# codelion/adaptive-classifier

Hardware: AMD Instinct MI355X
Metric: predict() queries/sec + kNN GB/s vs HBM roofline, 768-d (higher is better)
Workload: dtype f32

## Files before the change

### adaptive-classifier_amd/csrc/bert.hip

```cpp
#include "common.h"
#include "attention_core.h"

#include <math.h>
#include <atomic>
#include <chrono>
#include <string.h>

namespace {

typedef float f32x4 __attribute__((ext_vector_type(4)));
constexpr int kMaxVec = 8;

__device__ __forceinline__ float wave_sum(float v) {
#pragma unroll
    for (int o = 1; o < 64; o <<= 1) v += __shfl_xor(v, o);
    return v;
}

template <bool F16 = false>
__device__ __forceinline__ void layernorm_store(f32x4 (&x)[kMaxVec], int H, int lane, const float* g,
                                                const float* b, float eps, float* dst, uint16_t* planes = nullptr,
                                                int64_t rows = 0, int64_t row = 0) {
    const int nv = H >> 2;
    float s = 0.f;
#pragma unroll
    for (int e = 0; e < kMaxVec; ++e)
        if (lane + 64 * e < nv) s += (x[e].x + x[e].y) + (x[e].z + x[e].w);
    const float mean = wave_sum(s) / (float)H;
    float q = 0.f;
#pragma unroll
    for (int e = 0; e < kMaxVec; ++e)
        if (lane + 64 * e < nv) {
            const float d0 = x[e].x - mean, d1 = x[e].y - mean, d2 = x[e].z - mean, d3 = x[e].w - mean;
            q += (d0 * d0 + d1 * d1) + (d2 * d2 + d3 * d3);
        }
    const float var = wave_sum(q) / (float)H;
    const float rstd = 1.0f / sqrtf(var + eps);
#pragma unroll
    for (int e = 0; e < kMaxVec; ++e) {
        const int c4 = lane + 64 * e;
        if (c4 < nv) {
            const f32x4 gg = *reinterpret_cast<const f32x4*>(g + 4 * c4);
            const f32x4 bb = *reinterpret_cast<const f32x4*>(b + 4 * c4);
            f32x4 y;
            y.x = (x[e].x - mean) * rstd * gg.x + bb.x;
            y.y = (x[e].y - mean) * rstd * gg.y + bb.y;
            y.z = (x[e].z - mean) * rstd * gg.z + bb.z;
            y.w = (x[e].w - mean) * rstd * gg.w + bb.w;
            *reinterpret_cast<f32x4*>(dst + 4 * c4) = y;
            if (planes)
                ac::emit_planes4(planes + ac::plane_off(rows, row, 4 * c4), rows * (int64_t)H, y, F16);
        }
    }
}

template <bool F16>
__global__ __launch_bounds__(256) void embed_ln_kernel(const int64_t* ids, const int64_t* type_ids, int T, int S,
                                                       int H, const float* word, const float* pos,
                                                       const float* type, const float* g, const float* b,
                                                       float eps, float* out, uint16_t* planes,
                                                       const int32_t* __restrict__ tok_src = nullptr,
                                                       const int32_t* __restrict__ t_dev = nullptr) {
    if (t_dev) T = t_dev[0];
    const int lane = threadIdx.x & 63;
    const int t = blockIdx.x * 4 + (threadIdx.x >> 6);
    if (t >= T) return;
    const int src = tok_src ? tok_src[t] : t;
    const int64_t id = ids[src];
    const int64_t tt = type_ids ? type_ids[src] : 0;
    const int p = src % S;
    const int nv = H >> 2;
    f32x4 x[kMaxVec];
#pragma unroll
    for (int e = 0; e < kMaxVec; ++e) {
        const int c4 = lane + 64 * e;
        if (c4 < nv) {
            const f32x4 w = *reinterpret_cast<const f32x4*>(word + id * H + 4 * c4);
            if (type) {
                const f32x4 ty = *reinterpret_cast<const f32x4*>(type + tt * H + 4 * c4);
                const f32x4 po = *reinterpret_cast<const f32x4*>(pos + (int64_t)p * H + 4 * c4);
                x[e] = (w + ty) + po;
            } else {
                x[e] = w;
            }
        }
    }
    layernorm_store<F16>(x, H, lane, g, b, eps, out + (int64_t)t * H, planes, T, t);
}

template <bool F16>
__global__ __launch_bounds__(256) void ln_kernel_t(const float* in, int T, int H, const float* g, const float* b,
                                                   float eps, float* out, uint16_t* planes, int64_t in_stride) {
    const int lane = threadIdx.x & 63;
    const int t = blockIdx.x * 4 + (threadIdx.x >> 6);
    if (t >= T) return;
    const int nv = H >> 2;
    f32x4 x[kMaxVec];
#pragma unroll
    for (int e = 0; e < kMaxVec; ++e) {
        const int c4 = lane + 64 * e;
        if (c4 < nv) x[e] = *reinterpret_cast<const f32x4*>(in + (int64_t)t * in_stride + 4 * c4);
    }
    layernorm_store<F16>(x, H, lane, g, b, eps, out + (int64_t)t * H, planes, T, t);
}

inline void launch_ln(bool f16, int blocks, hipStream_t stream, const float* in, int T, int H, const float* g, const float* b,
                      float eps, float* out, uint16_t* planes, int64_t in_stride) {
    if (f16) hipLaunchKernelGGL(ln_kernel_t<true>, dim3(blocks), dim3(256), 0, stream, in, T, H, g, b, eps, out, planes, in_stride);
    else hipLaunchKernelGGL(ln_kernel_t<false>, dim3(blocks), dim3(256), 0, stream, in, T, H, g, b, eps, out, planes, in_stride);
}

__global__ __launch_bounds__(256) void splitk_ln_normalize_kernel(const float* __restrict__ part, int ksplit, int M, int H,
                                                                  const float* __restrict__ bias, const float* __restrict__ residual,
                                                                  int64_t ldr, const float* __restrict__ g, const float* __restrict__ be,
                                                                  float eps, float* __restrict__ out, int64_t ldo) {
    const int lane = threadIdx.x & 63;
    const int i = blockIdx.x * (blockDim.x >> 6) + (threadIdx.x >> 6);
    if (i >= M) return;
    const int nv = H >> 2;
    const size_t slice = (size_t)M * H;
    f32x4 x[kMaxVec];
    const f32x4 zero4 = {0.f, 0.f, 0.f, 0.f};
#pragma unroll
    for (int e = 0; e < kMaxVec; ++e) x[e] = zero4;
    for (int z0 = 0; z0 < ksplit; z0 += 4) {
        f32x4 t[4][kMaxVec];
#pragma unroll
        for (int u = 0; u < 4; ++u)
#pragma unroll
            for (int e = 0; e < kMaxVec; ++e) {
                const int c4 = lane + 64 * e;
                t[u][e] = (z0 + u < ksplit && c4 < nv) ? *reinterpret_cast<const f32x4*>(part + (size_t)(z0 + u) * slice + (size_t)i * H + 4 * c4) : zero4;
            }
#pragma unroll
        for (int u = 0; u < 4; ++u)
            if (z0 + u < ksplit) {
#pragma unroll
                for (int e = 0; e < kMaxVec; ++e)
                    if (z0 + u == 0) x[e] = t[u][e];
                    else { x[e].x += t[u][e].x; x[e].y += t[u][e].y; x[e].z += t[u][e].z; x[e].w += t[u][e].w; }
            }
    }
#pragma unroll
    for (int e = 0; e < kMaxVec; ++e) {
        const int c4 = lane + 64 * e;
        if (c4 < nv) {
            const f32x4 s = x[e];
            const f32x4 bb = *reinterpret_cast<const f32x4*>(bias + 4 * c4);
            const f32x4 rr = *reinterpret_cast<const f32x4*>(residual + (int64_t)i * ldr + 4 * c4);
            x[e].x = (s.x + bb.x) + rr.x; x[e].y = (s.y + bb.y) + rr.y; x[e].z = (s.z + bb.z) + rr.z; x[e].w = (s.w + bb.w) + rr.w;
        }
    }
    float s = 0.f;
#pragma unroll
    for (int e = 0; e < kMaxVec; ++e)
        if (lane + 64 * e < nv) s += (x[e].x + x[e].y) + (x[e].z + x[e].w);
    const float mean = wave_sum(s) / (float)H;
    float q = 0.f;
#pragma unroll
    for (int e = 0; e < kMaxVec; ++e)
        if (lane + 64 * e < nv) {
            const float d0 = x[e].x - mean, d1 = x[e].y - mean, d2 = x[e].z - mean, d3 = x[e].w - mean;
            q += (d0 * d0 + d1 * d1) + (d2 * d2 + d3 * d3);
        }
    const float var = wave_sum(q) / (float)H;
    const float rstd = 1.0f / sqrtf(var + eps);
    float ss = 0.f;
#pragma unroll
    for (int e = 0; e < kMaxVec; ++e) {
        const int c4 = lane + 64 * e;
        if (c4 < nv) {
            const f32x4 gg = *reinterpret_cast<const f32x4*>(g + 4 * c4);
            const f32x4 bb = *reinterpret_cast<const f32x4*>(be + 4 * c4);
            f32x4 y;
            y.x = (x[e].x - mean) * rstd * gg.x + bb.x;
            y.y = (x[e].y - mean) * rstd * gg.y + bb.y;
            y.z = (x[e].z - mean) * rstd * gg.z + bb.z;
            y.w = (x[e].w - mean) * rstd * gg.w + bb.w;
            x[e] = y;
            ss = fmaf(y.x, y.x, ss); ss = fmaf(y.y, y.y, ss); ss = fmaf(y.z, y.z, ss); ss = fmaf(y.w, y.w, ss);
        }
    }
    const float nrm = fmaxf(sqrtf(wave_sum(ss)), 1e-12f);
#pragma unroll
    for (int e = 0; e < kMaxVec; ++e) {
        const int c4 = lane + 64 * e;
        if (c4 < nv) {
            f32x4 y = x[e];
            y.x = y.x / nrm; y.y = y.y / nrm; y.z = y.z / nrm; y.w = y.w / nrm;
            float* dst = out + (int64_t)i * ldo + 4 * c4;
            dst[0] = y.x; dst[1] = y.y; dst[2] = y.z; dst[3] = y.w;
        }
    }
    for (int c = H + lane; c < ldo; c += 64) out[(int64_t)i * ldo + c] = 0.f;
}

__global__ __launch_bounds__(256) void cls_normalize_kernel(const float* x, int b, int S, int H, float* out,
                                                            int64_t ldo) {
    const int lane = threadIdx.x & 63;
    const int i = blockIdx.x * 4 + (threadIdx.x >> 6);
    if (i >= b) return;
    const float* src = x + (int64_t)i * S * H;
    float s = 0.f;
    for (int c = lane; c < H; c += 64) s = fmaf(src[c], src[c], s);
    const float nrm = fmaxf(sqrtf(wave_sum(s)), 1e-12f);
    for (int c = lane; c < H; c += 64) out[(int64_t)i * ldo + c] = src[c] / nrm;
    for (int c = H + lane; c < ldo; c += 64) out[(int64_t)i * ldo + c] = 0.f;
}

template <bool NORM>
__global__ __launch_bounds__(256) void pool_mean_normalize_kernel(const float* __restrict__ x, const int64_t* __restrict__ mask,
                                                                  const int32_t* __restrict__ cu, int S, int H,
                                                                  const float* __restrict__ g, const float* __restrict__ be, float eps,
                                                                  float* __restrict__ out, int64_t ldo) {
    extern __shared__ __attribute__((aligned(16))) float pool_part[];
    __shared__ int pool_count[4];
    const int lane = threadIdx.x & 63, wv = threadIdx.x >> 6, i = blockIdx.x;
    const int nv = H >> 2;
    const int64_t row0 = cu ? (int64_t)cu[i] : (int64_t)i * S;
    const int n = cu ? cu[i + 1] - cu[i] : S;
    const int64_t* mk = (!cu && mask) ? mask + (int64_t)i * S : nullptr;
    const f32x4 zero4 = {0.f, 0.f, 0.f, 0.f};
    f32x4 acc[kMaxVec];
#pragma unroll
    for (int e = 0; e < kMaxVec; ++e) acc[e] = zero4;
    int count = 0;
    for (int t = wv; t < n; t += 4) {
        if (mk && mk[t] == 0) continue;
        const float* src = x + (row0 + t) * (int64_t)H;
        f32x4 r[kMaxVec];
#pragma unroll
        for (int e = 0; e < kMaxVec; ++e) {
            const int c4 = lane + 64 * e;
            r[e] = c4 < nv ? *reinterpret_cast<const f32x4*>(src + 4 * c4) : zero4;
        }
        if constexpr (NORM) {
            float s = 0.f;
#pragma unroll
            for (int e = 0; e < kMaxVec; ++e)
                if (lane + 64 * e < nv) s += (r[e].x + r[e].y) + (r[e].z + r[e].w);
            const float mean = wave_sum(s) / (float)H;
            float q = 0.f;
#pragma unroll
            for (int e = 0; e < kMaxVec; ++e)
                if (lane + 64 * e < nv) {
                    const float d0 = r[e].x - mean, d1 = r[e].y - mean, d2 = r[e].z - mean, d3 = r[e].w - mean;
                    q += (d0 * d0 + d1 * d1) + (d2 * d2 + d3 * d3);
                }
            const float var = wave_sum(q) / (float)H;
            const float rstd = 1.0f / sqrtf(var + eps);
#pragma unroll
            for (int e = 0; e < kMaxVec; ++e) {
                const int c4 = lane + 64 * e;
                if (c4 < nv) {
                    const f32x4 gg = *reinterpret_cast<const f32x4*>(g + 4 * c4);
                    const f32x4 bb = *reinterpret_cast<const f32x4*>(be + 4 * c4);
                    f32x4 y;
                    y.x = (r[e].x - mean) * rstd * gg.x + bb.x;
                    y.y = (r[e].y - mean) * rstd * gg.y + bb.y;
                    y.z = (r[e].z - mean) * rstd * gg.z + bb.z;
                    y.w = (r[e].w - mean) * rstd * gg.w + bb.w;
                    r[e] = y;
                }
            }
        }
#pragma unroll
        for (int e = 0; e < kMaxVec; ++e) { acc[e].x += r[e].x; acc[e].y += r[e].y; acc[e].z += r[e].z; acc[e].w += r[e].w; }
        ++count;
    }
    if (wv > 0) {
#pragma unroll
        for (int e = 0; e < kMaxVec; ++e) {
            const int c4 = lane + 64 * e;
            if (c4 < nv) *reinterpret_cast<f32x4*>(pool_part + (size_t)(wv - 1) * H + 4 * c4) = acc[e];
        }
        if (lane == 0) pool_count[wv] = count;
    }
    __syncthreads();
    if (wv > 0) return;
    for (int w = 1; w < 4; ++w) {
#pragma unroll
        for (int e = 0; e < kMaxVec; ++e) {
            const int c4 = lane + 64 * e;
            if (c4 < nv) {
                const f32x4 p = *reinterpret_cast<const f32x4*>(pool_part + (size_t)(w - 1) * H + 4 * c4);
                acc[e].x += p.x; acc[e].y += p.y; acc[e].z += p.z; acc[e].w += p.w;
            }
        }
        count += pool_count[w];
    }
    const float den = (float)(count > 1 ? count : 1);
    float ss = 0.f;
#pragma unroll
    for (int e = 0; e < kMaxVec; ++e)
        if (lane + 64 * e < nv) {
            f32x4 y = acc[e];
            y.x = y.x / den; y.y = y.y / den; y.z = y.z / den; y.w = y.w / den;
            acc[e] = y;
            ss = fmaf(y.x, y.x, ss); ss = fmaf(y.y, y.y, ss); ss = fmaf(y.z, y.z, ss); ss = fmaf(y.w, y.w, ss);
        }
    const float nrm = fmaxf(sqrtf(wave_sum(ss)), 1e-12f);
#pragma unroll
    for (int e = 0; e < kMaxVec; ++e) {
        const int c4 = lane + 64 * e;
        if (c4 < nv) {
            float* dst = out + (int64_t)i * ldo + 4 * c4;
            dst[0] = acc[e].x / nrm; dst[1] = acc[e].y / nrm; dst[2] = acc[e].z / nrm; dst[3] = acc[e].w / nrm;
        }
    }
    for (int c = H + lane; c < ldo; c += 64) out[(int64_t)i * ldo + c] = 0.f;
}

constexpr int DH = 64;
constexpr int KT = 64;

using acattn::f32x16;
using acattn::rope_rotate;

__device__ __forceinline__ const float* rel_bias_row(int head, const float* table, int span) {
    return table + (int64_t)head * (2 * span - 1) + (span - 1);
}
template <bool ROPE, int DHT = 64, bool BIAS = false, typename... REL>
__global__ __launch_bounds__(64) void attention_mfma_kernel(const float* qkv, const int64_t* mask, int S_, int H,
                                                            float scale, float* ctx, uint16_t* ctx_planes,
                                                            const float* rope_cos, const float* rope_sin,
                                                            int window, const int32_t* __restrict__ cu = nullptr,
                                                            int64_t total_rows = 0, int f16 = 0, int boundary_stride = 0,
                                                            int nseq = 0, REL... rel) {
    static_assert(sizeof...(REL) == (BIAS ? 2 : 0), "the bias table and its span come with BIAS, and only then");
    const int lane = threadIdx.x;
    const int qt = blockIdx.x, head = blockIdx.y;
    int bi = blockIdx.z;
    if (boundary_stride > 0) {
        const int brow = boundary_stride * ((int)blockIdx.z + 1);
        int lo = 0, hi = nseq;
        while (hi - lo > 1) { const int mid = (lo + hi) >> 1; if (cu[mid] <= brow) lo = mid; else hi = mid; }
        if (cu[lo] == brow || brow >= cu[nseq]) return;
        bi = lo;
    }
    const int64_t ld = 3 * (int64_t)H;
    const int64_t row0 = cu ? (int64_t)cu[bi] : (int64_t)bi * S_;
    const int S = cu ? cu[bi + 1] - cu[bi] : S_;
    if (qt * 32 >= S) return;
    const float* base = qkv + row0 * ld + head * DHT;
    const int64_t rows = cu ? total_rows : (int64_t)gridDim.z * S_;
    if constexpr (BIAS)
        acattn::attention_tile<ROPE, DHT, true, true, true>(base, base + H, base + 2 * H, ld, S, qt, lane, scale,
                                                            mask ? mask + (int64_t)bi * S_ : nullptr, rope_cos, rope_sin, window,
                                                            ctx ? ctx + row0 * H + head * DHT : nullptr, H, ctx_planes, rows, row0,
                                                            head * DHT, f16, rel_bias_row(head, rel...));
    else
        acattn::attention_tile<ROPE, DHT>(base, base + H, base + 2 * H, ld, S, qt, lane, scale, mask ? mask + (int64_t)bi * S_ : nullptr,
                                          rope_cos, rope_sin, window, ctx ? ctx + row0 * H + head * DHT : nullptr, H, ctx_planes, rows,
                                          row0, head * DHT, f16);
}

template <bool ROPE, int DHT = 64, int KTT = KT, bool BIAS = false, typename... REL>
__global__ __launch_bounds__(64) void attention_cls_kernel(const float* qkv, const int64_t* mask, int S_, int H,
                                                           float scale, float* ctx_cls, const float* rope_cos,
                                                           const float* rope_sin, int window,
                                                           const int32_t* __restrict__ cu = nullptr,
                                                           const float* __restrict__ q_cls = nullptr, REL... rel) {
    static_assert(sizeof...(REL) == (BIAS ? 2 : 0), "the bias table and its span come with BIAS, and only then");
    static_assert(DHT == 64 || (DHT == 32 && !ROPE), "head dim 64, or 32 without RoPE");
    __shared__ float Ks[KTT][DHT + 1];
    __shared__ __attribute__((aligned(16))) float Vs[KTT][DHT];
    __shared__ float qs[DHT];
    __shared__ float ps[KTT];
    const int lane = threadIdx.x;
    const int head = blockIdx.x, bi = blockIdx.y;
    const int64_t ld = 3 * (int64_t)H;
    const int64_t row0 = cu ? (int64_t)cu[bi] : (int64_t)bi * S_;
    const int S = cu ? cu[bi + 1] - cu[bi] : S_;
    const float* base = qkv + row0 * ld + head * DHT;
    if (lane < DHT) qs[lane] = (q_cls ? q_cls[(int64_t)bi * H + head * DHT + lane] : base[lane]) * scale;
    float m = -INFINITY, l = 0.f, o = 0.f;
    const int Svis = (window >= 0 && window + 1 < S) ? window + 1 : S;
    for (int k0 = 0; k0 < Svis; k0 += KTT) {
        const int nk = (Svis - k0) < KTT ? (Svis - k0) : KTT;
        const int kl = lane < KTT ? lane : 0;
        __syncthreads();
        constexpr int LPR = DHT / 4;
        for (int r = lane / LPR; r < KTT; r += 64 / LPR) {
            const int c = (lane % LPR) * 4;
            f32x4 kv = {0.f, 0.f, 0.f, 0.f}, vv = {0.f, 0.f, 0.f, 0.f};
            if (r < nk) {
                const float* kp = base + (int64_t)(k0 + r) * ld + H;
                kv = *reinterpret_cast<const f32x4*>(kp + c);
                vv = *reinterpret_cast<const f32x4*>(kp + H + c);
            }
            Ks[r][c] = kv.x; Ks[r][c + 1] = kv.y; Ks[r][c + 2] = kv.z; Ks[r][c + 3] = kv.w;
            *reinterpret_cast<f32x4*>(&Vs[r][c]) = vv;
        }
        __syncthreads();
        const bool valid = lane < nk && (!mask || mask[(int64_t)bi * S_ + k0 + lane] != 0);
        float sc = 0.f;
        if constexpr (ROPE) {
            const int pos = (k0 + lane < S) ? k0 + lane : S - 1;
            const float* cs = rope_cos + (int64_t)pos * 32;
            const float* sn = rope_sin + (int64_t)pos * 32;
#pragma unroll 8
            for (int d = 0; d < 32; ++d) {
                const float lo = Ks[kl][d], hi = Ks[kl][d + 32], c = cs[d], sv = sn[d];
                sc = fmaf(qs[d], lo * c + (-hi) * sv, sc);
                sc = fmaf(qs[d + 32], hi * c + lo * sv, sc);
            }
        } else {
#pragma unroll 16
            for (int d = 0; d < DHT; ++d) sc = fmaf(qs[d], Ks[kl][d], sc);
        }
        if constexpr (BIAS) sc = sc + rel_bias_row(head, rel...)[(k0 + lane < S) ? k0 + lane : S - 1];
        sc = valid ? sc : -INFINITY;
        float cmax = sc;
#pragma unroll
        for (int off = 1; off < 64; off <<= 1) cmax = fmaxf(cmax, __shfl_xor(cmax, off));
        const float m_new = fmaxf(m, cmax);
        if (m_new == -INFINITY) continue;
        const float corr = expf(m - m_new);
        const float p = expf(sc - m_new);
        if (lane < KTT) ps[lane] = p;
        float psum = p;
#pragma unroll
        for (int off = 1; off < 64; off <<= 1) psum += __shfl_xor(psum, off);
        l = l * corr + psum;
        o *= corr;
        __syncthreads();
        if (lane < DHT)
            for (int j = 0; j < nk; ++j) o = fmaf(ps[j], Vs[j][lane], o);
        m = m_new;
    }
    if (lane < DHT) ctx_cls[(int64_t)bi * H + head * DHT + lane] = l > 0.f ? o / l : 0.f;
}

__global__ __launch_bounds__(256) void geglu_kernel(const float* __restrict__ u, int64_t T, int I, float* __restrict__ g,
                                                    uint16_t* __restrict__ planes, int interleaved32) {
    const int nq = I >> 3;
    const int64_t idx = (int64_t)blockIdx.x * 256 + threadIdx.x;
    if (idx >= T * nq) return;
    const int64_t row = idx / nq;
    const int q = (int)(idx - row * nq);
    const int c = 8 * q;
    const float* a = u + row * 2 * (int64_t)I + (interleaved32 ? (c >> 5) * 64 + (c & 31) : c);
    const int goff = interleaved32 ? 32 : I;
    f32x4 o[2];
#pragma unroll
    for (int e = 0; e < 2; ++e) {
        const f32x4 x = *reinterpret_cast<const f32x4*>(a + 4 * e);
        const f32x4 gate = *reinterpret_cast<const f32x4*>(a + goff + 4 * e);
#pragma unroll
        for (int c = 0; c < 4; ++c) o[e][c] = ac::gelu_erf(x[c]) * gate[c];
        *reinterpret_cast<f32x4*>(g + row * I + 8 * q + 4 * e) = o[e];
    }
    if (planes) {
        uint4 Hh, Mm, Ll;
        ac::split8(o[0], o[1], Hh, Mm, Ll);
        uint16_t* p = planes + ac::plane_off(T, row, 8 * q);
        const int64_t plane = T * (int64_t)I;
        *reinterpret_cast<uint4*>(p) = Hh;
        *reinterpret_cast<uint4*>(p + plane) = Mm;
        *reinterpret_cast<uint4*>(p + 2 * plane) = Ll;
    }
}

__global__ __launch_bounds__(256) void pack_lens_kernel(const int64_t* __restrict__ mask, int b, int S, int32_t* __restrict__ lens,
                                                        int32_t* __restrict__ info) {
    const int lane = threadIdx.x & 63;
    const int s = blockIdx.x * 4 + (threadIdx.x >> 6);
    if (s >= b) return;
    int n = 0, bad = 0;
    for (int p0 = 0; p0 < S; p0 += 64) {
        const int p = p0 + lane;
        const bool on = p < S && mask[(int64_t)s * S + p] != 0;
        const uint64_t m = __ballot(on);
        const int ones = __popcll(m);
        const uint64_t want = ones == 64 ? ~0ull : ((1ull << ones) - 1);
        if (m != want || (ones > 0 && n != p0)) bad = 1;
        n += ones;
    }
    if (lane == 0) { lens[s] = n; if (bad || n == 0) atomicOr(&info[1], 1); }
}
__global__ __launch_bounds__(1024) void pack_scan_kernel(const int32_t* __restrict__ lens, int b, int32_t* __restrict__ cu,
                                                         int32_t* __restrict__ info) {
    __shared__ int part[1024];
    const int tid = threadIdx.x;
    const int per = (b + 1023) / 1024;
    int sum = 0, mx = 0;
    for (int i = tid * per; i < (tid + 1) * per && i < b; ++i) { sum += lens[i]; mx = lens[i] > mx ? lens[i] : mx; }
    part[tid] = sum;
    __syncthreads();
    for (int o = 1; o < 1024; o <<= 1) {
        const int v = tid >= o ? part[tid - o] : 0;
        __syncthreads();
        part[tid] += v;
        __syncthreads();
    }
    int run = tid ? part[tid - 1] : 0;
    for (int i = tid * per; i < (tid + 1) * per && i < b; ++i) { cu[i] = run; run += lens[i]; }
    if (tid == 1023) { cu[b] = part[1023]; info[0] = part[1023]; }
    atomicMax(&info[2], mx);
}
__global__ __launch_bounds__(256) void pack_fill_kernel(const int32_t* __restrict__ cu, int b, int S, int32_t* __restrict__ tok_src) {
    const int lane = threadIdx.x & 63;
    const int s = blockIdx.x * 4 + (threadIdx.x >> 6);
    if (s >= b) return;
    const int r0 = cu[s], n = cu[s + 1] - r0;
    for (int p = lane; p < n; p += 64) tok_src[r0 + p] = s * S + p;
}
__global__ __launch_bounds__(256) void gather_rows_kernel(const float* __restrict__ in, const int32_t* __restrict__ rows, int n, int H,
                                                          float* __restrict__ out) {
    const int lane = threadIdx.x & 63;
    const int i = blockIdx.x * 4 + (threadIdx.x >> 6);
    if (i >= n) return;
    const f32x4* src = reinterpret_cast<const f32x4*>(in + (int64_t)rows[i] * H);
    f32x4* dst = reinterpret_cast<f32x4*>(out + (int64_t)i * H);
    for (int c = lane; c < (H >> 2); c += 64) dst[c] = src[c];
}

struct BertWs {
    size_t x, qkv, ctx, y, ffn, xp, ctxp, ffnp, small, lnctl, lnpart, cu, tile_seq, attn_xchg, pack_src, pack_info, total;
    size_t lnctl_bytes, attn_xchg_bytes;
};
__global__ __launch_bounds__(256) void iota_cu_kernel(int32_t* cu, int b, int S) {
    const int i = blockIdx.x * 256 + threadIdx.x;
    if (i <= b) cu[i] = i * S;
}
__global__ __launch_bounds__(1024) void pack_prologue_kernel(const int64_t* __restrict__ mask, int b, int S, int32_t* __restrict__ cu,
                                                             int32_t* __restrict__ tok_src, int32_t* __restrict__ info,
                                                             int32_t* __restrict__ tile_seq, unsigned* __restrict__ zero_a, int zero_a_words,
                                                             unsigned* __restrict__ zero_b, int zero_b_words, unsigned* __restrict__ verdict,
                                                             int clear_verdict, int32_t* host_slot, int epoch) {
    extern __shared__ int32_t pk_lds[];
#ifdef AC_PROLOGUE_STAMPS
#define PK_STAMP(i) do { if (threadIdx.x == 0) reinterpret_cast<unsigned long long*>(info + 16)[i] = __builtin_amdgcn_s_memrealtime(); } while (0)
#else
#define PK_STAMP(i) do {} while (0)
#endif
    PK_STAMP(0);
    __shared__ int part[16];
    __shared__ int s_bad, s_longest;
    int32_t* lens = pk_lds;
    int32_t* cus = pk_lds + b;
    const int tid = threadIdx.x, n = b * S;
    for (int i = tid; i < b; i += 1024) lens[i] = 0;
    if (tid == 0) { s_bad = 0; s_longest = 0; }
    __syncthreads();
    for (int i = tid; i < zero_a_words; i += 1024) zero_a[i] = 0u;
    for (int i = tid; i < zero_b_words; i += 1024) zero_b[i] = 0u;
    if (tid == 0) {
        if (clear_verdict) { verdict[0] = 0u; verdict[1] = 0u; }
        else { verdict[1] |= verdict[0]; verdict[0] = 0u; }
    }
    PK_STAMP(1);
    int bad = 0;
    for (int i0 = 8 * tid; i0 < n; i0 += 8 * 1024) {
        int64_t m[9];
        m[0] = i0 > 0 ? mask[i0 - 1] : 1;
#pragma unroll
        for (int u = 0; u < 8; ++u) m[u + 1] = i0 + u < n ? mask[i0 + u] : 0;
        int row = i0 / S, p = i0 - row * S, ones = 0;
#pragma unroll
        for (int u = 0; u < 8; ++u) {
            if (i0 + u < n && m[u + 1] != 0) {
                ++ones;
                if (p > 0 && m[u] == 0) bad = 1;
            }
            if (++p == S) {
                if (ones) atomicAdd(&lens[row], ones);
                p = 0; ++row; ones = 0;
            }
        }
        if (ones) atomicAdd(&lens[row], ones);
    }
    if (bad) s_bad = 1;
    __syncthreads();
    PK_STAMP(2);
    const int per = (b + 1023) / 1024;
    int sum = 0, mx = 0;
    for (int i = tid * per; i < (tid + 1) * per && i < b; ++i) {
        const int l = lens[i];
        sum += l; mx = l > mx ? l : mx;
        if (l == 0) bad = 1;
    }
    if (bad) s_bad = 1;
#pragma unroll
    for (int o = 1; o < 64; o <<= 1) { const int v = __shfl_xor(mx, o); mx = v > mx ? v : mx; }
    if ((tid & 63) == 0 && mx) atomicMax(&s_longest, mx);
    int incl = sum;
#pragma unroll
    for (int o = 1; o < 64; o <<= 1) {
        const int v = __shfl_up(incl, o);
        if ((tid & 63) >= o) incl += v;
    }
    if ((tid & 63) == 63) part[tid >> 6] = incl;
    __syncthreads();
    int wave_base = 0, grand = 0;
#pragma unroll
    for (int wv = 0; wv < 16; ++wv) {
        const int t = part[wv];
        if (wv < (tid >> 6)) wave_base += t;
        grand += t;
    }
    incl += wave_base;
    int run = incl - sum;
    for (int i = tid * per; i < (tid + 1) * per && i < b; ++i) { cus[i] = run; cu[i] = run; run += lens[i]; }
    const int total = grand;
    PK_STAMP(3);
    if (tid == 0) {
        cus[b] = total; cu[b] = total; info[0] = total; info[1] = s_bad; info[2] = s_longest; info[3] = 0;
        if (host_slot) {
            host_slot[0] = total; host_slot[1] = s_bad; host_slot[2] = s_longest;
            __threadfence_system();
            __hip_atomic_store(&host_slot[3], epoch, __ATOMIC_RELEASE, __HIP_MEMORY_SCOPE_SYSTEM);
        }
    }
    __syncthreads();
    PK_STAMP(4);
    for (int i = tid; i < n; i += 1024) {
        const int q = i / S, p = i - q * S;
        if (p < lens[q]) tok_src[cus[q] + p] = i;
    }
    PK_STAMP(5);
    const int ntiles = (total + ac::kQkvAttnRows - 1) / ac::kQkvAttnRows, lane = tid & 63;
    for (int t = tid >> 6; t < ntiles; t += 16) {
        auto first_at_or_after = [&](int row) { int lo = 0, hi = b; while (lo < hi) { const int mid = (lo + hi) >> 1; if (cus[mid] < row) lo = mid + 1; else hi = mid; } return lo; };
        const int sb = first_at_or_after(t * ac::kQkvAttnRows), se = first_at_or_after((t + 1) * ac::kQkvAttnRows), ns = se - sb;
        for (int i = lane; i < ac::kQkvAttnCu; i += 64) {
            int v = 0;
            if (i == 0) v = ns;
            else if (i - 1 <= ns) v = cus[sb + i - 1];
            tile_seq[(size_t)t * ac::kQkvAttnCu + i] = v;
        }
    }
    PK_STAMP(6);
}
constexpr size_t kLnAbortHead = 256;
__global__ void ln_verdict_roll_kernel(unsigned* w) {
    w[1] |= w[0];
    w[0] = 0u;
}
BertWs bert_ws(const ac_bert_config& c, int b, int S) {
    BertWs w;
    const size_t T = (size_t)b * S;
    size_t off = kLnAbortHead;
    auto take = [&](size_t n) { size_t o = off; off += ac::align_up(n * sizeof(float), 256); return o; };
    w.x = take(T * c.hidden);
    w.qkv = take(T * 3 * c.hidden);
    w.ctx = take(T * c.hidden);
    w.y = take(T * c.hidden);
    w.ffn = take(T * c.intermediate);
    auto take16 = [&](size_t n) { size_t o = off; off += ac::align_up(n * sizeof(uint16_t), 256); return o; };
    w.xp = take16(3 * T * c.hidden);
    w.ctxp = take16(3 * T * c.hidden);
    w.ffnp = take16(3 * T * c.intermediate);
    w.small = off;
    if (T <= 32) off += ac::bert_small_ws_bytes(c.hidden, c.intermediate);
    w.lnctl = off;
    w.lnctl_bytes = ac::align_up((size_t)c.layers * 2 * ac::pipe_ln_panels((int)T) * sizeof(unsigned), 256);
    off += w.lnctl_bytes;
    w.lnpart = off;
    off += ac::align_up(ac::pipe_ln_part_bytes((int)T, c.hidden), 256);
    w.cu = off;
    off += ac::align_up((size_t)(b + 1) * sizeof(int32_t), 256);
    w.tile_seq = off;
    off += ac::align_up(ac::qkv_attn_tile_seq_bytes((int)T), 256);
    w.attn_xchg = off;
    w.attn_xchg_bytes = ac::align_up(((T + ac::kQkvAttnRows - 1) / ac::kQkvAttnRows) * (size_t)c.heads * sizeof(unsigned), 256);
    off += w.attn_xchg_bytes;
    w.pack_src = off;
    off += ac::align_up(T * sizeof(int32_t), 256);
    w.pack_info = off;
    off += 256;
    w.total = off;
    return w;
}

int check_cfg(const ac_bert_config* c) {
    AC_REQUIRE(c != nullptr, AC_EINVAL, "bert: config is NULL");
    AC_REQUIRE(c->hidden >= 64 && c->layers >= 1 && c->heads >= 1 && c->intermediate >= 4, AC_EINVAL,
               "bert: bad config");
    AC_REQUIRE(c->hidden % 4 == 0 && c->hidden <= 64 * 4 * kMaxVec, AC_EUNSUPPORTED,
               "bert: hidden=%d unsupported (must be a multiple of 4 and <= %d)", c->hidden, 64 * 4 * kMaxVec);
    AC_REQUIRE(c->hidden == c->heads * 64 || c->hidden == c->heads * 32, AC_EUNSUPPORTED,
               "bert: head dim %d unsupported (64 or 32)", c->hidden / c->heads);
    AC_REQUIRE(c->gemm_arith_opt >= 0 && c->gemm_arith_opt <= 3 && c->ln_fusion_opt >= 0 && c->ln_fusion_opt <= 3 &&
                   c->one_launch_opt >= 0 && c->one_launch_opt <= 2, AC_EINVAL,
               "bert: per-call options out of range (gemm_arith_opt %d, ln_fusion_opt %d, one_launch_opt %d)", c->gemm_arith_opt,
               c->ln_fusion_opt, c->one_launch_opt);
    AC_REQUIRE(c->pool_opt >= AC_POOL_DEFAULT && c->pool_opt <= AC_POOL_MEAN, AC_EINVAL,
               "bert: pool_opt %d out of range (0 = default = AC_POOL_CLS, AC_POOL_CLS, AC_POOL_MEAN)", c->pool_opt);
    return AC_OK;
}

int check_rel_bias(const ac_bert_weights* w, int S, const char* who) {
    AC_REQUIRE(!w->attn_rel_bias || (w->rel_span >= 1 && S <= w->rel_span), AC_EINVAL,
               "%s: S=%d exceeds rel_span=%d of the relative position bias table (attn_rel_bias needs 1 <= S <= rel_span)", who, S,
               w->rel_span);
    return AC_OK;
}

}

extern "C" int ac_bert_workspace(const ac_bert_config* cfg, int b, int S, size_t* bytes) {
    int rc = check_cfg(cfg);
    if (rc) return rc;
    AC_REQUIRE(bytes && b >= 0 && S >= 1, AC_EINVAL, "bert workspace: bad arguments");
    *bytes = bert_ws(*cfg, b > 0 ? b : 1, S).total;
    return AC_OK;
}

namespace {

static bool tail_fused() {
    const char* e = getenv("AC_BERT_TAIL_FUSED");
    return !(e && atoi(e) == 0);
}
inline bool pools_mean(int pool_opt) { return pool_opt == AC_POOL_MEAN; }
inline int token_layers(const ac_bert_config& c) { return pools_mean(c.pool_opt) ? c.layers : c.layers - 1; }
struct EncodePlan { bool wplanes, pl, f16; };
EncodePlan encode_plan(const ac_bert_config& c, const ac_bert_weights* w, int T) {
    const int H = c.hidden, I = c.intermediate;
    EncodePlan p;
    p.wplanes = w->qkv_w3 && w->ao_w3 && w->ff1_w3 && w->ff2_w3;
    p.pl = p.wplanes && ac::linear_takes_planes(T, H, H) && ac::linear_takes_planes(T, H, I) && (H % 8) == 0;
    p.f16 = p.pl && ac::gemm_arith() == AC_GEMM_F16X2 && w->qkv_wh && w->ao_wh && w->ff1_wh && w->ff2_wh && token_layers(c) > 0 &&
            ac::linear_f16x2_takes(T, 3 * H, H) && ac::linear_f16x2_takes(T, H, H) && ac::linear_f16x2_takes(T, I, H) &&
            ac::linear_f16x2_takes(T, H, I);
    return p;
}
void launch_embed(const ac_bert_config& c, const ac_bert_weights* w, const EncodePlan& pn, const int64_t* d_ids, const int64_t* d_type_ids,
                  int rows, int S, float* x, uint16_t* xp, const int32_t* tok_src, const int32_t* t_dev, hipStream_t stream) {
    const int H = c.hidden, tok_blocks = (rows + 3) / 4;
    if (pn.f16)
        hipLaunchKernelGGL(embed_ln_kernel<true>, dim3(tok_blocks), dim3(256), 0, stream, d_ids, d_type_ids, rows, S, H,
                           w->word_emb, w->pos_emb, w->type_emb, w->emb_ln_g, w->emb_ln_b, c.ln_eps, x, xp, tok_src, t_dev);
    else
        hipLaunchKernelGGL(embed_ln_kernel<false>, dim3(tok_blocks), dim3(256), 0, stream, d_ids, d_type_ids, rows, S, H,
                           w->word_emb, w->pos_emb, w->type_emb, w->emb_ln_g, w->emb_ln_b, c.ln_eps, x,
                           pn.pl ? xp : nullptr, tok_src, t_dev);
}
constexpr int kPreCtl = 1, kPreEmbed = 2;
int bert_encode_impl(const ac_bert_config* cfg, const ac_bert_weights* w, const int64_t* d_ids, const int64_t* d_type_ids,
                     const int64_t* d_mask, int b, int S, const int32_t* cu, const int32_t* tok_src, int T, int Smax,
                     float* d_out, int64_t ldo, void* d_ws, size_t ws_bytes, hipStream_t stream, int pre = 0) {
    int rc;
    const ac_bert_config& c = *cfg;
    const BertWs ws = bert_ws(c, b, S);
    AC_REQUIRE(d_ws && ws_bytes >= ws.total, AC_EWORKSPACE, "bert_encode_cls: workspace %zu < %zu", ws_bytes, ws.total);
    char* base = (char*)d_ws;
    float* x = (float*)(base + ws.x);
    float* qkv = (float*)(base + ws.qkv);
    float* ctx = (float*)(base + ws.ctx);
    float* y = (float*)(base + ws.y);
    float* ffn = (float*)(base + ws.ffn);
    const int H = c.hidden, I = c.intermediate;

    uint16_t* xp = (uint16_t*)(base + ws.xp);
    uint16_t* ctxp = (uint16_t*)(base + ws.ctxp);
    uint16_t* ffnp = (uint16_t*)(base + ws.ffnp);
    const EncodePlan pn = encode_plan(c, w, T);
    const bool wplanes = pn.wplanes, pl = pn.pl;
    const bool f16 = pn.f16;
    const bool pool = pools_mean(c.pool_opt);
    const bool fuse_ln = pl && token_layers(c) > 0 && ac::pipe_ln_applies(T, H, H) && ac::pipe_ln_applies(T, H, I);
    unsigned* ln_abort = (unsigned*)base;
    if (!(pre & kPreCtl)) {
        hipLaunchKernelGGL(ln_verdict_roll_kernel, dim3(1), dim3(1), 0, stream, ln_abort);
        AC_LAUNCH_CHECK();
    }
    unsigned* ln_count = (unsigned*)(base + ws.lnctl);
    const int ln_panels = ac::pipe_ln_panels(T);
    if (fuse_ln && !(pre & kPreCtl)) AC_HIP_CHECK(hipMemsetAsync(base + ws.lnctl, 0, ws.lnctl_bytes, stream));

    if (!(pre & kPreEmbed)) {
        launch_embed(c, w, pn, d_ids, d_type_ids, T, S, x, xp, tok_src, nullptr, stream);
        AC_LAUNCH_CHECK();
    }
    const int dh = c.hidden / c.heads;
    const float scale = 1.0f / sqrtf((float)dh);
    const int32_t* cu_at = cu;
    const float* rel = w->attn_rel_bias;
    const int rel_span = w->rel_span;
    const bool fuse_attn = !rel && pl && token_layers(c) > 0 && dh == 64 && (cu || !d_mask) && ac::qkv_attn_applies(T, H, c.heads, Smax);
    if (fuse_attn && !cu) {
        int32_t* cuw = (int32_t*)(base + ws.cu);
        hipLaunchKernelGGL(iota_cu_kernel, dim3((b + 256) / 256), dim3(256), 0, stream, cuw, b, S);
        AC_LAUNCH_CHECK();
        cu_at = cuw;
    }
    int32_t* tile_seq = (int32_t*)(base + ws.tile_seq);
    unsigned* attn_xchg = nullptr;
    if (fuse_attn) {
        if (!(pre & kPreCtl) || !cu) {
            rc = ac::qkv_attn_tile_seq(cu_at, b, T, tile_seq, stream);
            if (rc) return rc;
        }
        if (ac::qkv_attn_exchange_applies(T, c.heads, (int)f16)) {
            attn_xchg = (unsigned*)(base + ws.attn_xchg);
            if (!(pre & kPreCtl)) AC_HIP_CHECK(hipMemsetAsync(attn_xchg, 0, ws.attn_xchg_bytes, stream));
        }
    }
    for (int l = 0; l < c.layers; ++l) {
        const uint16_t* qkv_w3 = wplanes ? w->qkv_w3[l] : nullptr;
        const uint16_t* ao_w3 = wplanes ? w->ao_w3[l] : nullptr;
        const uint16_t* ff1_w3 = wplanes ? w->ff1_w3[l] : nullptr;
        const uint16_t* ff2_w3 = wplanes ? w->ff2_w3[l] : nullptr;
        const bool last = (l == c.layers - 1) && !pool;
        const int Ml = last ? b : T;
        const bool lp = pl && !last;
        const float* resid = x;
        int64_t ldres = last ? (int64_t)S * H : H;
        const bool q_cls_only = last && T >= 4 * b;
        if (last && cu) {
            hipLaunchKernelGGL(gather_rows_kernel, dim3((b + 3) / 4), dim3(256), 0, stream, x, cu, b, H, ffn);
            AC_LAUNCH_CHECK();
            resid = ffn;
            ldres = H;
        }
        if (fuse_attn && !last) {
            rc = ac::launch_gemm_pipe_qkv_attn(xp, T, f16 ? w->qkv_wh[l] : qkv_w3, 3 * H, w->qkv_b[l], T, H, c.heads, cu_at, tile_seq, b, Smax,
                                               scale, ctxp, qkv, stream, (int)f16, attn_xchg, (unsigned)(l + 1), ln_abort);
            if (rc) return rc;
            const int nbound = (T - 1) / ac::kQkvAttnRows;
            if (nbound > 0 && !attn_xchg) {
                hipLaunchKernelGGL((attention_mfma_kernel<false, 64>), dim3((Smax + 31) / 32, c.heads, nbound), dim3(64), 0, stream, qkv,
                                   nullptr, S, H, scale, ctx, ctxp, nullptr, nullptr, -1, cu_at, (int64_t)T, (int)f16, ac::kQkvAttnRows, b);
                AC_LAUNCH_CHECK();
            }
        } else if (q_cls_only) {
            const int64_t HH = (int64_t)H * H;
            rc = f16 ? ac::linear_f16x2(xp, w->qkv_wh[l] + (int64_t)H * 8, w->qkv_b[l] + H, nullptr, 0, qkv + H, 3 * H, nullptr, T, 2 * H, H, 0,
                                        stream, 3 * H)
                     : ac::linear_f32(x, H, w->qkv_w[l] + HH, H, w->qkv_b[l] + H, nullptr, 0, qkv + H, 3 * H, T, 2 * H, H, 0, nullptr, 1.f,
                                      stream, 0.f, 0, qkv_w3 ? qkv_w3 + (int64_t)H * 8 : nullptr, pl ? xp : nullptr, nullptr, 3 * H);
            if (rc) return rc;
            rc = ac::linear_f32_splitk(resid, ldres, w->qkv_w[l], H, w->qkv_b[l], nullptr, 0, y, H, b, H, H, 0, qkv_w3, ctx,
                                       (size_t)T * H * sizeof(float), stream, 3 * H);
        } else {
            rc = f16 ? ac::linear_f16x2(xp, w->qkv_wh[l], w->qkv_b[l], nullptr, 0, qkv, 3 * H, nullptr, T, 3 * H, H, 0, stream)
                     : ac::linear_f32(x, H, w->qkv_w[l], H, w->qkv_b[l], nullptr, 0, qkv, 3 * H, T, 3 * H, H, 0, nullptr, 1.f,
                                      stream, 0.f, 0, qkv_w3, pl ? xp : nullptr);
        }
        if (rc) return rc;
        if (fuse_attn && !last) {
        } else if (last) {
            const float* qc = q_cls_only ? y : nullptr;
            if (rel && dh == 64 && Smax <= 32)
                hipLaunchKernelGGL((attention_cls_kernel<false, 64, 32, true>), dim3(c.heads, b), dim3(64), 0, stream, qkv, d_mask, S, H, scale,
                                   ctx, nullptr, nullptr, -1, cu, qc, rel, rel_span);
            else if (rel && dh == 64)
                hipLaunchKernelGGL((attention_cls_kernel<false, 64, KT, true>), dim3(c.heads, b), dim3(64), 0, stream, qkv, d_mask, S, H, scale,
                                   ctx, nullptr, nullptr, -1, cu, qc, rel, rel_span);
            else if (rel)
                hipLaunchKernelGGL((attention_cls_kernel<false, 32, KT, true>), dim3(c.heads, b), dim3(64), 0, stream, qkv, d_mask, S, H, scale,
                                   ctx, nullptr, nullptr, -1, cu, qc, rel, rel_span);
            else if (dh == 64 && Smax <= 32)
                hipLaunchKernelGGL((attention_cls_kernel<false, 64, 32>), dim3(c.heads, b), dim3(64), 0, stream, qkv, d_mask, S, H, scale,
                                   ctx, nullptr, nullptr, -1, cu, qc);
            else if (dh == 64)
                hipLaunchKernelGGL((attention_cls_kernel<false, 64>), dim3(c.heads, b), dim3(64), 0, stream, qkv, d_mask, S, H, scale,
                                   ctx, nullptr, nullptr, -1, cu, qc);
            else
                hipLaunchKernelGGL((attention_cls_kernel<false, 32>), dim3(c.heads, b), dim3(64), 0, stream, qkv, d_mask, S, H, scale,
                                   ctx, nullptr, nullptr, -1, cu, qc);
        } else {
            if (rel && dh == 64)
                hipLaunchKernelGGL((attention_mfma_kernel<false, 64, true>), dim3((Smax + 31) / 32, c.heads, b), dim3(64), 0, stream, qkv,
                                   d_mask, S, H, scale, ctx, lp ? ctxp : nullptr, nullptr, nullptr, -1, cu, (int64_t)T, (int)f16, 0, 0,
                                   rel, rel_span);
            else if (rel)
                hipLaunchKernelGGL((attention_mfma_kernel<false, 32, true>), dim3((Smax + 31) / 32, c.heads, b), dim3(64), 0, stream, qkv,
                                   d_mask, S, H, scale, ctx, lp ? ctxp : nullptr, nullptr, nullptr, -1, cu, (int64_t)T, (int)f16, 0, 0,
                                   rel, rel_span);
            else if (dh == 64)
                hipLaunchKernelGGL((attention_mfma_kernel<false, 64>), dim3((Smax + 31) / 32, c.heads, b), dim3(64), 0, stream, qkv,
                                   d_mask, S, H, scale, ctx, lp ? ctxp : nullptr, nullptr, nullptr, -1, cu, (int64_t)T, (int)f16);
            else
                hipLaunchKernelGGL((attention_mfma_kernel<false, 32>), dim3((Smax + 31) / 32, c.heads, b), dim3(64), 0, stream, qkv,
                                   d_mask, S, H, scale, ctx, lp ? ctxp : nullptr, nullptr, nullptr, -1, cu, (int64_t)T, (int)f16);
        }
        AC_LAUNCH_CHECK();
        const int lblocks = (Ml + 3) / 4;
        const bool fl = fuse_ln && lp;
        if (fl) {
            rc = ac::launch_gemm_pipe_ln(ctxp, Ml, f16 ? w->ao_wh[l] : ao_w3, H, w->ao_b[l], x, H, x, H, Ml, H, H, w->ln1_g[l], w->ln1_b[l], c.ln_eps,
                                         base + ws.lnpart, ln_count + (size_t)(2 * l) * ln_panels, ln_abort, xp, stream, (int)f16);
            if (rc) return rc;
        } else {
            rc = last ? ac::linear_f32_splitk(ctx, H, w->ao_w[l], H, w->ao_b[l], resid, ldres, y, H, Ml, H, H, 0, ao_w3, qkv,
                                              (size_t)T * 3 * H * sizeof(float), stream)
                      : (f16 ? ac::linear_f16x2(ctxp, w->ao_wh[l], w->ao_b[l], resid, ldres, y, H, nullptr, Ml, H, H, 0, stream)
                             : ac::linear_f32(ctx, H, w->ao_w[l], H, w->ao_b[l], resid, ldres, y, H, Ml, H, H, 0, nullptr, 1.f, stream,
                                              0.f, 0, ao_w3, lp ? ctxp : nullptr));
            if (rc) return rc;
            launch_ln(f16, lblocks, stream, y, Ml, H, w->ln1_g[l], w->ln1_b[l], c.ln_eps, last ? ctx : x, lp ? xp : nullptr, (int64_t)H);
            AC_LAUNCH_CHECK();
        }
        float* x1 = last ? ctx : x;
        rc = last ? ac::linear_f32_splitk(x1, H, w->ff1_w[l], H, w->ff1_b[l], nullptr, 0, ffn, I, Ml, I, H, 2, ff1_w3, qkv,
                                          (size_t)T * 3 * H * sizeof(float), stream)
                  : (f16 ? ac::linear_f16x2(xp, w->ff1_wh[l], w->ff1_b[l], nullptr, 0, nullptr, I, ffnp, Ml, I, H, 2, stream)
                         : ac::linear_f32(x1, H, w->ff1_w[l], H, w->ff1_b[l], nullptr, 0, ffn, I, Ml, I, H, 2, nullptr, 1.f, stream,
                                          0.f, 0, ff1_w3, lp ? xp : nullptr, lp ? ffnp : nullptr));
        if (rc) return rc;
        if (fl) {
            rc = ac::launch_gemm_pipe_ln(ffnp, Ml, f16 ? w->ff2_wh[l] : ff2_w3, H, w->ff2_b[l], x, H, x, H, Ml, H, I, w->ln2_g[l], w->ln2_b[l], c.ln_eps,
                                         base + ws.lnpart, ln_count + (size_t)(2 * l + 1) * ln_panels, ln_abort, xp, stream, (int)f16);
            if (rc) return rc;
            continue;
        }
        if (last && tail_fused()) {
            int ks = 0;
            rc = ac::linear_f32_splitk(ffn, I, w->ff2_w[l], I, w->ff2_b[l], x1, H, y, H, Ml, H, I, 0, ff2_w3, qkv,
                                       (size_t)T * 3 * H * sizeof(float), stream, 0, &ks);
            if (rc) return rc;
            if (ks > 0) {
                hipLaunchKernelGGL(splitk_ln_normalize_kernel, dim3(b), dim3(64), 0, stream, qkv, ks, b, H, w->ff2_b[l], x1, (int64_t)H,
                                   w->ln2_g[l], w->ln2_b[l], c.ln_eps, d_out, ldo);
                AC_LAUNCH_CHECK();
                return AC_OK;
            }
            launch_ln(f16, lblocks, stream, y, Ml, H, w->ln2_g[l], w->ln2_b[l], c.ln_eps, x, nullptr, (int64_t)H);
            AC_LAUNCH_CHECK();
            break;
        }
        rc = last ? ac::linear_f32_splitk(ffn, I, w->ff2_w[l], I, w->ff2_b[l], x1, H, y, H, Ml, H, I, 0, ff2_w3, qkv,
                                          (size_t)T * 3 * H * sizeof(float), stream)
                  : (f16 ? ac::linear_f16x2(ffnp, w->ff2_wh[l], w->ff2_b[l], x1, H, y, H, nullptr, Ml, H, I, 0, stream)
                         : ac::linear_f32(ffn, I, w->ff2_w[l], I, w->ff2_b[l], x1, H, y, H, Ml, H, I, 0, nullptr, 1.f, stream, 0.f, 0,
                                          ff2_w3, lp ? ffnp : nullptr));
        if (rc) return rc;
        launch_ln(f16, lblocks, stream, y, Ml, H, w->ln2_g[l], w->ln2_b[l], c.ln_eps, x, lp ? xp : nullptr, (int64_t)H);
        AC_LAUNCH_CHECK();
    }
    if (pool) {
        hipLaunchKernelGGL(pool_mean_normalize_kernel<false>, dim3(b), dim3(256), 3 * (size_t)H * sizeof(float), stream, x, d_mask, cu, S, H,
                           (const float*)nullptr, (const float*)nullptr, 0.f, d_out, ldo);
        AC_LAUNCH_CHECK();
        return AC_OK;
    }
    hipLaunchKernelGGL(cls_normalize_kernel, dim3((b + 3) / 4), dim3(256), 0, stream, x, b, 1, H, d_out, ldo);
    AC_LAUNCH_CHECK();
    return AC_OK;
}

}

extern "C" int ac_bert_encode_cls_opts(const ac_bert_config* cfg, const ac_bert_weights* w, const int64_t* d_ids,
                                       const int64_t* d_type_ids, const int64_t* d_mask, int b, int S,
                                       float* d_out, int64_t ldo, void* d_ws, size_t ws_bytes, int opts, int* used_one_launch,
                                       ac_stream_t stream_) {
    if (used_one_launch) *used_one_launch = 0;
    int rc = check_cfg(cfg);
    if (rc) return rc;
    if (b == 0) return AC_OK;
    const ac::CallScope scope(cfg->gemm_arith_opt, cfg->ln_fusion_opt, cfg->one_launch_opt);
    AC_REQUIRE(w && d_ids && d_out && b > 0 && S >= 1 && S <= cfg->max_pos && ldo >= cfg->hidden, AC_EINVAL,
               "bert_encode_cls: bad arguments (b=%d S=%d max_pos=%d)", b, S, cfg->max_pos);
    if ((rc = check_rel_bias(w, S, "bert_encode_cls"))) return rc;
    if (b * S <= 32 && !(opts & AC_BERT_LAYERED) && !pools_mean(cfg->pool_opt) && !w->attn_rel_bias) {
        const BertWs ws = bert_ws(*cfg, b, S);
        AC_REQUIRE(d_ws && ws_bytes >= ws.total, AC_EWORKSPACE, "bert_encode_cls: workspace %zu < %zu", ws_bytes, ws.total);
        rc = ac::bert_small_encode(*cfg, *w, d_ids, d_type_ids, d_mask, b, S, d_out, ldo, (char*)d_ws + ws.small, (hipStream_t)stream_);
        if (rc == AC_OK && used_one_launch) *used_one_launch = 1;
        if (rc != 1) return rc;
    }
    return bert_encode_impl(cfg, w, d_ids, d_type_ids, d_mask, b, S, nullptr, nullptr, b * S, S, d_out, ldo, d_ws, ws_bytes,
                            (hipStream_t)stream_);
}

extern "C" int ac_bert_encode_cls(const ac_bert_config* cfg, const ac_bert_weights* w, const int64_t* d_ids,
                                  const int64_t* d_type_ids, const int64_t* d_mask, int b, int S,
                                  float* d_out, int64_t ldo, void* d_ws, size_t ws_bytes, ac_stream_t stream_) {
    return ac_bert_encode_cls_opts(cfg, w, d_ids, d_type_ids, d_mask, b, S, d_out, ldo, d_ws, ws_bytes, 0, nullptr, stream_);
}

extern "C" int ac_bert_one_launch_status(const ac_bert_config* cfg, int b, int S, const void* d_ws, size_t ws_bytes,
                                         int* aborted, ac_stream_t stream_) {
    int rc = check_cfg(cfg);
    if (rc) return rc;
    AC_REQUIRE(aborted && d_ws && b > 0 && S >= 1 && b * S <= 32, AC_EINVAL, "bert_one_launch_status: bad arguments");
    const BertWs ws = bert_ws(*cfg, b, S);
    AC_REQUIRE(ws_bytes >= ws.total, AC_EWORKSPACE, "bert_one_launch_status: workspace %zu < %zu", ws_bytes, ws.total);
    return ac::bert_small_aborted(cfg->hidden, cfg->intermediate, (const char*)d_ws + ws.small, (hipStream_t)stream_, aborted);
}

extern "C" int ac_bert_ln_fusion_status(const ac_bert_config* cfg, int b, int S, const void* d_ws, size_t ws_bytes,
                                       int* aborted, ac_stream_t stream_) {
    int rc = check_cfg(cfg);
    if (rc) return rc;
    (void)b; (void)S;
    AC_REQUIRE(aborted && d_ws && ws_bytes >= kLnAbortHead, AC_EINVAL, "bert_ln_fusion_status: bad arguments");
    unsigned flag[2] = {0, 0};
    AC_HIP_CHECK(hipMemcpyAsync(flag, (const char*)d_ws, sizeof(flag), hipMemcpyDeviceToHost, (hipStream_t)stream_));
    AC_HIP_CHECK(hipStreamSynchronize((hipStream_t)stream_));
    *aborted = (flag[0] | flag[1]) != 0;
    return AC_OK;
}

extern "C" int ac_bert_ln_fusion_clear(void* d_ws, size_t ws_bytes, ac_stream_t stream_) {
    AC_REQUIRE(d_ws && ws_bytes >= kLnAbortHead, AC_EINVAL, "bert_ln_fusion_clear: bad arguments");
    AC_HIP_CHECK(hipMemsetAsync(d_ws, 0, 2 * sizeof(unsigned), (hipStream_t)stream_));
    return AC_OK;
}

extern "C" int ac_bert_pack(const int64_t* d_mask, int b, int S, int32_t* d_cu, int32_t* d_tok_src, int32_t* d_info,
                            ac_stream_t stream_) {
    hipStream_t stream = (hipStream_t)stream_;
    AC_REQUIRE(d_mask && d_cu && d_tok_src && d_info && b >= 1 && S >= 1, AC_EINVAL, "bert_pack: bad arguments");
    AC_HIP_CHECK(hipMemsetAsync(d_info, 0, 4 * sizeof(int32_t), stream));
    int32_t* lens = d_tok_src;
    hipLaunchKernelGGL(pack_lens_kernel, dim3((b + 3) / 4), dim3(256), 0, stream, d_mask, b, S, lens, d_info);
    AC_LAUNCH_CHECK();
    hipLaunchKernelGGL(pack_scan_kernel, dim3(1), dim3(1024), 0, stream, lens, b, d_cu, d_info);
    AC_LAUNCH_CHECK();
    hipLaunchKernelGGL(pack_fill_kernel, dim3((b + 3) / 4), dim3(256), 0, stream, d_cu, b, S, d_tok_src);
    AC_LAUNCH_CHECK();
    return AC_OK;
}

namespace {
int32_t* info_slot(int* epoch_out) {
    static int32_t* base = [] {
        void* p = nullptr;
        if (hipHostMalloc(&p, 64 * 64, hipHostMallocCoherent | hipHostMallocMapped | hipHostMallocPortable) != hipSuccess) { (void)hipGetLastError(); return (int32_t*)nullptr; }
        memset(p, 0, 64 * 64);
        return (int32_t*)p;
    }();
    static std::atomic<unsigned> next{0};
    const unsigned n = next.fetch_add(1, std::memory_order_relaxed) + 1;
    *epoch_out = (int)(n & 0x3fffffff) + 1;
    return base ? base + 16 * (n & 63) : nullptr;
}
}

static std::atomic<long long> g_unpad_wait_ns{0};
extern "C" long long ac_bert_unpad_last_wait_ns(void) { return g_unpad_wait_ns.load(std::memory_order_relaxed); }

extern "C" int ac_bert_encode_cls_unpad(const ac_bert_config* cfg, const ac_bert_weights* w, const int64_t* d_ids,
                                        const int64_t* d_type_ids, const int64_t* d_mask, int b, int S, float* d_out, int64_t ldo,
                                        void* d_ws, size_t ws_bytes, int clear_verdict, int* total_tokens, int* path, ac_stream_t stream_) {
    if (total_tokens) *total_tokens = 0;
    if (path) *path = AC_BERT_PATH_PACKED;
    int rc = check_cfg(cfg);
    if (rc) return rc;
    if (b == 0) return AC_OK;
    hipStream_t stream = (hipStream_t)stream_;
    const ac::CallScope scope(cfg->gemm_arith_opt, cfg->ln_fusion_opt, cfg->one_launch_opt);
    AC_REQUIRE(w && d_ids && d_mask && d_out && b > 0 && S >= 2 && S <= cfg->max_pos && ldo >= cfg->hidden && (int64_t)b * S > 32 &&
                   (int64_t)b * S < ((int64_t)1 << 30),
               AC_EINVAL, "bert_encode_cls_unpad: bad arguments (b=%d S=%d max_pos=%d; more than 32 token rows)", b, S, cfg->max_pos);
    if ((rc = check_rel_bias(w, S, "bert_encode_cls_unpad"))) return rc;
    const ac_bert_config& c = *cfg;
    const BertWs ws = bert_ws(c, b, S);
    AC_REQUIRE(d_ws && ws_bytes >= ws.total, AC_EWORKSPACE, "bert_encode_cls_unpad: workspace %zu < %zu", ws_bytes, ws.total);
    char* base = (char*)d_ws;
    int32_t* cu = (int32_t*)(base + ws.cu);
    int32_t* src = (int32_t*)(base + ws.pack_src);
    int32_t* info = (int32_t*)(base + ws.pack_info);
    int epoch = 0;
    int32_t* slot = info_slot(&epoch);
    const size_t lds = (size_t)(2 * b + 1) * sizeof(int32_t);
    AC_REQUIRE(slot && lds <= 96 * 1024, AC_EUNSUPPORTED, "bert_encode_cls_unpad: %d sequences in one call (or no pinned host memory): "
               "use ac_bert_pack + ac_bert_encode_cls_packed", b);
    if (lds > 48 * 1024) (void)hipFuncSetAttribute((const void*)pack_prologue_kernel, hipFuncAttributeMaxDynamicSharedMemorySize, (int)lds);
    hipLaunchKernelGGL(pack_prologue_kernel, dim3(1), dim3(1024), lds, stream, d_mask, b, S, cu, src, info, (int32_t*)(base + ws.tile_seq),
                       (unsigned*)(base + ws.lnctl), (int)(ws.lnctl_bytes / 4), (unsigned*)(base + ws.attn_xchg), (int)(ws.attn_xchg_bytes / 4),
                       (unsigned*)base, clear_verdict, slot, epoch);
    AC_LAUNCH_CHECK();
    const EncodePlan lo = encode_plan(c, w, b), hi = encode_plan(c, w, b * S);
    const bool early = lo.pl == hi.pl && lo.f16 == hi.f16;
    if (early) {
        launch_embed(c, w, hi, d_ids, d_type_ids, b * S, S, (float*)(base + ws.x), (uint16_t*)(base + ws.xp), src, info, stream);
        AC_LAUNCH_CHECK();
    }
    volatile int32_t* vs = slot;
    bool seen = false;
    const auto wait_t0 = std::chrono::steady_clock::now();
    for (int spin = 0; spin < 200000 && !seen; ++spin) {
        seen = __atomic_load_n(&vs[3], __ATOMIC_ACQUIRE) == epoch;
        if (!seen) __builtin_ia32_pause();
    }
    if (!seen) {
        AC_HIP_CHECK(hipStreamSynchronize(stream));
        seen = __atomic_load_n(&vs[3], __ATOMIC_ACQUIRE) == epoch;
        AC_REQUIRE(seen, AC_EHIP, "bert_encode_cls_unpad: the packing kernel's report never arrived");
    }
    g_unpad_wait_ns.store(std::chrono::duration_cast<std::chrono::nanoseconds>(std::chrono::steady_clock::now() - wait_t0).count(),
                          std::memory_order_relaxed);
    const int total = vs[0], not_prefix = vs[1], longest = vs[2];
    if (total_tokens) *total_tokens = total;
    if (!not_prefix && total < b * S) {
        AC_REQUIRE(total >= b && longest >= 1 && longest <= S, AC_EHIP, "bert_encode_cls_unpad: bad report (%d rows, longest %d)", total, longest);
        return bert_encode_impl(cfg, w, d_ids, d_type_ids, nullptr, b, S, cu, src, total, longest, d_out, ldo, d_ws, ws_bytes, stream,
                                kPreCtl | (early ? kPreEmbed : 0));
    }
    if (path) *path = not_prefix ? AC_BERT_PATH_PADDED_MASK : AC_BERT_PATH_PADDED;
    if (total_tokens) *total_tokens = b * S;
    return bert_encode_impl(cfg, w, d_ids, d_type_ids, not_prefix ? d_mask : nullptr, b, S, nullptr, nullptr, b * S, S, d_out, ldo, d_ws,
                            ws_bytes, stream);
}

extern "C" int ac_bert_encode_cls_packed(const ac_bert_config* cfg, const ac_bert_weights* w, const int64_t* d_ids,
                                         const int64_t* d_type_ids, int b, int S, const int32_t* d_cu,
                                         const int32_t* d_tok_src, int total_tokens, int longest, float* d_out, int64_t ldo,
                                         void* d_ws, size_t ws_bytes, ac_stream_t stream_) {
    int rc = check_cfg(cfg);
    if (rc) return rc;
    if (b == 0) return AC_OK;
    const ac::CallScope scope(cfg->gemm_arith_opt, cfg->ln_fusion_opt, cfg->one_launch_opt);
    AC_REQUIRE(w && d_ids && d_out && d_cu && d_tok_src && b > 0 && S >= 1 && S <= cfg->max_pos && ldo >= cfg->hidden &&
                   total_tokens >= b && total_tokens <= b * S && longest >= 1 && longest <= S,
               AC_EINVAL, "bert_encode_cls_packed: bad arguments (b=%d S=%d tokens=%d longest=%d)", b, S, total_tokens, longest);
    if ((rc = check_rel_bias(w, S, "bert_encode_cls_packed"))) return rc;
    return bert_encode_impl(cfg, w, d_ids, d_type_ids, nullptr, b, S, d_cu, d_tok_src, total_tokens, longest, d_out, ldo, d_ws,
                            ws_bytes, (hipStream_t)stream_);
}

namespace {

struct MbWs {
    size_t x, y, xn, qkv, ctx, u, g, xnp, ctxp, gp, total;
};
MbWs mb_ws(const ac_modernbert_config& c, int b, int S) {
    MbWs w;
    const size_t T = (size_t)b * S, H = c.hidden, I = c.intermediate;
    size_t off = 0;
    auto take = [&](size_t n) { size_t o = off; off += ac::align_up(n * sizeof(float), 256); return o; };
    auto take16 = [&](size_t n) { size_t o = off; off += ac::align_up(n * sizeof(uint16_t), 256); return o; };
    w.x = take(T * H); w.y = take(T * H); w.xn = take(T * H);
    w.qkv = take(T * 3 * H); w.ctx = take(T * H);
    w.u = take(T * 2 * I); w.g = take(T * I);
    w.xnp = take16(3 * T * H); w.ctxp = take16(3 * T * H); w.gp = take16(3 * T * I);
    w.total = off;
    return w;
}

int check_mb(const ac_modernbert_config* c) {
    AC_REQUIRE(c != nullptr, AC_EINVAL, "modernbert: config is NULL");
    AC_REQUIRE(c->hidden >= 64 && c->layers >= 1 && c->heads >= 1 && c->intermediate >= 8 && c->global_every >= 1 &&
                   c->local_window >= 0 && c->max_pos >= 1,
               AC_EINVAL, "modernbert: bad config");
    AC_REQUIRE(c->hidden % 4 == 0 && c->hidden <= 64 * 4 * kMaxVec && c->intermediate % 8 == 0, AC_EUNSUPPORTED,
               "modernbert: hidden=%d / intermediate=%d unsupported", c->hidden, c->intermediate);
    AC_REQUIRE(c->hidden == c->heads * DH, AC_EUNSUPPORTED, "modernbert: head dim %d unsupported (only %d)",
               c->hidden / c->heads, DH);
    AC_REQUIRE(c->gemm_arith_opt >= 0 && c->gemm_arith_opt <= 3, AC_EINVAL, "modernbert: gemm_arith_opt %d out of range", c->gemm_arith_opt);
    AC_REQUIRE(c->pool_opt >= AC_POOL_DEFAULT && c->pool_opt <= AC_POOL_MEAN, AC_EINVAL,
               "modernbert: pool_opt %d out of range (0 = default = AC_POOL_CLS, AC_POOL_CLS, AC_POOL_MEAN)", c->pool_opt);
    return AC_OK;
}

}

extern "C" int ac_modernbert_workspace(const ac_modernbert_config* cfg, int b, int S, size_t* bytes) {
    int rc = check_mb(cfg);
    if (rc) return rc;
    AC_REQUIRE(bytes && b >= 0 && S >= 1, AC_EINVAL, "modernbert workspace: bad arguments");
    *bytes = mb_ws(*cfg, b > 0 ? b : 1, S).total;
    return AC_OK;
}

namespace {

int modernbert_encode_impl(const ac_modernbert_config* cfg, const ac_modernbert_weights* w, const int64_t* d_ids,
                           const int64_t* d_mask, int b, int S, const int32_t* cu, const int32_t* tok_src, int T, int Smax,
                           float* d_out, int64_t ldo, void* d_ws, size_t ws_bytes, hipStream_t stream) {
    int rc;
    AC_REQUIRE(w->tok_emb && w->emb_norm_g && w->final_norm_g && w->zero_bias && w->rope_cos_global &&
                   w->rope_sin_global && w->rope_cos_local && w->rope_sin_local && w->attn_norm_g && w->wqkv && w->wo &&
                   w->mlp_norm_g && w->wi && w->wo2,
               AC_EINVAL, "modernbert_encode_cls: missing weights");
    const ac_modernbert_config& c = *cfg;
    const MbWs ws = mb_ws(c, b, S);
    AC_REQUIRE(d_ws && ws_bytes >= ws.total, AC_EWORKSPACE, "modernbert_encode_cls: workspace %zu < %zu", ws_bytes, ws.total);
    char* base = (char*)d_ws;
    float* x = (float*)(base + ws.x);
    float* y = (float*)(base + ws.y);
    float* xn = (float*)(base + ws.xn);
    float* qkv = (float*)(base + ws.qkv);
    float* ctx = (float*)(base + ws.ctx);
    float* u = (float*)(base + ws.u);
    float* g = (float*)(base + ws.g);
    uint16_t* xnp = (uint16_t*)(base + ws.xnp);
    uint16_t* ctxp = (uint16_t*)(base + ws.ctxp);
    uint16_t* gp = (uint16_t*)(base + ws.gp);
    const int H = c.hidden, I = c.intermediate;
    const int tok_blocks = (T + 3) / 4;
    const float* zb = w->zero_bias;
    auto opt = [&](const float* const* arr, int l) -> const float* { return (arr && arr[l]) ? arr[l] : zb; };
    const bool wplanes = w->wqkv3 && w->wo3 && w->wi3 && w->wo23;
    const bool pl = wplanes && ac::linear_takes_planes(T, H, H) && ac::linear_takes_planes(T, H, I) && (H % 8) == 0;

    hipLaunchKernelGGL(embed_ln_kernel<false>, dim3(tok_blocks), dim3(256), 0, stream, d_ids, (const int64_t*)nullptr, T, S, H,
                       w->tok_emb, (const float*)nullptr, (const float*)nullptr, w->emb_norm_g,
                       w->emb_norm_b ? w->emb_norm_b : zb, c.norm_eps, x, pl ? xnp : nullptr, tok_src);
    AC_LAUNCH_CHECK();
    const float scale = 1.0f / sqrtf((float)DH);
    const bool pool = pools_mean(c.pool_opt);
    for (int l = 0; l < c.layers; ++l) {
        const float* a_in = x;
        if (l > 0) {
            AC_REQUIRE(w->attn_norm_g[l] != nullptr, AC_EINVAL, "modernbert: attn_norm weight of layer %d is NULL", l);
            hipLaunchKernelGGL(ln_kernel_t<false>, dim3(tok_blocks), dim3(256), 0, stream, x, T, H, w->attn_norm_g[l],
                               opt(w->attn_norm_b, l), c.norm_eps, xn, pl ? xnp : nullptr, (int64_t)H);
            AC_LAUNCH_CHECK();
            a_in = xn;
        }
        rc = ac::linear_f32(a_in, H, w->wqkv[l], H, opt(w->wqkv_b, l), nullptr, 0, qkv, 3 * H, T, 3 * H, H, 0, nullptr,
                            1.f, stream, 0.f, 0, wplanes ? w->wqkv3[l] : nullptr, pl ? xnp : nullptr);
        if (rc) return rc;
        const bool global = (l % c.global_every) == 0;
        const float* rc_ = global ? w->rope_cos_global : w->rope_cos_local;
        const float* rs_ = global ? w->rope_sin_global : w->rope_sin_local;
        const int win = global ? -1 : c.local_window;
        const bool last = (l == c.layers - 1) && !pool;
        const int Ml = last ? b : T;
        const bool lp = last ? (wplanes && ac::linear_takes_planes(b, H, H) && ac::linear_takes_planes(b, H, I) && (H % 8) == 0) : pl;
        const float* resid = x;
        int64_t ldres = last ? (int64_t)S * H : H;
        if (last) {
            hipLaunchKernelGGL((attention_cls_kernel<true, 64>), dim3(c.heads, b), dim3(64), 0, stream, qkv, d_mask, S, H, scale, ctx,
                               rc_, rs_, win, cu);
            if (cu) {
                AC_LAUNCH_CHECK();
                hipLaunchKernelGGL(gather_rows_kernel, dim3((b + 3) / 4), dim3(256), 0, stream, x, cu, b, H, g);
                resid = g;
                ldres = H;
            }
        } else {
            hipLaunchKernelGGL((attention_mfma_kernel<true, 64>), dim3((Smax + 31) / 32, c.heads, b), dim3(64), 0, stream, qkv, d_mask,
                               S, H, scale, ctx, pl ? ctxp : nullptr, rc_, rs_, win, cu, (int64_t)T);
        }
        AC_LAUNCH_CHECK();
        rc = ac::linear_f32(ctx, H, w->wo[l], H, opt(w->wo_b, l), resid, ldres, y, H, Ml, H, H, 0, nullptr, 1.f,
                            stream, 0.f, 0, wplanes ? w->wo3[l] : nullptr, (pl && !last) ? ctxp : nullptr);
        if (rc) return rc;
        hipLaunchKernelGGL(ln_kernel_t<false>, dim3((Ml + 3) / 4), dim3(256), 0, stream, y, Ml, H, w->mlp_norm_g[l],
                           opt(w->mlp_norm_b, l), c.norm_eps, xn, lp ? xnp : nullptr, (int64_t)H);
        AC_LAUNCH_CHECK();
        if (lp && w->wi_interleaved32) {
            rc = ac::linear_f32(xn, H, w->wi[l], H, opt(w->wi_b, l), nullptr, 0, nullptr, I, Ml, 2 * I, H, 3, nullptr, 1.f,
                                stream, 0.f, 0, w->wi3[l], xnp, gp);
            if (rc) return rc;
        } else {
            rc = ac::linear_f32(xn, H, w->wi[l], H, opt(w->wi_b, l), nullptr, 0, u, 2 * I, Ml, 2 * I, H, 0, nullptr, 1.f,
                                stream, 0.f, 0, wplanes ? w->wi3[l] : nullptr, lp ? xnp : nullptr);
            if (rc) return rc;
            const int64_t units = (int64_t)Ml * (I / 8);
            hipLaunchKernelGGL(geglu_kernel, dim3((unsigned)((units + 255) / 256)), dim3(256), 0, stream, u, (int64_t)Ml, I, g,
                               lp ? gp : nullptr, w->wi_interleaved32);
            AC_LAUNCH_CHECK();
        }
        rc = ac::linear_f32(g, I, w->wo2[l], I, opt(w->wo2_b, l), y, H, x, H, Ml, H, I, 0, nullptr, 1.f, stream, 0.f, 0,
                            wplanes ? w->wo23[l] : nullptr, lp ? gp : nullptr);
        if (rc) return rc;
    }
    if (pool) {
        hipLaunchKernelGGL(pool_mean_normalize_kernel<true>, dim3(b), dim3(256), 3 * (size_t)H * sizeof(float), stream, x, d_mask, cu, S, H,
                           w->final_norm_g, w->final_norm_b ? w->final_norm_b : zb, c.norm_eps, d_out, ldo);
        AC_LAUNCH_CHECK();
        return AC_OK;
    }
    hipLaunchKernelGGL(ln_kernel_t<false>, dim3((b + 3) / 4), dim3(256), 0, stream, x, b, H, w->final_norm_g,
                       w->final_norm_b ? w->final_norm_b : zb, c.norm_eps, xn, (uint16_t*)nullptr, (int64_t)H);
    AC_LAUNCH_CHECK();
    hipLaunchKernelGGL(cls_normalize_kernel, dim3((b + 3) / 4), dim3(256), 0, stream, xn, b, 1, H, d_out, ldo);
    AC_LAUNCH_CHECK();
    return AC_OK;
}

}

extern "C" int ac_modernbert_encode_cls(const ac_modernbert_config* cfg, const ac_modernbert_weights* w,
                                        const int64_t* d_ids, const int64_t* d_mask, int b, int S, float* d_out,
                                        int64_t ldo, void* d_ws, size_t ws_bytes, ac_stream_t stream_) {
    int rc = check_mb(cfg);
    if (rc) return rc;
    if (b == 0) return AC_OK;
    const ac::CallScope scope(cfg->gemm_arith_opt, 0, 0);
    AC_REQUIRE(w && d_ids && d_out && b > 0 && S >= 1 && S <= cfg->max_pos && ldo >= cfg->hidden, AC_EINVAL,
               "modernbert_encode_cls: bad arguments (b=%d S=%d max_pos=%d)", b, S, cfg->max_pos);
    return modernbert_encode_impl(cfg, w, d_ids, d_mask, b, S, nullptr, nullptr, b * S, S, d_out, ldo, d_ws, ws_bytes,
                                  (hipStream_t)stream_);
}

extern "C" int ac_modernbert_encode_cls_packed(const ac_modernbert_config* cfg, const ac_modernbert_weights* w,
                                               const int64_t* d_ids, int b, int S, const int32_t* d_cu,
                                               const int32_t* d_tok_src, int total_tokens, int longest, float* d_out,
                                               int64_t ldo, void* d_ws, size_t ws_bytes, ac_stream_t stream_) {
    int rc = check_mb(cfg);
    if (rc) return rc;
    if (b == 0) return AC_OK;
    const ac::CallScope scope(cfg->gemm_arith_opt, 0, 0);
    AC_REQUIRE(w && d_ids && d_out && d_cu && d_tok_src && b > 0 && S >= 1 && S <= cfg->max_pos && ldo >= cfg->hidden &&
                   total_tokens >= b && total_tokens <= b * S && longest >= 1 && longest <= S,
               AC_EINVAL, "modernbert_encode_cls_packed: bad arguments (b=%d S=%d tokens=%d longest=%d)", b, S, total_tokens, longest);
    return modernbert_encode_impl(cfg, w, d_ids, nullptr, b, S, d_cu, d_tok_src, total_tokens, longest, d_out, ldo, d_ws, ws_bytes,
                                  (hipStream_t)stream_);
}
```

### adaptive-classifier_amd/csrc/common.h

```cpp
#pragma once
#include <atomic>
#include <hip/hip_runtime.h>
#include <stdarg.h>
#include <stdint.h>
#include <stdio.h>

#include "../../include/acamd.h"

namespace ac {

void set_error(const char* fmt, ...);

struct DevInfo {
    int cus;
    int lds_per_block;
    size_t hbm_bytes;
    int hw_cus;
};
const DevInfo& dev_info();

bool test_hooks_enabled();
#define AC_TEST_HOOK_ONLY(name)                                                                                                   \
    do {                                                                                                                          \
        if (!ac::test_hooks_enabled()) {                                                                                          \
            ac::set_error(name ": process-wide switches are test hooks; this process did not enable them (AC_TEST_HOOKS=1)");    \
            return AC_EUNSUPPORTED;                                                                                               \
        }                                                                                                                         \
    } while (0)

bool first_call_on_device(std::atomic<unsigned long long>& done);

#define AC_HIP_CHECK(expr)                                                              \
    do {                                                                                \
        hipError_t _e = (expr);                                                         \
        if (_e != hipSuccess) {                                                         \
            ac::set_error("%s failed: %s (%s:%d)", #expr, hipGetErrorString(_e),        \
                          __FILE__, __LINE__);                                          \
            return AC_EHIP;                                                             \
        }                                                                               \
    } while (0)

#define AC_REQUIRE(cond, code, ...)                                                     \
    do {                                                                                \
        if (!(cond)) {                                                                  \
            ac::set_error(__VA_ARGS__);                                                 \
            return (code);                                                              \
        }                                                                               \
    } while (0)

#define AC_LAUNCH_CHECK()                                                               \
    do {                                                                                \
        hipError_t _e = hipGetLastError();                                              \
        if (_e != hipSuccess) {                                                         \
            ac::set_error("kernel launch failed: %s (%s:%d)", hipGetErrorString(_e),    \
                          __FILE__, __LINE__);                                          \
            return AC_EHIP;                                                             \
        }                                                                               \
    } while (0)

__host__ __device__ static inline size_t align_up(size_t x, size_t a) { return (x + a - 1) / a * a; }
static inline int next_pow2(int x) { int p = 1; while (p < x) p <<= 1; return p; }

int linear_f32(const float* A, int64_t lda, const float* W, int64_t ldw, const float* bias,
               const float* residual, int64_t ldr, float* C, int64_t ldc, int M, int N, int K, int act,
               const uint8_t* mask, float mask_scale, hipStream_t stream, float drop_p = 0.f,
               uint64_t drop_seed = 0, const uint16_t* W_planes = nullptr, const uint16_t* A_planes = nullptr,
               uint16_t* C_planes = nullptr, int64_t w_plane_rows = 0);
int linear_f32_splitk(const float* A, int64_t lda, const float* W, int64_t ldw, const float* bias, const float* residual,
                      int64_t ldr, float* C, int64_t ldc, int M, int N, int K, int act, const uint16_t* W_planes, float* scratch,
                      size_t scratch_bytes, hipStream_t stream, int64_t w_plane_rows = 0, int* partials_only = nullptr);
bool pipe_ln_applies(int M, int N, int K);
size_t pipe_ln_part_bytes(int M, int N);
int pipe_ln_panels(int M);
int launch_gemm_pipe_ln(const uint16_t* Ap, int64_t a_rows, const uint16_t* Wp, int64_t w_rows, const float* bias,
                        const float* residual, int64_t ldr, float* C, int64_t ldc, int M, int N, int K, const float* gamma,
                        const float* beta, float eps, void* part, unsigned* count, unsigned* abort_flag, uint16_t* planes,
                        hipStream_t stream, int f16 = 0);
constexpr int kQkvAttnRows = 256;
constexpr int kQkvAttnCu = 264;
bool qkv_attn_applies(int M, int H, int heads, int smax);
size_t qkv_attn_tile_seq_bytes(int M);
int qkv_attn_tile_seq(const int32_t* cu, int b, int M, int32_t* tile_seq, hipStream_t stream);
bool qkv_attn_exchange_applies(int M, int heads, int f16);
int launch_gemm_pipe_qkv_attn(const uint16_t* Ap, int64_t a_rows, const uint16_t* Wp, int64_t w_rows, const float* bias, int M, int H,
                              int heads, const int32_t* cu, const int32_t* tile_seq, int b, int smax, float scale, uint16_t* ctx_planes,
                              float* qkv, hipStream_t stream, int f16 = 0, unsigned* exchange = nullptr, unsigned epoch = 0,
                              unsigned* abort_flag = nullptr);
bool linear_takes_planes(int M, int N, int K);

__host__ __device__ static inline bool dropout_keep(uint64_t seed, uint64_t idx, float p) {
    uint64_t z = seed + idx * 0x9E3779B97F4A7C15ull;
    z = (z ^ (z >> 30)) * 0xBF58476D1CE4E5B9ull;
    z = (z ^ (z >> 27)) * 0x94D049BB133111EBull;
    z ^= z >> 31;
    return (float)(z >> 40) * (1.0f / 16777216.0f) >= p;
}
#ifdef __HIPCC__
typedef __bf16 bf16x2_t __attribute__((ext_vector_type(2)));
typedef float f32x2_t __attribute__((ext_vector_type(2)));
typedef float f32x4_t __attribute__((ext_vector_type(4)));

__device__ __forceinline__ uint32_t pack_bf16(float a, float b) {
    const f32x2_t f = {a, b};
    return __builtin_bit_cast(uint32_t, __builtin_convertvector(f, bf16x2_t));
}
__device__ __forceinline__ void split2(float a, float b, uint32_t& h, uint32_t& m, uint32_t& l) {
    h = pack_bf16(a, b);
    const float ra = a - __uint_as_float(h << 16), rb = b - __uint_as_float(h & 0xffff0000u);
    m = pack_bf16(ra, rb);
    const float sa = ra - __uint_as_float(m << 16), sb = rb - __uint_as_float(m & 0xffff0000u);
    l = pack_bf16(sa, sb);
}
__device__ __forceinline__ void split4(const f32x4_t& x, uint2& H, uint2& M, uint2& L) {
    split2(x[0], x[1], H.x, M.x, L.x);
    split2(x[2], x[3], H.y, M.y, L.y);
}
__device__ __forceinline__ void split8(const f32x4_t& x0, const f32x4_t& x1, uint4& H, uint4& M, uint4& L) {
    split2(x0[0], x0[1], H.x, M.x, L.x);
    split2(x0[2], x0[3], H.y, M.y, L.y);
    split2(x1[0], x1[1], H.z, M.z, L.z);
    split2(x1[2], x1[3], H.w, M.w, L.w);
}
constexpr int kF16ActLog2 = 6, kF16WLog2 = 10;
constexpr float kF16ActScale = (float)(1 << kF16ActLog2), kF16OutScale = 1.0f / (float)(1 << (kF16ActLog2 + kF16WLog2));
typedef _Float16 f16x2_t __attribute__((ext_vector_type(2)));
__device__ __forceinline__ void split2h(float a, float b, float s, uint32_t& h, uint32_t& l) {
    a *= s; b *= s;
    const f16x2_t hv = {(_Float16)a, (_Float16)b};
    const f16x2_t lv = {(_Float16)(a - (float)hv[0]), (_Float16)(b - (float)hv[1])};
    h = __builtin_bit_cast(uint32_t, hv);
    l = __builtin_bit_cast(uint32_t, lv);
}
__device__ __forceinline__ void split4h(const f32x4_t& x, float s, uint2& H, uint2& L) {
    split2h(x[0], x[1], s, H.x, L.x);
    split2h(x[2], x[3], s, H.y, L.y);
}
__device__ __forceinline__ void split8h(const f32x4_t& x0, const f32x4_t& x1, float s, uint4& H, uint4& L) {
    split2h(x0[0], x0[1], s, H.x, L.x);
    split2h(x0[2], x0[3], s, H.y, L.y);
    split2h(x1[0], x1[1], s, H.z, L.z);
    split2h(x1[2], x1[3], s, H.w, L.w);
}
__device__ __forceinline__ void emit_planes4(uint16_t* p, int64_t plane, const f32x4_t& v, int f16) {
    if (f16) {
        uint2 H, L;
        split4h(v, kF16ActScale, H, L);
        *reinterpret_cast<uint2*>(p) = H;
        *reinterpret_cast<uint2*>(p + plane) = L;
    } else {
        uint2 H, M, L;
        split4(v, H, M, L);
        *reinterpret_cast<uint2*>(p) = H;
        *reinterpret_cast<uint2*>(p + plane) = M;
        *reinterpret_cast<uint2*>(p + 2 * plane) = L;
    }
}
__device__ __forceinline__ void emit_planes8(uint16_t* p, int64_t plane, const f32x4_t& v0, const f32x4_t& v1, int f16) {
    if (f16) {
        uint4 H, L;
        split8h(v0, v1, kF16ActScale, H, L);
        *reinterpret_cast<uint4*>(p) = H;
        *reinterpret_cast<uint4*>(p + plane) = L;
    } else {
        uint4 H, M, L;
        split8(v0, v1, H, M, L);
        *reinterpret_cast<uint4*>(p) = H;
        *reinterpret_cast<uint4*>(p + plane) = M;
        *reinterpret_cast<uint4*>(p + 2 * plane) = L;
    }
}
__device__ __forceinline__ float gelu_erf(float x) {
    const float t = x * 0.70710678118654752440f;
    const float a = fminf(__builtin_fabsf(t), 4.0f);
    float p = -1.160484225692926e-05f;
    p = __builtin_fmaf(p, a, 0.00015296465426217765f);
    p = __builtin_fmaf(p, a, -0.0008482354460284114f);
    p = __builtin_fmaf(p, a, 0.002274787751957774f);
    p = __builtin_fmaf(p, a, -8.480761607643217e-05f);
    p = __builtin_fmaf(p, a, -0.027724474668502808f);
    p = __builtin_fmaf(p, a, 0.1483079046010971f);
    p = __builtin_fmaf(p, a, 0.9184429049491882f);
    p = __builtin_fmaf(p, a, 1.6279072761535645f);
    const float e = __builtin_amdgcn_exp2f(-(p * a));
    const float r = __builtin_copysignf(1.0f - e, t);
    return 0.5f * x * (1.0f + r);
}

typedef float gelu_f32x2 __attribute__((ext_vector_type(2)));
__device__ __forceinline__ gelu_f32x2 gelu_erf2(gelu_f32x2 x) {
    const gelu_f32x2 t = x * 0.70710678118654752440f;
    const gelu_f32x2 a = __builtin_elementwise_min(__builtin_elementwise_abs(t), (gelu_f32x2){4.0f, 4.0f});
    gelu_f32x2 p = {-1.160484225692926e-05f, -1.160484225692926e-05f};
    p = __builtin_elementwise_fma(p, a, (gelu_f32x2){0.00015296465426217765f, 0.00015296465426217765f});
    p = __builtin_elementwise_fma(p, a, (gelu_f32x2){-0.0008482354460284114f, -0.0008482354460284114f});
    p = __builtin_elementwise_fma(p, a, (gelu_f32x2){0.002274787751957774f, 0.002274787751957774f});
    p = __builtin_elementwise_fma(p, a, (gelu_f32x2){-8.480761607643217e-05f, -8.480761607643217e-05f});
    p = __builtin_elementwise_fma(p, a, (gelu_f32x2){-0.027724474668502808f, -0.027724474668502808f});
    p = __builtin_elementwise_fma(p, a, (gelu_f32x2){0.1483079046010971f, 0.1483079046010971f});
    p = __builtin_elementwise_fma(p, a, (gelu_f32x2){0.9184429049491882f, 0.9184429049491882f});
    p = __builtin_elementwise_fma(p, a, (gelu_f32x2){1.6279072761535645f, 1.6279072761535645f});
    const gelu_f32x2 pa = p * a;
    const gelu_f32x2 e = {__builtin_amdgcn_exp2f(-pa[0]), __builtin_amdgcn_exp2f(-pa[1])};
    const gelu_f32x2 om = (gelu_f32x2){1.0f, 1.0f} - e;
    const gelu_f32x2 r = {__builtin_copysignf(om[0], t[0]), __builtin_copysignf(om[1], t[1])};
    return (x * 0.5f) * ((gelu_f32x2){1.0f, 1.0f} + r);
}

__device__ __forceinline__ int64_t plane_off(int64_t rows, int64_t row, int k) {
    return ((int64_t)(k >> 3) * rows + row) * 8 + (k & 7);
}
__device__ __forceinline__ uint32_t fkey(float f) {
    uint32_t b = __float_as_uint(f);
    return (b & 0x80000000u) ? ~b : (b | 0x80000000u);
}
__device__ __forceinline__ float fkey_inv(uint32_t k) {
    uint32_t b = (k & 0x80000000u) ? (k & 0x7fffffffu) : ~k;
    return __uint_as_float(b);
}
#endif

size_t knn_planes_bytes(int64_t rows, int D);
double knn_batch_gamma(int D);
int knn_prepare_store(const float* X, int64_t ldx, int64_t rows, int D, uint16_t* plane, float* norms, uint32_t* maxnorm_bits,
                      hipStream_t stream);
int knn_update_store(const float* X, int64_t ldx, int64_t n_old, int64_t n_new, int D, uint16_t* plane, float* norms, int64_t row0,
                     int64_t nrows, int32_t* exponent_changed, hipStream_t stream);
int knn_prepare_queries(const double* sampleD, int kp, const float* Q, int64_t ldQ, int D, int nq, const uint32_t* maxnorm_bits,
                        double gamma, uint16_t* qplane, float* thr, float* qfac, hipStream_t stream, int32_t* zero_ints = nullptr,
                        int64_t zero_count = 0);
int64_t knn_sample_rows(int64_t N, int64_t stride);
struct SelArgs;
int knn_batch_launch(bool ip, const uint16_t* Pp, const float* pnorm, int64_t N, int D, const uint16_t* Qp, int nq, const float* thr,
                     const float* qfac, float* cand_d, int32_t* cand_i, int32_t* cand_cnt, int cap, int segs, int64_t row_stride,
                     int best_only, hipStream_t stream, int32_t* clear_ctr = nullptr, int32_t* clear_stats = nullptr,
                     int two_phase_kp = 0, unsigned* wgmin = nullptr, void* ctl = nullptr,
                     const SelArgs* sel = nullptr);
bool ln_fusion_enabled();
bool knn_batch_two_phase_applies(int64_t N, int nq, int kp, int segs);
size_t knn_batch_two_phase_bytes();

struct MergeParams {
    const float* P = nullptr;
    int64_t N = 0;
    int64_t ldP = 0;
    const float* Q = nullptr;
    int64_t ldQ = 0;
    int D = 0;
    int Dp = 0;
    int k = 0;
    int kp = 0;
    int G = 0;
    int nblk = 0;
    double gamma = 0;
    const int32_t* cand_cnt = nullptr;
    int cand_cap = 0, cand_segs = 1;
    int32_t* cand_cnt_clear = nullptr;
    float* thr_out = nullptr;
    int64_t run_stride = 0;
    int64_t row_offset = 0;
    const float* part_d = nullptr;
    const int32_t* part_i = nullptr;
    const float* part_maxnorm = nullptr;
    float* outD = nullptr;
    double* outD64 = nullptr;
    int64_t* outI = nullptr;
    int32_t* flags = nullptr;
    int32_t* stats = nullptr;
    int fb_S = 0, fb_F = 0;
    double* fb_d = nullptr;
    int32_t* fb_i = nullptr;
    int32_t* fb_slotctr = nullptr;
    int thr_only = 0;
};
struct SelArgs {
    const uint64_t* sel = nullptr;
    int64_t sel_bit0 = 0;
    const int64_t* ids = nullptr;
    int64_t n_ids = 0;
    int by_ids = 0;
};
constexpr int kKnnSmallN = 8192;
struct WsTake {
    size_t off = 0;
    size_t operator()(size_t n) { const size_t o = off; off += align_up(n, 256); return o; }
};
struct ExactPlan {
    int fb_S = 1, fb_F = 1;
    size_t off_flags = 0, off_fb_d = 0, off_fb_i = 0, off_fb_ctr = 0, merge_lds = 0, fb_lds = 0;
};
void knn_exact_plan(ExactPlan* ep, WsTake& take, int k, int kp, int Dp, size_t list_bytes, int fb_F);
MergeParams knn_merge_params(const float* P, int64_t N, int64_t ldP, const float* Q, int64_t ldQ, int D, int Dp, int k, int kp,
                             int64_t row_offset, float* outD, double* outD64, int64_t* outI, int32_t* stats, char* ws,
                             const ExactPlan& ep);
int knn_merge_launch(bool ip, const MergeParams& mp, int nq, size_t attr_lds, size_t lds, hipStream_t stream, const SelArgs* sel = nullptr,
                     const float* sel_thr = nullptr);
int knn_exact_tail(bool ip, const MergeParams& mp, const ExactPlan& ep, int nq, size_t merge_lds, hipStream_t stream, const SelArgs* sel = nullptr,
                   const float* sel_thr = nullptr);
int knn_small_exact_launch(bool ip, const MergeParams& mp, int nq, int npow2, hipStream_t stream, const SelArgs* sel = nullptr);

struct KnnSweepShape {
    int Dp = 0;
    int ng = 0;
    int kp = 0, cap = 0;
    bool small = false;
};
int knn_sweep_shape(int64_t N, int D, int nq, int k, KnnSweepShape* s);
size_t knn_query_tile_bytes(int TQ, int ng);
double knn_sweep_gamma0(int ng);
int64_t knn_residency_groups(const void* kernel, size_t lds, int nqt, int64_t ntiles);
const float* knn_zeros_device();
int knn_check_store(const char* who, const float* d_P, int64_t ldP, int Dp);

struct CallOpts { int arith = -1, ln_fusion = -1, one_launch = -1; };
CallOpts& call_opts();
struct CallScope {
    CallOpts saved;
    CallScope(int arith_opt, int ln_fusion_opt, int one_launch_opt);
    ~CallScope();
    CallScope(const CallScope&) = delete;
    CallScope& operator=(const CallScope&) = delete;
};

int gemm_arith();
void set_gemm_arith(int mode);
inline bool arith_split() { return gemm_arith() != AC_GEMM_F32; }
bool linear_f16x2_takes(int M, int N, int K);
int linear_f16x2(const uint16_t* Ap, const uint16_t* Wp, const float* bias, const float* residual, int64_t ldr, float* C,
                 int64_t ldc, uint16_t* Cp, int M, int N, int K, int act, hipStream_t stream, int64_t w_plane_rows = 0);
int gemm_f32(int transA, int transB, int M, int N, int K, float alpha, const float* A, int64_t lda,
             const float* B, int64_t ldb, float beta, float* C, int64_t ldc, const float* gate,
             int64_t ldg, float gate_scale, hipStream_t stream);

int head_backward_pair(const float* dY, int64_t ldy, const float* Aact, int64_t lda_act, const float* W, int64_t ldw, int B,
                       int Hout, int Hin, float gate_scale, float* gW, float* dA, float* gb_in, hipStream_t stream);

int persistent_mask();
int set_persistent_mask(int m);

size_t head_epoch_ws_bytes(int H1, int H2);
int head_epoch_persistent(const ac_head_dims& d, float* P, float* M, float* V, float* Gout, const float* X, int64_t ldx,
                          const int64_t* y, const float* T, int64_t ldt, int loss_kind, const int64_t* order, int64_t n_total,
                          int batch, float dropout_p, uint64_t seed0, const float* F, const float* Old, float lambda_B,
                          float lam_direct, float max_norm, float lr, float beta1, float beta2, float eps, float wd, int step0,
                          float* out, float* loss_accum, void* ws, hipStream_t stream);

long long head_epoch_launches();
long long bert_small_launches();
size_t bert_small_ws_bytes(int H, int I);
int bert_small_encode(const ac_bert_config& c, const ac_bert_weights& w, const int64_t* ids, const int64_t* type_ids,
                      const int64_t* mask, int b, int S, float* out, int64_t ldo, void* ws, hipStream_t stream);
int bert_small_aborted(int H, int I, const void* ws, hipStream_t stream, int* aborted);

}
```

### adaptive-classifier_amd/csrc/gemm.hip

```cpp
#include "common.h"
#include "gemm_common.h"
#ifndef AC_XCD_REMAP
#define AC_XCD_REMAP 1
#endif

#include <math.h>
#include <stdlib.h>
#include <string.h>

#include <atomic>
#include <type_traits>

namespace {

using namespace acg;

constexpr int BN = kTileN, BK = kStageK;
constexpr int kTileThreads = kBlock4;

__device__ __forceinline__ int tile_slot(int row, int c4) {
    const int rg = row >> 5, i = row & 31, kb = c4 >> 1, h = c4 & 1;
    return ((rg * 4 + kb) << 6) + (((h << 5) + i) ^ c4);
}

template <int EPI, int TM>
__global__ __launch_bounds__(kTileThreads, TM == 2 ? 2 : 3) void gemm_tile_nt(
    const float* __restrict__ A, int64_t lda, const float* __restrict__ W, int64_t ldw,
    float* __restrict__ C, int64_t ldc, int M, int N, int K, Epilogue epi) {
    constexpr int BM = 64 * TM;
    constexpr int A_SLOTS = (BM / 32) * 4 * 64, W_SLOTS = (BN / 32) * 4 * 64;
    constexpr int PA = BM / 32, PW = BN / 32;
    __shared__ __attribute__((aligned(16))) f32x4 lds[2][A_SLOTS + W_SLOTS];

    const int tid = threadIdx.x, lane = tid & 63, wave = tid >> 6;
    const int wm = wave >> 1, wn = wave & 1;
    const int ntn = (N + BN - 1) / BN;
    const int bn = blockIdx.x % ntn, bm = blockIdx.x / ntn;
    const int m0 = bm * BM, n0 = bn * BN;

    const int srow = tid >> 3, sc4 = tid & 7;
    const float* aptr[PA];
    const float* wptr[PW];
    int aslot[PA], wslot[PW];
#pragma unroll
    for (int p = 0; p < PA; ++p) {
        int ra = m0 + srow + 32 * p; if (ra > M - 1) ra = M - 1;
        aptr[p] = A + (int64_t)ra * lda + 4 * sc4;
        aslot[p] = tile_slot(srow + 32 * p, sc4);
    }
#pragma unroll
    for (int p = 0; p < PW; ++p) {
        int rw = n0 + srow + 32 * p; if (rw > N - 1) rw = N - 1;
        wptr[p] = W + (int64_t)rw * ldw + 4 * sc4;
        wslot[p] = A_SLOTS + tile_slot(srow + 32 * p, sc4);
    }

    f32x16 acc[TM][2];
#pragma unroll
    for (int a = 0; a < TM; ++a)
#pragma unroll
        for (int b = 0; b < 2; ++b)
#pragma unroll
            for (int r = 0; r < 16; ++r) acc[a][b][r] = 0.f;

    const int nk = K / BK;
    f32x4 ra[PA], rw[PW];
#pragma unroll
    for (int p = 0; p < PA; ++p) ra[p] = *reinterpret_cast<const f32x4*>(aptr[p]);
#pragma unroll
    for (int p = 0; p < PW; ++p) rw[p] = *reinterpret_cast<const f32x4*>(wptr[p]);
#pragma unroll
    for (int p = 0; p < PA; ++p) lds[0][aslot[p]] = ra[p];
#pragma unroll
    for (int p = 0; p < PW; ++p) lds[0][wslot[p]] = rw[p];
    __syncthreads();

    const int h = lane >> 5;
    for (int kt = 0; kt < nk; ++kt) {
        const int cur = kt & 1;
        const int knext = (kt + 1 < nk) ? (kt + 1) * BK : kt * BK;
#pragma unroll
        for (int p = 0; p < PA; ++p) ra[p] = *reinterpret_cast<const f32x4*>(aptr[p] + knext);
#pragma unroll
        for (int p = 0; p < PW; ++p) rw[p] = *reinterpret_cast<const f32x4*>(wptr[p] + knext);
        __builtin_amdgcn_sched_barrier(0);
        const f32x4* As = lds[cur];
        const f32x4* Ws = lds[cur] + A_SLOTS;
#pragma unroll
        for (int kb = 0; kb < 4; ++kb) {
            const int sl = lane ^ ((kb * 2 + h) & 7);
            f32x4 af[TM], bf[2];
#pragma unroll
            for (int a = 0; a < TM; ++a) af[a] = As[(((TM * wm + a) * 4 + kb) << 6) + sl];
#pragma unroll
            for (int b = 0; b < 2; ++b) bf[b] = Ws[(((2 * wn + b) * 4 + kb) << 6) + sl];
#pragma unroll
            for (int s = 0; s < 4; ++s)
#pragma unroll
                for (int a = 0; a < TM; ++a)
#pragma unroll
                    for (int b = 0; b < 2; ++b)
                        acc[a][b] = __builtin_amdgcn_mfma_f32_32x32x2f32(af[a][s], bf[b][s], acc[a][b], 0, 0, 0);
        }
        __builtin_amdgcn_sched_barrier(0);
#pragma unroll
        for (int p = 0; p < PA; ++p) lds[cur ^ 1][aslot[p]] = ra[p];
#pragma unroll
        for (int p = 0; p < PW; ++p) lds[cur ^ 1][wslot[p]] = rw[p];
        __syncthreads();
    }

    store_tile<EPI, TM>(acc, C, ldc, M, N, m0, n0, wm, wn, lane, epi);
}

using ac::split8;

__device__ __forceinline__ int split_slot(int row, int q) {
    const int rg = row >> 5, i = row & 31, c = q >> 1, kg = q & 1;
    return ((rg * 2 + c) << 6) + (((kg << 5) + i) ^ (q << 2));
}

template <int EPI, int TM>
__global__ __launch_bounds__(kTileThreads, TM == 2 ? 3 : 4) void gemm_split_nt(
    const float* __restrict__ A, int64_t lda, const float* __restrict__ W, int64_t ldw,
    float* __restrict__ C, int64_t ldc, int M, int N, int K, Epilogue epi) {
    constexpr int BM = 64 * TM;
    constexpr int A_SLOTS = (BM / 32) * 2 * 64, W_SLOTS = (BN / 32) * 2 * 64;
    constexpr int PA = BM / 64, PW = BN / 64;
    __shared__ uint4 lds[3][A_SLOTS + W_SLOTS];

    const int tid = threadIdx.x, lane = tid & 63, wave = tid >> 6;
    const int wm = wave >> 1, wn = wave & 1;
    const int ntn = (N + BN - 1) / BN;
    const int bn = blockIdx.x % ntn, bm = blockIdx.x / ntn;
    const int m0 = bm * BM, n0 = bn * BN;

    const int srow = tid >> 2, sq = tid & 3;
    const float* aptr[PA];
    const float* wptr[PW];
    int aslot[PA], wslot[PW];
#pragma unroll
    for (int p = 0; p < PA; ++p) {
        int ra = m0 + srow + 64 * p; if (ra > M - 1) ra = M - 1;
        aptr[p] = A + (int64_t)ra * lda + 8 * sq;
        aslot[p] = split_slot(srow + 64 * p, sq);
    }
#pragma unroll
    for (int p = 0; p < PW; ++p) {
        int rw = n0 + srow + 64 * p; if (rw > N - 1) rw = N - 1;
        wptr[p] = W + (int64_t)rw * ldw + 8 * sq;
        wslot[p] = A_SLOTS + split_slot(srow + 64 * p, sq);
    }

    f32x16 acc[TM][2];
#pragma unroll
    for (int a = 0; a < TM; ++a)
#pragma unroll
        for (int b = 0; b < 2; ++b)
#pragma unroll
            for (int r = 0; r < 16; ++r) acc[a][b][r] = 0.f;

    f32x4 ra[PA][2], rw[PW][2];
    auto load_tile = [&](int k0) {
#pragma unroll
        for (int p = 0; p < PA; ++p) {
            ra[p][0] = *reinterpret_cast<const f32x4*>(aptr[p] + k0);
            ra[p][1] = *reinterpret_cast<const f32x4*>(aptr[p] + k0 + 4);
        }
#pragma unroll
        for (int p = 0; p < PW; ++p) {
            rw[p][0] = *reinterpret_cast<const f32x4*>(wptr[p] + k0);
            rw[p][1] = *reinterpret_cast<const f32x4*>(wptr[p] + k0 + 4);
        }
    };
    auto store_tile_lds = [&]() {
#pragma unroll
        for (int p = 0; p < PA; ++p) {
            uint4 H, Mi, L;
            split8(ra[p][0], ra[p][1], H, Mi, L);
            lds[0][aslot[p]] = H; lds[1][aslot[p]] = Mi; lds[2][aslot[p]] = L;
        }
#pragma unroll
        for (int p = 0; p < PW; ++p) {
            uint4 H, Mi, L;
            split8(rw[p][0], rw[p][1], H, Mi, L);
            lds[0][wslot[p]] = H; lds[1][wslot[p]] = Mi; lds[2][wslot[p]] = L;
        }
    };

    const int nk = K / BK;
    load_tile(0);
    store_tile_lds();
    __syncthreads();

    const int kg = lane >> 5;
    for (int kt = 0; kt < nk; ++kt) {
        load_tile((kt + 1 < nk) ? (kt + 1) * BK : kt * BK);
        __builtin_amdgcn_sched_barrier(0);
#pragma unroll
        for (int c = 0; c < 2; ++c) {
            const int sl = lane ^ ((2 * c + kg) << 2);
            bf16x8_t af[TM][3], bf[2][3];
#pragma unroll
            for (int pl = 0; pl < 3; ++pl) {
#pragma unroll
                for (int a = 0; a < TM; ++a)
                    af[a][pl] = __builtin_bit_cast(bf16x8_t, lds[pl][(((TM * wm + a) * 2 + c) << 6) + sl]);
#pragma unroll
                for (int b = 0; b < 2; ++b)
                    bf[b][pl] = __builtin_bit_cast(bf16x8_t, lds[pl][A_SLOTS + (((2 * wn + b) * 2 + c) << 6) + sl]);
            }
            constexpr int PAIRS[6][2] = {{2, 0}, {0, 2}, {1, 1}, {1, 0}, {0, 1}, {0, 0}};
#pragma unroll
            for (int pr = 0; pr < 6; ++pr)
#pragma unroll
                for (int a = 0; a < TM; ++a)
#pragma unroll
                    for (int b = 0; b < 2; ++b)
                        acc[a][b] = __builtin_amdgcn_mfma_f32_32x32x16_bf16(af[a][PAIRS[pr][0]], bf[b][PAIRS[pr][1]],
                                                                            acc[a][b], 0, 0, 0);
        }
        __builtin_amdgcn_sched_barrier(0);
        __syncthreads();
        store_tile_lds();
        __syncthreads();
    }
    store_tile<EPI, TM>(acc, C, ldc, M, N, m0, n0, wm, wn, lane, epi);
}

__global__ __launch_bounds__(256) void split_planes_kernel(const float* __restrict__ X, int64_t ldx, int64_t rows,
                                                           int K, uint16_t* __restrict__ P) {
    const int nq = K >> 3;
    const int64_t u = (int64_t)blockIdx.x * 256 + threadIdx.x;
    if (u >= rows * nq) return;
    const int64_t row = u / nq;
    const int q = (int)(u - row * nq);
    const float* src = X + row * ldx + 8 * q;
    uint4 H, Mi, L;
    split8(*reinterpret_cast<const f32x4*>(src), *reinterpret_cast<const f32x4*>(src + 4), H, Mi, L);
    const int64_t plane = rows * (int64_t)K;
    uint16_t* dst = P + ((int64_t)q * rows + row) * 8;
    *reinterpret_cast<uint4*>(dst) = H;
    *reinterpret_cast<uint4*>(dst + plane) = Mi;
    *reinterpret_cast<uint4*>(dst + 2 * plane) = L;
}

__global__ __launch_bounds__(256) void split_planes_f16_kernel(const float* __restrict__ X, int64_t ldx, int64_t rows,
                                                               int K, float scale, uint16_t* __restrict__ P) {
    const int nq = K >> 3;
    const int64_t u = (int64_t)blockIdx.x * 256 + threadIdx.x;
    if (u >= rows * nq) return;
    const int64_t row = u / nq;
    const int q = (int)(u - row * nq);
    const float* src = X + row * ldx + 8 * q;
    uint4 H, L;
    ac::split8h(*reinterpret_cast<const f32x4*>(src), *reinterpret_cast<const f32x4*>(src + 4), scale, H, L);
    uint16_t* dst = P + ((int64_t)q * rows + row) * 8;
    *reinterpret_cast<uint4*>(dst) = H;
    *reinterpret_cast<uint4*>(dst + rows * (int64_t)K) = L;
}

constexpr int SBK = 16;

template <int EPI, int TM, bool A_PLANES, bool C_PLANES, int WMW = 2>
__global__ __launch_bounds__(128 * WMW, (WMW == 2 ? 3 : 4)) void gemm_planes_nt(
    const float* __restrict__ A, int64_t lda, const uint16_t* __restrict__ Ap, int64_t a_rows,
    const uint16_t* __restrict__ Wp, int64_t w_rows, float* __restrict__ C, int64_t ldc, int M, int N, int K,
    Epilogue epi) {
    constexpr int BM = 32 * TM * WMW;
    constexpr int RA = BM / 32, RW = BN / 32;
    __shared__ uint4 lds[2][3][(RA + RW) * 64];

    const int tid = threadIdx.x, lane = tid & 63;
    const int wave = __builtin_amdgcn_readfirstlane(tid >> 6);
    const int wm = wave >> 1, wn = wave & 1;
    const int ntn = (N + BN - 1) / BN;
    const int tile = AC_XCD_REMAP ? xcd_tile_id(blockIdx.x, gridDim.x) : (int)blockIdx.x;
    const int bn = tile % ntn, bm = tile / ntn;
    const int m0 = bm * BM, n0 = bn * BN;
    const int i = lane & 31, kg = lane >> 5;

    int wrow = n0 + 32 * (wave & 3) + i; if (wrow > N - 1) wrow = N - 1;
    const uint16_t* wsrc = Wp + ((int64_t)kg * w_rows + wrow) * 8;
    const int64_t w_plane = w_rows * (int64_t)K, w_step = 2 * w_rows * 8;
    int arow = m0 + 32 * wave + i; if (arow > M - 1) arow = M - 1;
    const uint16_t* asrc = A_PLANES ? Ap + ((int64_t)kg * a_rows + arow) * 8 : nullptr;
    const int64_t a_plane = a_rows * (int64_t)K, a_step = 2 * a_rows * 8;
    static_assert(!(WMW == 4 && !A_PLANES), "the 8-wave tile is built for pre-split A only");
    const int frow = tid >> 1, fkg = tid & 1;
    int farow = m0 + frow; if (farow > M - 1) farow = M - 1;
    const float* fsrc = A_PLANES ? nullptr : A + (int64_t)farow * lda + 8 * fkg;
    const int fslot = (frow >> 5) * 64 + fkg * 32 + (frow & 31);
    const bool fact = frow < BM;

    auto stage_glds = [&](int kt, int buf) {
        if (WMW == 2 || wave < RW) {
#pragma unroll
            for (int p = 0; p < 3; ++p)
                __builtin_amdgcn_global_load_lds((glb_void_t*)(wsrc + p * w_plane + kt * w_step),
                                                 (lds_void_t*)&lds[buf][p][(RA + wave) * 64], 16, 0, 0);
        }
        if (A_PLANES && wave < RA) {
#pragma unroll
            for (int p = 0; p < 3; ++p)
                __builtin_amdgcn_global_load_lds((glb_void_t*)(asrc + p * a_plane + kt * a_step),
                                                 (lds_void_t*)&lds[buf][p][wave * 64], 16, 0, 0);
        }
    };
    f32x4 fa0, fa1;
    auto load_a = [&](int kt) {
        fa0 = *reinterpret_cast<const f32x4*>(fsrc + kt * SBK);
        fa1 = *reinterpret_cast<const f32x4*>(fsrc + kt * SBK + 4);
    };
    auto store_a = [&](int buf) {
        uint4 H, Mi, L;
        split8(fa0, fa1, H, Mi, L);
        if (fact) { lds[buf][0][fslot] = H; lds[buf][1][fslot] = Mi; lds[buf][2][fslot] = L; }
    };

    f32x16 acc[TM][2];
#pragma unroll
    for (int a = 0; a < TM; ++a)
#pragma unroll
        for (int b = 0; b < 2; ++b)
#pragma unroll
            for (int r = 0; r < 16; ++r) acc[a][b][r] = 0.f;

    const int nk = K / SBK;
    stage_glds(0, 0);
    if (!A_PLANES) { load_a(0); store_a(0); }
    __syncthreads();

    for (int kt = 0; kt < nk; ++kt) {
        const int cur = kt & 1;
        const int nxt = (kt + 1 < nk) ? kt + 1 : kt;
        stage_glds(nxt, cur ^ 1);
        if (!A_PLANES) load_a(nxt);
        bf16x8_t af[TM][3], bf[2][3];
#pragma unroll
        for (int pl = 0; pl < 3; ++pl) {
#pragma unroll
            for (int a = 0; a < TM; ++a) af[a][pl] = __builtin_bit_cast(bf16x8_t, lds[cur][pl][(TM * wm + a) * 64 + lane]);
#pragma unroll
            for (int b = 0; b < 2; ++b) bf[b][pl] = __builtin_bit_cast(bf16x8_t, lds[cur][pl][(RA + 2 * wn + b) * 64 + lane]);
        }
        constexpr int PAIRS[6][2] = {{2, 0}, {0, 2}, {1, 1}, {1, 0}, {0, 1}, {0, 0}};
#pragma unroll
        for (int pr = 0; pr < 6; ++pr)
#pragma unroll
            for (int a = 0; a < TM; ++a)
#pragma unroll
                for (int b = 0; b < 2; ++b)
                    acc[a][b] = __builtin_amdgcn_mfma_f32_32x32x16_bf16(af[a][PAIRS[pr][0]], bf[b][PAIRS[pr][1]],
                                                                        acc[a][b], 0, 0, 0);
        if (!A_PLANES) store_a(cur ^ 1);
        __syncthreads();
    }
    if (C_PLANES) {
        static_assert(sizeof(lds) >= 2 * WMW * kTrFloats * sizeof(float), "transpose scratch must fit the staging buffers");
        store_tile_planes<EPI, TM>(acc, reinterpret_cast<uint16_t*>(C), M, N, m0, n0, wm, wn, lane, epi,
                                   reinterpret_cast<float*>(&lds[0][0][0]) + wave * kTrFloats);
    } else store_tile<EPI, TM, BM>(acc, C, ldc, M, N, m0, n0, wm, wn, lane, epi);
}

__global__ __launch_bounds__(256, 3) void gemm_planes_splitk_nt(const float* __restrict__ A, int64_t lda,
                                                                const uint16_t* __restrict__ Wp, int64_t w_rows,
                                                                float* __restrict__ part, int M, int N, int K, int ksplit) {
    constexpr int BM = 64, RA = 2, RW = BN / 32;
    __shared__ uint4 lds[2][3][(RA + RW) * 64];
    const int tid = threadIdx.x, lane = tid & 63;
    const int wave = __builtin_amdgcn_readfirstlane(tid >> 6);
    const int wm = wave >> 1, wn = wave & 1;
    const int ntn = (N + BN - 1) / BN;
    const int ntiles = (int)gridDim.x / ksplit, z = (int)blockIdx.x / ntiles, tile = (int)blockIdx.x - z * ntiles;
    const int bn = tile % ntn, bm = tile / ntn;
    const int m0 = bm * BM, n0 = bn * BN;
    const int i = lane & 31, kg = lane >> 5;
    int wrow = n0 + 32 * (wave & 3) + i; if (wrow > N - 1) wrow = N - 1;
    const uint16_t* wsrc = Wp + ((int64_t)kg * w_rows + wrow) * 8;
    const int64_t w_plane = w_rows * (int64_t)K, w_step = 2 * w_rows * 8;
    const int frow = tid >> 1, fkg = tid & 1;
    int farow = m0 + frow; if (farow > M - 1) farow = M - 1;
    const float* fsrc = A + (int64_t)farow * lda + 8 * fkg;
    const int fslot = (frow >> 5) * 64 + fkg * 32 + (frow & 31);
    const bool fact = frow < BM;
    auto stage_glds = [&](int kt, int buf) {
#pragma unroll
        for (int p = 0; p < 3; ++p)
            __builtin_amdgcn_global_load_lds((glb_void_t*)(wsrc + p * w_plane + kt * w_step),
                                             (lds_void_t*)&lds[buf][p][(RA + wave) * 64], 16, 0, 0);
    };
    f32x4 fa0, fa1;
    auto load_a = [&](int kt) {
        fa0 = *reinterpret_cast<const f32x4*>(fsrc + kt * SBK);
        fa1 = *reinterpret_cast<const f32x4*>(fsrc + kt * SBK + 4);
    };
    auto store_a = [&](int buf) {
        uint4 H, Mi, L;
        split8(fa0, fa1, H, Mi, L);
        if (fact) { lds[buf][0][fslot] = H; lds[buf][1][fslot] = Mi; lds[buf][2][fslot] = L; }
    };
    f32x16 acc[1][2];
#pragma unroll
    for (int b = 0; b < 2; ++b)
#pragma unroll
        for (int r = 0; r < 16; ++r) acc[0][b][r] = 0.f;
    const int nks = K / SBK / ksplit, kt_lo = z * nks, kt_hi = kt_lo + nks;
    stage_glds(kt_lo, 0);
    load_a(kt_lo); store_a(0);
    __syncthreads();
    for (int kt = kt_lo; kt < kt_hi; ++kt) {
        const int cur = (kt - kt_lo) & 1;
        const int nxt = (kt + 1 < kt_hi) ? kt + 1 : kt;
        stage_glds(nxt, cur ^ 1);
        load_a(nxt);
        bf16x8_t af[3], bf[2][3];
#pragma unroll
        for (int pl = 0; pl < 3; ++pl) {
            af[pl] = __builtin_bit_cast(bf16x8_t, lds[cur][pl][wm * 64 + lane]);
#pragma unroll
            for (int b = 0; b < 2; ++b) bf[b][pl] = __builtin_bit_cast(bf16x8_t, lds[cur][pl][(RA + 2 * wn + b) * 64 + lane]);
        }
        constexpr int PAIRS[6][2] = {{2, 0}, {0, 2}, {1, 1}, {1, 0}, {0, 1}, {0, 0}};
#pragma unroll
        for (int pr = 0; pr < 6; ++pr)
#pragma unroll
            for (int b = 0; b < 2; ++b)
                acc[0][b] = __builtin_amdgcn_mfma_f32_32x32x16_bf16(af[PAIRS[pr][0]], bf[b][PAIRS[pr][1]], acc[0][b], 0, 0, 0);
        store_a(cur ^ 1);
        __syncthreads();
    }
    Epilogue none{};
    store_tile<EPI_IDENT, 1, BM>(acc, part + (size_t)z * M * N, N, M, N, m0, n0, wm, wn, lane, none);
}

__global__ __launch_bounds__(256) void gemm_splitk_reduce(const float* __restrict__ part, int ksplit, int M, int N, float* __restrict__ C,
                                                          int64_t ldc, Epilogue epi) {
    const int64_t e4 = (int64_t)blockIdx.x * 256 + threadIdx.x;
    const int n4 = N >> 2;
    if (e4 >= (int64_t)M * n4) return;
    const int row = (int)(e4 / n4), col = (int)(e4 % n4) * 4;
    const size_t slice = (size_t)M * N;
    f32x4 s = *reinterpret_cast<const f32x4*>(part + (size_t)row * N + col);
    for (int z = 1; z < ksplit; ++z) {
        const f32x4 t = *reinterpret_cast<const f32x4*>(part + z * slice + (size_t)row * N + col);
        s.x += t.x; s.y += t.y; s.z += t.z; s.w += t.w;
    }
    float* dst = C + (int64_t)row * ldc + col;
    dst[0] = apply_epilogue(epi, s.x, row, col, C, ldc, N);
    dst[1] = apply_epilogue(epi, s.y, row, col + 1, C, ldc, N);
    dst[2] = apply_epilogue(epi, s.z, row, col + 2, C, ldc, N);
    dst[3] = apply_epilogue(epi, s.w, row, col + 3, C, ldc, N);
}

template <bool KMAJ>
__device__ __forceinline__ f32x4 load_frag(const float* base, int64_t ld, int idx, int idx_max, int k0,
                                           int K, bool vec_ok) {
    f32x4 v = {0.f, 0.f, 0.f, 0.f};
    if (KMAJ) {
        const float* p = base + (int64_t)idx * ld + k0;
        if (vec_ok && k0 + 3 < K) {
            v = *reinterpret_cast<const f32x4*>(p);
        } else {
#pragma unroll
            for (int s = 0; s < 4; ++s) if (k0 + s < K) v[s] = p[s];
        }
    } else {
#pragma unroll
        for (int s = 0; s < 4; ++s) if (k0 + s < K) v[s] = base[(int64_t)(k0 + s) * ld + idx];
    }
    (void)idx_max;
    return v;
}

template <bool AK, bool BKM>
__device__ __forceinline__ void gemm_direct_tile(const float* __restrict__ A, int64_t lda, const float* __restrict__ B,
                                                 int64_t ldb, float* __restrict__ C, int64_t ldc, int M, int N, int K,
                                                 const Epilogue& epi, int m0, int n0, float (*red)[16][64],
                                                 float* __restrict__ colsum) {
    const int tid = threadIdx.x, lane = tid & 63, wave = tid >> 6;
    const int i = lane & 31, h = lane >> 5;
    int arow = m0 + i; if (arow > M - 1) arow = M - 1;
    int bcol = n0 + i; if (bcol > N - 1) bcol = N - 1;
    const bool avec = AK && ((lda & 3) == 0) && ((((uintptr_t)A) & 15) == 0);
    const bool bvec = BKM && ((ldb & 3) == 0) && ((((uintptr_t)B) & 15) == 0);

    const int nkb = (K + 7) / 8;
    const int kb_lo = (int)(((int64_t)wave * nkb) / 4), kb_hi = (int)(((int64_t)(wave + 1) * nkb) / 4);
    f32x16 acc;
#pragma unroll
    for (int r = 0; r < 16; ++r) acc[r] = 0.f;
    for (int kb = kb_lo; kb < kb_hi; ++kb) {
        const int k0 = kb * 8 + 4 * h;
        const f32x4 a = load_frag<AK>(A, lda, arow, M, k0, K, avec);
        const f32x4 b = load_frag<BKM>(B, ldb, bcol, N, k0, K, bvec);
#pragma unroll
        for (int s = 0; s < 4; ++s) acc = __builtin_amdgcn_mfma_f32_32x32x2f32(a[s], b[s], acc, 0, 0, 0);
    }
#pragma unroll
    for (int r = 0; r < 16; ++r) red[wave][r][lane] = acc[r];
    __syncthreads();
    float outv[4];
#pragma unroll
    for (int e = 0; e < 4; ++e) {
        const int o = tid + 256 * e;
        const int r = o >> 6, l = o & 63;
        const float v = ((red[0][r][l] + red[1][r][l]) + red[2][r][l]) + red[3][r][l];
        const int64_t row = m0 + acc_row32(r, l);
        const int col = n0 + (l & 31);
        outv[e] = 0.f;
        if (row < M && col < N) { outv[e] = apply_epilogue(epi, v, row, col, C, ldc, N); C[row * ldc + col] = outv[e]; }
    }
    if (colsum) {
        __syncthreads();
#pragma unroll
        for (int e = 0; e < 4; ++e) { const int o = tid + 256 * e; red[0][o >> 6][o & 63] = outv[e]; }
        __syncthreads();
        if (tid < 32 && n0 + tid < N) {
            float sacc = 0.f;
            for (int row = 0; row < 32; ++row) {
                const int hh = (row >> 2) & 1, r = (row & 3) + 4 * (row >> 3);
                sacc += red[0][r][tid + 32 * hh];
            }
            colsum[n0 + tid] = sacc;
        }
    }
}

template <bool AK, bool BKM>
__global__ __launch_bounds__(256) void gemm_direct(const float* __restrict__ A, int64_t lda,
                                                   const float* __restrict__ B, int64_t ldb,
                                                   float* __restrict__ C, int64_t ldc, int M, int N, int K,
                                                   Epilogue epi) {
    __shared__ float red[4][16][64];
    gemm_direct_tile<AK, BKM>(A, lda, B, ldb, C, ldc, M, N, K, epi, blockIdx.y * 32, blockIdx.x * 32, red, nullptr);
}

struct DirectProblem {
    const float* A; int64_t lda; const float* B; int64_t ldb; float* C; int64_t ldc; int M, N, K; Epilogue epi; float* colsum;
};
__global__ __launch_bounds__(256) void gemm_direct_pair(DirectProblem p1, DirectProblem p2, int nblk1) {
    __shared__ float red[4][16][64];
    const int b = blockIdx.x;
    if (b < nblk1) {
        const int tn = (p1.N + 31) / 32;
        gemm_direct_tile<false, false>(p1.A, p1.lda, p1.B, p1.ldb, p1.C, p1.ldc, p1.M, p1.N, p1.K, p1.epi, (b / tn) * 32, (b % tn) * 32,
                                       red, nullptr);
    } else {
        const int t = b - nblk1, tn = (p2.N + 31) / 32;
        gemm_direct_tile<true, false>(p2.A, p2.lda, p2.B, p2.ldb, p2.C, p2.ldc, p2.M, p2.N, p2.K, p2.epi, (t / tn) * 32, (t % tn) * 32,
                                      red, p2.colsum);
    }
}

constexpr int kFtWaves = kBlock8 / 64;
__global__ __launch_bounds__(kFtWaves * 64) void gemm_fewtiles_nt(const float* __restrict__ A, int64_t lda,
                                                                  const float* __restrict__ W, int64_t ldw,
                                                                  float* __restrict__ C, int64_t ldc, int M, int N, int K,
                                                                  Epilogue epi, int tiles_n) {
    __shared__ float red[kFtWaves][16][64];
    const int tid = threadIdx.x, lane = tid & 63, wave = tid >> 6;
    const int m0 = (blockIdx.x / tiles_n) * 32, n0 = (blockIdx.x % tiles_n) * 32;
    const int i = lane & 31, h = lane >> 5;
    int arow = m0 + i; if (arow > M - 1) arow = M - 1;
    int wrow = n0 + i; if (wrow > N - 1) wrow = N - 1;
    const float* ap = A + (int64_t)arow * lda + 8 * h;
    const float* wp = W + (int64_t)wrow * ldw + 8 * h;
    f32x16 acc;
#pragma unroll
    for (int r = 0; r < 16; ++r) acc[r] = 0.f;
    const f32x4 zero = {0.f, 0.f, 0.f, 0.f};
    auto load = [&](int s, f32x4 (&a)[2], f32x4 (&b)[2]) {
        const int k = 16 * (kFtWaves * s + wave);
        if (k + 8 * h < K) {
            a[0] = *reinterpret_cast<const f32x4*>(ap + k); a[1] = *reinterpret_cast<const f32x4*>(ap + k + 4);
            b[0] = *reinterpret_cast<const f32x4*>(wp + k); b[1] = *reinterpret_cast<const f32x4*>(wp + k + 4);
        } else {
            a[0] = a[1] = b[0] = b[1] = zero;
        }
    };
    const int nslots = (K + 16 * kFtWaves - 1) / (16 * kFtWaves);
    f32x4 a0[2], b0[2], a1[2], b1[2];
    load(0, a0, b0);
    for (int s = 0; s < nslots; s += 2) {
        load(s + 1, a1, b1);
#pragma unroll
        for (int e = 0; e < 2; ++e)
#pragma unroll
            for (int c = 0; c < 4; ++c) acc = __builtin_amdgcn_mfma_f32_32x32x2f32(a0[e][c], b0[e][c], acc, 0, 0, 0);
        load(s + 2, a0, b0);
#pragma unroll
        for (int e = 0; e < 2; ++e)
#pragma unroll
            for (int c = 0; c < 4; ++c) acc = __builtin_amdgcn_mfma_f32_32x32x2f32(a1[e][c], b1[e][c], acc, 0, 0, 0);
    }
#pragma unroll
    for (int r = 0; r < 16; ++r) red[wave][r][lane] = acc[r];
    __syncthreads();
#pragma unroll
    for (int e = 0; e < 2; ++e) {
        const int o = tid + 512 * e;
        const int r = o >> 6, l = o & 63;
        const float v = (((red[0][r][l] + red[1][r][l]) + (red[2][r][l] + red[3][r][l])) +
                         ((red[4][r][l] + red[5][r][l]) + (red[6][r][l] + red[7][r][l])));
        const int64_t row = m0 + acc_row32(r, l);
        const int col = n0 + (l & 31);
        if (row < M && col < N) C[row * ldc + col] = apply_epilogue(epi, v, row, col, C, ldc, N);
    }
}

constexpr int kSmWaves = kBlock8 / 64;
template <int J> struct SmGroup { static constexpr int value = (J >= 4) ? 3 : 6; };

template <int J>
__global__ __launch_bounds__(kSmWaves * 64) void gemm_smallm_nt(const float* __restrict__ X, int64_t ldx,
                                                                 const float* __restrict__ W, int64_t ldw,
                                                                 float* __restrict__ C, int64_t ldc, int M, int N, int K,
                                                                 Epilogue epi) {
    __shared__ float red[kSmWaves][J][4][64];
    constexpr int kSmGroup = SmGroup<J>::value;
    const int tid = threadIdx.x, lane = tid & 63, wave = tid >> 6;
    const int n0 = blockIdx.x * 16;
    const int i = lane & 15, h = lane >> 4;
    int wrow = n0 + i; if (wrow > N - 1) wrow = N - 1;
    const float* wp = W + (int64_t)wrow * ldw + 4 * h;
    const float* xp[J];
#pragma unroll
    for (int jj = 0; jj < J; ++jj) {
        int m = 16 * jj + i; if (m > M - 1) m = M - 1;
        xp[jj] = X + (int64_t)m * ldx + 4 * h;
    }
    const int nkb = (K + 15) / 16;
    const int kb_lo = (int)(((int64_t)wave * nkb) / kSmWaves), kb_hi = (int)(((int64_t)(wave + 1) * nkb) / kSmWaves);
    f32x4 acc[J];
#pragma unroll
    for (int jj = 0; jj < J; ++jj) acc[jj] = f32x4{0.f, 0.f, 0.f, 0.f};

    f32x4 wa[2][kSmGroup], xb[2][kSmGroup][J];
#define AC_SM_LOAD(Bf, kb0)                                                              \
    _Pragma("unroll") for (int u = 0; u < kSmGroup; ++u) {                               \
        int col = ((kb0) + u) * 16;                                                      \
        if (col + 4 * h > K - 4) col = K - 4 - 4 * h;                                    \
        wa[Bf][u] = *reinterpret_cast<const f32x4*>(wp + col);                           \
        _Pragma("unroll") for (int jj = 0; jj < J; ++jj)                                 \
            xb[Bf][u][jj] = *reinterpret_cast<const f32x4*>(xp[jj] + col);               \
    }
#define AC_SM_COMPUTE(Bf, kb0)                                                           \
    _Pragma("unroll") for (int u = 0; u < kSmGroup; ++u) {                               \
        const bool ok = ((kb0) + u) < kb_hi && (((kb0) + u) * 16 + 4 * h) < K;           \
        const f32x4 zero = {0.f, 0.f, 0.f, 0.f};                                         \
        const f32x4 a = ok ? wa[Bf][u] : zero;                                           \
        _Pragma("unroll") for (int s = 0; s < 4; ++s)                                    \
            _Pragma("unroll") for (int jj = 0; jj < J; ++jj)                             \
                acc[jj] = __builtin_amdgcn_mfma_f32_16x16x4f32(a[s], xb[Bf][u][jj][s], acc[jj], 0, 0, 0); \
    }
    if (kb_lo < kb_hi) {
        AC_SM_LOAD(0, kb_lo);
        for (int kb = kb_lo; kb < kb_hi; kb += 2 * kSmGroup) {
            AC_SM_LOAD(1, kb + kSmGroup);
            __builtin_amdgcn_sched_barrier(0);
            AC_SM_COMPUTE(0, kb);
            __builtin_amdgcn_sched_barrier(0);
            AC_SM_LOAD(0, kb + 2 * kSmGroup);
            __builtin_amdgcn_sched_barrier(0);
            AC_SM_COMPUTE(1, kb + kSmGroup);
            __builtin_amdgcn_sched_barrier(0);
        }
    }
#undef AC_SM_LOAD
#undef AC_SM_COMPUTE
#pragma unroll
    for (int jj = 0; jj < J; ++jj)
#pragma unroll
        for (int r = 0; r < 4; ++r) red[wave][jj][r][lane] = acc[jj][r];
    __syncthreads();
    for (int o = tid; o < J * 256; o += kSmWaves * 64) {
        const int jj = o >> 8, r = (o >> 6) & 3, l = o & 63;
        float v = 0.f;
#pragma unroll
        for (int w = 0; w < kSmWaves; ++w) v += red[w][jj][r][l];
        const int m = 16 * jj + (l & 15), n = n0 + 4 * (l >> 4) + r;
        if (m < M && n < N) C[(int64_t)m * ldc + n] = apply_epilogue(epi, v, m, n, C, ldc, N);
    }
}

template <int... Vs, class F> static bool pick(int v, F&& f) { return ((v == Vs && (f(std::integral_constant<int, Vs>{}), true)) || ...); }
template <class L> static bool launch_smallm(const GemmPlan& p, L&& go) { return pick<1, 2, 4>(p.J, [&](auto J) { go(gemm_smallm_nt<decltype(J)::value>); }); }
template <bool SPLIT, class L> static bool launch_tiled(const GemmPlan& p, L&& go) {
    return pick<EPI_GENERIC, EPI_BIAS, EPI_BIAS_GELU, EPI_BIAS_RES, EPI_BIAS_RELU>(p.cls, [&](auto E) { pick<1, 2>(p.tm, [&](auto TM) {
        if constexpr (SPLIT) go(gemm_split_nt<decltype(E)::value, decltype(TM)::value>); else go(gemm_tile_nt<decltype(E)::value, decltype(TM)::value>);
    }); });
}
template <bool CP, int WMW, class L> static bool launch_planes(const GemmPlan& p, L&& go) {
    auto one = [&](auto E) {
        if constexpr (WMW == 4) go(gemm_planes_nt<decltype(E)::value, 2, true, CP, 4>);
        else pick<1, 2>(p.tm, [&](auto TM) {
            if (CP || p.a_planes) go(gemm_planes_nt<decltype(E)::value, decltype(TM)::value, true, CP, 2>);
            else if constexpr (!CP) go(gemm_planes_nt<decltype(E)::value, decltype(TM)::value, false, false, 2>);
        });
    };
    if constexpr (CP) return pick<EPI_BIAS, EPI_BIAS_GELU, EPI_GEGLU32>(p.cls, one);
    else if constexpr (WMW == 4) return pick<EPI_BIAS, EPI_BIAS_GELU, EPI_BIAS_RES>(p.cls, one);
    else return pick<EPI_GENERIC, EPI_BIAS, EPI_BIAS_GELU, EPI_BIAS_RES, EPI_BIAS_RELU>(p.cls, one);
}
template <class L> static void launch_direct(bool ak, bool bk, L&& go) { pick<0, 1>(ak, [&](auto AK) { pick<0, 1>(bk, [&](auto BKM) { go(gemm_direct<decltype(AK)::value != 0, decltype(BKM)::value != 0>); }); }); }

static int launch_gemm(bool a_kmaj, bool b_kmaj, const float* A, int64_t lda, const float* B, int64_t ldb, float* C, int64_t ldc, int M, int N, int K,
                       const Epilogue& epi, hipStream_t stream, const uint16_t* Bp = nullptr, int64_t b_rows = 0, const uint16_t* Ap = nullptr,
                       int64_t a_rows = 0, uint16_t* Cp = nullptr) {
    if (M <= 0 || N <= 0) return AC_OK;
    GemmQuery q;
    q.M = M; q.N = N; q.K = K; q.a_kmaj = a_kmaj; q.b_kmaj = b_kmaj;
    q.aligned = ((lda & 3) == 0) && ((ldb & 3) == 0) && ((((uintptr_t)A) & 15) == 0) && ((((uintptr_t)B) & 15) == 0);
    q.a_planes = Ap != nullptr; q.w_planes = Bp != nullptr; q.c_planes = Cp != nullptr;
    q.act = epi.act; q.alpha = epi.alpha; q.beta = epi.beta; q.drop_p = epi.drop_p;
    q.bias = epi.bias != nullptr; q.residual = epi.residual != nullptr; q.mask = epi.mask != nullptr; q.gate = epi.gate != nullptr;
    const GemmPlan p = gemm_plan(q, ac::gemm_env());
    const dim3 grid(p.grid_x, p.grid_y), block(p.block);
    auto nt = [&](auto* kern) { hipLaunchKernelGGL(kern, grid, block, 0, stream, A, lda, B, ldb, C, ldc, M, N, K, epi); };
    auto pl = [&](auto* kern) { hipLaunchKernelGGL(kern, grid, block, 0, stream, A, lda, Ap, a_rows, Bp, b_rows, Cp ? reinterpret_cast<float*>(Cp) : C, ldc, M, N, K, epi); };
    bool built = true;
    switch (p.family) {
        case GEMM_REFUSE: ac::set_error(p.refusal, M, N, K); return AC_EUNSUPPORTED;
        case GEMM_RING: return ac::launch_gemm_pipe(p.cfg, Ap, a_rows, Bp, b_rows, C, ldc, Cp, M, N, K, p.cls, epi, stream);
        case GEMM_SMALLM: built = launch_smallm(p, nt); break;
        case GEMM_FEWTILES: hipLaunchKernelGGL(gemm_fewtiles_nt, grid, block, 0, stream, A, lda, B, ldb, C, ldc, M, N, K, epi, (N + 31) / 32); break;
        case GEMM_PLANES8: built = Cp ? launch_planes<true, 4>(p, pl) : launch_planes<false, 4>(p, pl); break;
        case GEMM_PLANES: built = Cp ? launch_planes<true, 2>(p, pl) : launch_planes<false, 2>(p, pl); break;
        case GEMM_SPLIT: built = launch_tiled<true>(p, nt); break;
        case GEMM_TILE: built = launch_tiled<false>(p, nt); break;
        default: launch_direct(a_kmaj, b_kmaj, nt); break;
    }
    AC_REQUIRE(built, AC_EUNSUPPORTED, "gemm: the plan names a kernel that is not built (family %d, class %d)", p.family, p.cls);
    AC_LAUNCH_CHECK();
    return AC_OK;
}

}

namespace ac {
static std::atomic<int> g_gemm_arith{-1};
int gemm_arith() {
    if (const int o = call_opts().arith; o >= 0) return o;
    int v = g_gemm_arith.load(std::memory_order_relaxed);
    if (v < 0) {
        v = AC_GEMM_BF16X3;
        if (const char* e = getenv("AC_GEMM_ARITH"))
            v = (strcmp(e, "f32") == 0) ? AC_GEMM_F32 : (strcmp(e, "f16x2") == 0) ? AC_GEMM_F16X2 : AC_GEMM_BF16X3;
        g_gemm_arith.store(v, std::memory_order_relaxed);
    }
    return v;
}
void set_gemm_arith(int v) { g_gemm_arith.store(v, std::memory_order_relaxed); }
static std::atomic<int> g_gemm_variant{-1};
int gemm_variant() {
    int v = g_gemm_variant.load(std::memory_order_relaxed);
    if (v < 0) {
        v = 0;
        if (const char* e = getenv("AC_GEMM_VARIANT")) v = atoi(e);
        g_gemm_variant.store(v, std::memory_order_relaxed);
    }
    return v;
}
acg::PipeTable g_pipe_table, g_pipe_table_f16;
acg::GemmEnv gemm_env() {
    acg::GemmEnv e;
    e.cus = dev_info().cus; e.arith = gemm_arith(); e.variant = gemm_variant();
    if (const char* s = getenv("AC_GEMM_TM")) e.force_tm = atoi(s);
    if (const char* s = getenv("AC_GEMM_FEWTILES")) e.fewtiles = atoi(s) != 0;
    static const int tile256_env = getenv("AC_GEMM_TILE256") ? atoi(getenv("AC_GEMM_TILE256")) : -1;
    e.force_tile256 = tile256_env;
    e.table = g_pipe_table; e.table_f16 = g_pipe_table_f16;
    return e;
}
bool linear_takes_planes(int M, int N, int K) { return acg::linear_takes_planes(M, N, K, gemm_env()); }
int linear_f32(const float* A, int64_t lda, const float* W, int64_t ldw, const float* bias,
               const float* residual, int64_t ldr, float* C, int64_t ldc, int M, int N, int K, int act,
               const uint8_t* mask, float mask_scale, hipStream_t stream, float drop_p, uint64_t drop_seed,
               const uint16_t* Wp, const uint16_t* Ap, uint16_t* Cp, int64_t w_plane_rows) {
    Epilogue e;
    e.bias = bias; e.residual = residual; e.ldr = ldr; e.act = act; e.mask = mask; e.mask_scale = mask_scale;
    e.drop_p = mask ? 0.f : drop_p; e.drop_seed = drop_seed;
    return launch_gemm(true, true, A, lda, W, ldw, C, ldc, M, N, K, e, stream, Wp, w_plane_rows > 0 ? w_plane_rows : N, Ap, M, Cp);
}
bool linear_f16x2_takes(int M, int N, int K) { return acg::linear_f16x2_takes(M, N, K, gemm_env()); }
int linear_f16x2(const uint16_t* Ap, const uint16_t* Wp, const float* bias, const float* residual, int64_t ldr, float* C,
                 int64_t ldc, uint16_t* Cp, int M, int N, int K, int act, hipStream_t stream, int64_t w_plane_rows) {
    AC_REQUIRE(Ap && Wp && bias && (C || Cp), AC_EINVAL, "linear_f16x2: null pointer");
    GemmQuery q;
    q.M = M; q.N = N; q.K = K; q.f16 = q.a_planes = q.w_planes = q.bias = true; q.c_planes = Cp != nullptr; q.act = act; q.residual = residual != nullptr;
    const GemmPlan p = gemm_plan(q, gemm_env());
    AC_REQUIRE(p.family == GEMM_RING, AC_EUNSUPPORTED, p.refusal, M, N, K);
    AC_REQUIRE((act == ACT_NONE || (act == ACT_GELU && Cp)) && !(Cp && residual), AC_EUNSUPPORTED,
               "linear_f16x2: act %d / residual / planes-out combination not built", act);
    Epilogue e;
    e.bias = bias; e.residual = residual; e.ldr = ldr; e.act = act;
    return launch_gemm_pipe(p.cfg, Ap, M, Wp, w_plane_rows > 0 ? w_plane_rows : N, C, ldc, Cp, M, N, K, p.cls, e, stream, 1);
}
int linear_f32_splitk(const float* A, int64_t lda, const float* W, int64_t ldw, const float* bias, const float* residual,
                      int64_t ldr, float* C, int64_t ldc, int M, int N, int K, int act, const uint16_t* Wp, float* scratch,
                      size_t scratch_bytes, hipStream_t stream, int64_t w_plane_rows, int* partials_only) {
    if (partials_only) *partials_only = 0;
    const acg::GemmEnv env = gemm_env();
    const int64_t tiles = tiles_of(M, N, 64, BN);
    const bool a_aligned = (lda % 4) == 0 && ((((uintptr_t)A) & 15) == 0);
    const bool direct = W && (int64_t)M * N * K <= kSplitKFewMaxMac &&
                        fewtiles_takes(M, N, K, a_aligned && (ldw % 4) == 0 && ((((uintptr_t)W) & 15) == 0), env);
    const int ksplit = direct ? 1 : splitk_slices(M, N, K, a_aligned, Wp && scratch ? scratch_bytes : 0, env);
    if (ksplit == 1)
        return linear_f32(A, lda, W, ldw, bias, residual, ldr, C, ldc, M, N, K, act, nullptr, 1.f, stream, 0.f, 0, Wp, nullptr, nullptr, w_plane_rows);
    hipLaunchKernelGGL(gemm_planes_splitk_nt, dim3((unsigned)(tiles * ksplit)), dim3(256), 0, stream, A, lda, Wp,
                       w_plane_rows > 0 ? w_plane_rows : (int64_t)N, scratch, M, N, K, ksplit);
    AC_LAUNCH_CHECK();
    if (partials_only) { *partials_only = ksplit; return AC_OK; }
    Epilogue e;
    e.bias = bias; e.residual = residual; e.ldr = ldr; e.act = act;
    const int64_t n4 = (int64_t)M * (N / 4);
    hipLaunchKernelGGL(gemm_splitk_reduce, dim3((unsigned)((n4 + 255) / 256)), dim3(256), 0, stream, scratch, ksplit, M, N, C, ldc, e);
    AC_LAUNCH_CHECK();
    return AC_OK;
}
int head_backward_pair(const float* dY, int64_t ldy, const float* Aact, int64_t lda_act, const float* W, int64_t ldw, int B,
                       int Hout, int Hin, float gate_scale, float* gW, float* dA, float* gb_in, hipStream_t stream) {
    AC_REQUIRE(B >= 1 && B <= 32, AC_EUNSUPPORTED, "head_backward_pair: B=%d (<= 32)", B);
    Epilogue g;
    g.gate = Aact; g.ldg = lda_act; g.gate_scale = gate_scale;
    const DirectProblem p1{dY, ldy, Aact, lda_act, gW, Hin, Hout, Hin, B, Epilogue{}, nullptr};
    const DirectProblem p2{dY, ldy, W, ldw, dA, Hin, B, Hin, Hout, g, gb_in};
    const int nblk1 = ((Hout + 31) / 32) * ((Hin + 31) / 32), nblk2 = (Hin + 31) / 32;
    hipLaunchKernelGGL(gemm_direct_pair, dim3(nblk1 + nblk2), dim3(256), 0, stream, p1, p2, nblk1);
    AC_LAUNCH_CHECK();
    return AC_OK;
}
int gemm_f32(int transA, int transB, int M, int N, int K, float alpha, const float* A, int64_t lda,
             const float* B, int64_t ldb, float beta, float* C, int64_t ldc, const float* gate, int64_t ldg,
             float gate_scale, hipStream_t stream) {
    Epilogue e;
    e.alpha = alpha; e.beta = beta; e.gate = gate; e.ldg = ldg; e.gate_scale = gate_scale;
    return launch_gemm(transA == 0, transB != 0, A, lda, B, ldb, C, ldc, M, N, K, e, stream);
}
}

extern "C" int ac_linear_f32(const float* d_A, int64_t lda, const float* d_W, int64_t ldw,
                             const float* d_bias, const float* d_residual, int64_t ldr, float* d_C,
                             int64_t ldc, int M, int N, int K, int act, ac_stream_t stream) {
    AC_REQUIRE(d_A && d_W && d_C, AC_EINVAL, "linear: null pointer");
    AC_REQUIRE(M >= 0 && N >= 0 && K >= 1 && lda >= K && ldw >= K && ldc >= N, AC_EINVAL,
               "linear: bad shape M=%d N=%d K=%d", M, N, K);
    AC_REQUIRE(act >= 0 && act <= 2, AC_EINVAL, "linear: bad activation %d", act);
    return ac::linear_f32(d_A, lda, d_W, ldw, d_bias, d_residual, ldr, d_C, ldc, M, N, K, act, nullptr, 1.f,
                          (hipStream_t)stream);
}

extern "C" int ac_gemm_f32(int transA, int transB, int M, int N, int K, float alpha, const float* d_A,
                           int64_t lda, const float* d_B, int64_t ldb, float beta, float* d_C,
                           int64_t ldc, ac_stream_t stream) {
    AC_REQUIRE(d_A && d_B && d_C, AC_EINVAL, "gemm: null pointer");
    AC_REQUIRE(M >= 0 && N >= 0 && K >= 1, AC_EINVAL, "gemm: bad shape");
    return ac::gemm_f32(transA, transB, M, N, K, alpha, d_A, lda, d_B, ldb, beta, d_C, ldc, nullptr, 0, 1.f,
                        (hipStream_t)stream);
}

extern "C" int ac_gemm_set_arith(int mode) {
    AC_TEST_HOOK_ONLY("ac_gemm_set_arith");
    AC_REQUIRE(mode == AC_GEMM_F32 || mode == AC_GEMM_BF16X3 || mode == AC_GEMM_F16X2, AC_EINVAL, "gemm arith: unknown mode %d", mode);
    ac::set_gemm_arith(mode);
    return AC_OK;
}
extern "C" int ac_gemm_get_arith(void) { return ac::gemm_arith(); }
extern "C" int ac_gemm_set_variant(int v) {
    AC_TEST_HOOK_ONLY("ac_gemm_set_variant");
    AC_REQUIRE(v == 0 || v == 1 || v >= 1000, AC_EINVAL, "gemm variant: unknown value %d", v);
    ac::g_gemm_variant.store(v, std::memory_order_relaxed);
    return AC_OK;
}

extern "C" int ac_split_bf16x3(const float* d_X, int64_t ldx, int64_t rows, int K, uint16_t* d_planes,
                               ac_stream_t stream) {
    AC_REQUIRE(d_X && d_planes, AC_EINVAL, "split: null pointer");
    AC_REQUIRE(rows >= 0 && K >= 8 && (K % 8) == 0 && ldx >= K && (ldx % 4) == 0 && (((uintptr_t)d_X) & 15) == 0 &&
                   (((uintptr_t)d_planes) & 15) == 0,
               AC_EINVAL, "split: K=%d must be a multiple of 8, rows 16-byte aligned", K);
    if (rows == 0) return AC_OK;
    const int64_t units = rows * (K / 8);
    hipLaunchKernelGGL(split_planes_kernel, dim3((unsigned)((units + 255) / 256)), dim3(256), 0, (hipStream_t)stream,
                       d_X, ldx, rows, K, d_planes);
    AC_LAUNCH_CHECK();
    return AC_OK;
}

extern "C" int ac_split_f16x2(const float* d_X, int64_t ldx, int64_t rows, int K, int scale_log2, uint16_t* d_planes,
                              ac_stream_t stream) {
    AC_REQUIRE(d_X && d_planes, AC_EINVAL, "split: null pointer");
    AC_REQUIRE(rows >= 0 && K >= 8 && (K % 8) == 0 && ldx >= K && (ldx % 4) == 0 && (((uintptr_t)d_X) & 15) == 0 &&
                   (((uintptr_t)d_planes) & 15) == 0 && scale_log2 >= -14 && scale_log2 <= 15,
               AC_EINVAL, "split: K=%d must be a multiple of 8, rows 16-byte aligned, scale 2^%d", K, scale_log2);
    if (rows == 0) return AC_OK;
    const int64_t units = rows * (K / 8);
    hipLaunchKernelGGL(split_planes_f16_kernel, dim3((unsigned)((units + 255) / 256)), dim3(256), 0, (hipStream_t)stream,
                       d_X, ldx, rows, K, ldexpf(1.0f, scale_log2), d_planes);
    AC_LAUNCH_CHECK();
    return AC_OK;
}

extern "C" int ac_linear_f16x2(const uint16_t* d_A_planes, const uint16_t* d_W_planes, const float* d_bias,
                               const float* d_residual, int64_t ldr, float* d_C, int64_t ldc, uint16_t* d_C_planes, int M,
                               int N, int K, int act, ac_stream_t stream) {
    AC_REQUIRE(M >= 1 && N >= 1 && K >= 1 && (d_C_planes || ldc >= N) && (!d_residual || ldr >= N), AC_EINVAL,
               "linear_f16x2: bad shape M=%d N=%d K=%d", M, N, K);
    return ac::linear_f16x2(d_A_planes, d_W_planes, d_bias, d_residual, ldr, d_C, ldc, d_C_planes, M, N, K, act,
                            (hipStream_t)stream);
}

extern "C" int ac_linear_bf16x3(const float* d_A, int64_t lda, const uint16_t* d_A_planes, const float* d_W,
                                int64_t ldw, const uint16_t* d_W_planes, const float* d_bias,
                                const float* d_residual, int64_t ldr, float* d_C, int64_t ldc,
                                uint16_t* d_C_planes, int M, int N, int K, int act, ac_stream_t stream) {
    AC_REQUIRE(d_A && d_W && (d_C || d_C_planes), AC_EINVAL, "linear: null pointer");
    AC_REQUIRE(M >= 0 && N >= 0 && K >= 1 && lda >= K && ldw >= K && (d_C_planes || ldc >= N), AC_EINVAL,
               "linear: bad shape M=%d N=%d K=%d", M, N, K);
    AC_REQUIRE(act >= 0 && act <= 3 && (act != 3 || d_C_planes), AC_EINVAL, "linear: bad activation %d", act);
    AC_REQUIRE(!d_A_planes || d_W_planes, AC_EINVAL, "linear: A planes need W planes");
    return ac::linear_f32(d_A, lda, d_W, ldw, d_bias, d_residual, ldr, d_C, ldc, M, N, K, act, nullptr, 1.f,
                          (hipStream_t)stream, 0.f, 0, d_W_planes,
                          (d_A_planes && ac::linear_takes_planes(M, N, K)) ? d_A_planes : nullptr, d_C_planes);
}

extern "C" int ac_gemm_occupancy(int kernel, int tm, int* blocks_per_cu) {
    AC_REQUIRE(blocks_per_cu && (tm == 1 || tm == 2) && kernel >= 0 && kernel <= 2, AC_EINVAL, "occupancy: bad arguments");
    const void* f = nullptr;
    if (kernel == 0) f = tm == 2 ? (const void*)gemm_tile_nt<EPI_BIAS, 2> : (const void*)gemm_tile_nt<EPI_BIAS, 1>;
    else if (kernel == 1) f = tm == 2 ? (const void*)gemm_split_nt<EPI_BIAS, 2> : (const void*)gemm_split_nt<EPI_BIAS, 1>;
    else f = tm == 2 ? (const void*)gemm_planes_nt<EPI_BIAS, 2, true, false> : (const void*)gemm_planes_nt<EPI_BIAS, 1, true, false>;
    AC_HIP_CHECK(hipOccupancyMaxActiveBlocksPerMultiprocessor(blocks_per_cu, f, kTileThreads, 0));
    return AC_OK;
}
```

### adaptive-classifier_amd/csrc/knn_exact.hip

```cpp
#include "common.h"
#include "knn_stream.h"

#include <float.h>
#include <math.h>

namespace {

using ac::MergeParams;
using ac::SelArgs;
using ac::fkey;
using ac::fkey_inv;
using acknn::f32x4;
using acknn::exact_term;
using acknn::exact_wave;
using acknn::exact_wave_sum;
using acknn::exact_lane;

template <bool IP>
__device__ __forceinline__ void emit_hit(const MergeParams& prm, size_t at, bool real, double key, int64_t id) {
    const double v = IP ? -key : key;
    prm.outD[at] = real ? (float)v : (IP ? -FLT_MAX : FLT_MAX);
    if (prm.outD64) prm.outD64[at] = real ? v : (IP ? -(double)INFINITY : (double)INFINITY);
    prm.outI[at] = real ? id + prm.row_offset : -1;
}

__device__ __forceinline__ bool row_selected(const SelArgs& sa, int64_t row) {
    const int64_t b = sa.sel_bit0 + row;
    return (sa.sel[b >> 6] >> (b & 63)) & 1ull;
}

constexpr int kMergeThreads = 256;

template <typename KeyFn, typename ActiveFn>
__device__ __forceinline__ uint32_t block_radix_select(int n, int want, KeyFn key_of, ActiveFn active,
                                                       int* hist, int* bcast, int* rank_in_ties, int* n_ties) {
    const int tid = threadIdx.x;
    __shared__ int wave_tot[kMergeThreads / 64];
    uint32_t prefix = 0;
    for (int shift = 24; shift >= 0; shift -= 8) {
        hist[tid] = 0;
        __syncthreads();
        const uint32_t himask = shift == 24 ? 0u : (0xffffffffu << (shift + 8));
        int run_bin = -1, run_cnt = 0;
        for (int t = tid; t < n; t += kMergeThreads) {
            if (!active(t)) continue;
            const uint32_t key = key_of(t);
            if ((key & himask) != (prefix & himask)) continue;
            const int bin = (int)((key >> shift) & 255u);
            if (bin == run_bin) { ++run_cnt; continue; }
            if (run_cnt) atomicAdd(&hist[run_bin], run_cnt);
            run_bin = bin; run_cnt = 1;
        }
        if (run_cnt) atomicAdd(&hist[run_bin], run_cnt);
        __syncthreads();
        const int mine_cnt = hist[tid];
        int c = mine_cnt;
#pragma unroll
        for (int o = 1; o < 64; o <<= 1) { const int v = __shfl_up(c, o); if ((tid & 63) >= o) c += v; }
        if ((tid & 63) == 63) wave_tot[tid >> 6] = c;
        __syncthreads();
        for (int w = 0; w < (tid >> 6); ++w) c += wave_tot[w];
        c -= mine_cnt;
        const int mine = hist[tid];
        if (c < want && want <= c + mine) { bcast[0] = tid; bcast[1] = want - c; bcast[2] = mine; }
        __syncthreads();
        prefix |= (uint32_t)bcast[0] << shift;
        want = bcast[1];
        *n_ties = bcast[2];
        __syncthreads();
    }
    *rank_in_ties = want;
    return prefix;
}

template <bool IP, bool SEL = false>
__device__ __forceinline__ void knn_merge_rerank_body(const MergeParams& prm, char* smem, const float* sel_thr = nullptr) {
    const int q = blockIdx.x;
    const int tid = threadIdx.x;
    const int lane = tid & 63;
    const int wave = tid >> 6;
    const int n = prm.cand_cnt ? prm.cand_cap : prm.G * prm.kp;
    const int kp = prm.kp;
    const int segs = prm.cand_cnt ? prm.cand_segs : 1, segcap = n / segs;
    const bool cand = segs > 1;

    uint32_t* keys = reinterpret_cast<uint32_t*>(smem);
    size_t off = ac::align_up((size_t)n * 4, 16);
    int32_t* cid = reinterpret_cast<int32_t*>(smem + off);
    if (cand) off += ac::align_up((size_t)n * 4, 16);
    float* qrow = reinterpret_cast<float*>(smem + off);
    off += ac::align_up((size_t)prm.Dp * 4, 16);
    unsigned long long* sel = reinterpret_cast<unsigned long long*>(smem + off);
    off += (size_t)kp * 8;
    double* exact = reinterpret_cast<double*>(smem + off);
    off += (size_t)kp * 8;
    int* hist = reinterpret_cast<int*>(smem + off);
    off += 256 * 4;
    int* misc = reinterpret_cast<int*>(smem + off);
    double* dmisc = reinterpret_cast<double*>(misc + 8);

    const float* pd = prm.part_d + (size_t)q * n;
    const int32_t* pi = prm.part_i + (size_t)q * n;
    if (tid < 8) misc[tid] = 0;
    for (int c = tid; c < prm.Dp; c += kMergeThreads)
        qrow[c] = c < prm.D ? prm.Q[(size_t)q * prm.ldQ + c] : 0.f;
    int nkeys = n;
    if (cand) {
        __shared__ int seg_off[kMergeThreads + 1];
        __shared__ int scan_tot[kMergeThreads / 64];
        const int raw = tid < segs ? prm.cand_cnt[(size_t)q * segs + tid] : 0;
        const int mine = raw < segcap ? raw : segcap;
        int c = mine;
#pragma unroll
        for (int o = 1; o < 64; o <<= 1) { const int v = __shfl_up(c, o); if (lane >= o) c += v; }
        if (lane == 63) scan_tot[wave] = c;
        __syncthreads();
        if (raw > segcap) misc[6] = 1;
        for (int w = 0; w < wave; ++w) c += scan_tot[w];
        seg_off[tid + 1] = c;
        if (tid == 0) seg_off[0] = 0;
        __syncthreads();
        nkeys = seg_off[kMergeThreads];
        for (int j = tid; j < nkeys; j += kMergeThreads) {
            int lo = 0, hi = segs;
            while (hi - lo > 1) { const int mid = (lo + hi) >> 1; if (seg_off[mid] <= j) lo = mid; else hi = mid; }
            const int t = lo * segcap + (j - seg_off[lo]);
            keys[j] = fkey(pd[t]);
            cid[j] = pi[t];
        }
        if (tid == 0) misc[5] = nkeys;
        if (prm.cand_cnt_clear && tid < segs) prm.cand_cnt_clear[(size_t)q * segs + tid] = 0;
    } else {
        const int raw = prm.cand_cnt ? prm.cand_cnt[q] : n;
        const int nfill = raw < n ? raw : n;
        if (tid == 0 && raw > n) misc[6] = 1;
        int nreal_local = 0;
#pragma unroll 8
        for (int t = tid; t < n; t += kMergeThreads) {
            const bool real = t < nfill && pi[t] >= 0;
            keys[t] = real ? fkey(pd[t]) : 0xffffffffu;
            nreal_local += real ? 1 : 0;
        }
        __syncthreads();
        atomicAdd(&misc[5], nreal_local);
        if (prm.cand_cnt_clear && tid == 0) prm.cand_cnt_clear[q] = 0;
    }
    __syncthreads();
    const bool overflow = misc[6] != 0;
    const int nreal = misc[5];
    const int nsel = nreal < kp ? nreal : kp;
    auto id_of = [&](int t) -> int32_t { return cand ? cid[t] : pi[t]; };

    uint32_t T = 0xffffffffu;
    int32_t tie_id_max = 0x7fffffff;
    if (nsel > 0) {
        int r = 0, c_eq = 0;
        T = block_radix_select(nkeys, nsel, [&](int t) { return keys[t]; },
                               [&](int t) { return keys[t] != 0xffffffffu; }, hist, misc, &r, &c_eq);
        if (c_eq != r) {
            int r2 = 0, c2 = 0;
            tie_id_max = (int32_t)block_radix_select(
                nkeys, r, [&](int t) { return (uint32_t)id_of(t); },
                [&](int t) { return keys[t] != 0xffffffffu && keys[t] == T; }, hist, misc, &r2, &c2);
        }
    }
    if (prm.thr_only) {
        if (tid == 0 && prm.thr_out && nreal >= kp && nsel > 0) {
            const float t = nextafterf(fkey_inv(T), INFINITY);
            if (t < prm.thr_out[q]) prm.thr_out[q] = t;
        }
        return;
    }
    for (int t = tid; t < nkeys; t += kMergeThreads) {
        const uint32_t key0 = keys[t];
        const int32_t id = key0 != 0xffffffffu ? id_of(t) : -1;
        if (nsel > 0 && id >= 0) {
            const uint32_t key = key0;
            if (key < T || (key == T && id <= tie_id_max)) {
                const int s = atomicAdd(&misc[4], 1);
                if (s < kp) sel[s] = ((unsigned long long)key << 32) | (uint32_t)id;
            }
        }
    }
    __syncthreads();
    const int ns = misc[4] < kp ? misc[4] : kp;
    const unsigned long long T64 = (unsigned long long)T << 32;

    const int nc4 = prm.Dp >> 2;
    constexpr int RU = 4;
    for (int s0 = wave * RU; s0 < ns; s0 += (kMergeThreads / 64) * RU) {
        const f32x4* prow[RU];
#pragma unroll
        for (int u = 0; u < RU; ++u) {
            const int s = s0 + u < ns ? s0 + u : s0;
            const int32_t id = (int32_t)(uint32_t)(sel[s] & 0xffffffffull);
            const int64_t prow_i = prm.run_stride ? (int64_t)(id >> 3) * prm.run_stride + (id & 7) : (int64_t)id;
            prow[u] = reinterpret_cast<const f32x4*>(prm.P + (size_t)prow_i * prm.ldP);
        }
        double acc[RU][4];
#pragma unroll
        for (int u = 0; u < RU; ++u) { acc[u][0] = 0; acc[u][1] = 0; acc[u][2] = 0; acc[u][3] = 0; }
#pragma unroll 2
        for (int c4 = lane; c4 < nc4; c4 += 64) {
            f32x4 p[RU];
#pragma unroll
            for (int u = 0; u < RU; ++u) p[u] = prow[u][c4];
            const f32x4 qq = *reinterpret_cast<const f32x4*>(qrow + 4 * c4);
#pragma unroll
            for (int u = 0; u < RU; ++u) {
                acc[u][0] = exact_term<IP>(p[u].x, qq.x, acc[u][0]); acc[u][1] = exact_term<IP>(p[u].y, qq.y, acc[u][1]);
                acc[u][2] = exact_term<IP>(p[u].z, qq.z, acc[u][2]); acc[u][3] = exact_term<IP>(p[u].w, qq.w, acc[u][3]);
            }
        }
#pragma unroll
        for (int u = 0; u < RU; ++u) {
            const double a = exact_wave_sum(acc[u][0], acc[u][1], acc[u][2], acc[u][3]);
            if (lane == 0 && s0 + u < ns) exact[s0 + u] = IP ? -a : a;
        }
    }
    if (wave == 0) {
        double a = 0;
        for (int c = lane; c < prm.Dp; c += 64) a = fma((double)qrow[c], (double)qrow[c], a);
#pragma unroll
        for (int o = 1; o < 64; o <<= 1) a += __shfl_xor(a, o);
        if (lane == 0) { dmisc[0] = a; dmisc[1] = INFINITY; }
    }
    __syncthreads();

    const int kout = prm.k;
    for (int t = tid; t < ns; t += kMergeThreads) {
        const double dt = exact[t];
        const uint32_t it = (uint32_t)(sel[t] & 0xffffffffull);
        int rank = 0;
        for (int s = 0; s < ns; ++s) {
            const double ds = exact[s];
            const uint32_t is = (uint32_t)(sel[s] & 0xffffffffull);
            rank += (ds < dt || (ds == dt && is < it)) ? 1 : 0;
        }
        if (rank < kout) emit_hit<IP>(prm, (size_t)q * kout + rank, true, dt, (int64_t)it);
        if (rank == kout - 1) dmisc[1] = dt;
    }
    for (int t = ns + tid; t < kout; t += kMergeThreads)
        emit_hit<IP>(prm, (size_t)q * kout + t, false, 0.0, -1);
    __syncthreads();

    float mx_all = 0.f;
    for (int b = tid; b < prm.nblk; b += kMergeThreads) mx_all = fmaxf(mx_all, prm.part_maxnorm[b]);
#pragma unroll
    for (int o = 1; o < 64; o <<= 1) mx_all = fmaxf(mx_all, __shfl_xor(mx_all, o));
    if (lane == 0) hist[wave] = (int)__float_as_uint(mx_all);
    __syncthreads();
    if (tid == 0 && prm.thr_out) {
        float mx = 0.f;
        for (int w = 0; w < kMergeThreads / 64; ++w) mx = fmaxf(mx, __uint_as_float((uint32_t)hist[w]));
        const double qn2 = dmisc[0], tau = dmisc[1];
        const double pn = sqrt((double)mx * 1.001), qn = sqrt(qn2);
        const double E = prm.gamma * (pn + qn) * (pn + qn) + 1e-30;
        const double bound = IP ? 2.0 * tau + E : tau - qn2 + E;
        float t = (float)bound;
        if ((double)t < bound) t = nextafterf(t, INFINITY);
        if (isfinite(tau) && ns >= kout && t < prm.thr_out[q]) prm.thr_out[q] = t;
    }
    if (tid == 0) {
        int ok = 1;
        if (prm.N > (int64_t)kp) {
            float mx = 0.f;
            for (int w = 0; w < kMergeThreads / 64; ++w) mx = fmaxf(mx, __uint_as_float((uint32_t)hist[w]));
            const double qn2 = dmisc[0];
            const double pn = sqrt((double)mx * 1.001), qn = sqrt(qn2);
            const double E = prm.gamma * (pn + qn) * (pn + qn) + 1e-30;
            const double a_last = (double)fkey_inv((uint32_t)(T64 >> 32));
            const double kth = dmisc[1];
            if constexpr (IP) {
                ok = (ns >= kout) && (kth < 0.5 * (a_last - E)) && !overflow;
            } else {
                ok = (ns >= kout) && (kth < a_last - E + qn2) && !overflow;
            }
            if (prm.cand_cnt && nreal < kp) ok = 0;
            if constexpr (SEL) { if (!prm.cand_cnt && nreal < kp && !overflow) ok = 1; }
            if constexpr (SEL) { if (sel_thr && prm.cand_cnt && nreal <= kp && !overflow && sel_thr[q] == INFINITY) ok = 1; }
        }
        int flag = 0;
        if (!ok) {
            const int slot = atomicAdd(prm.fb_slotctr, 1);
            flag = slot < prm.fb_F ? slot + 1 : -1;
            if (prm.stats) atomicAdd(&prm.stats[0], 1);
        }
        prm.flags[q] = flag;
    }
}
template <bool IP>
__global__ __launch_bounds__(kMergeThreads) void knn_merge_rerank(MergeParams prm) {
    extern __shared__ __attribute__((aligned(16))) char smem[];
    knn_merge_rerank_body<IP>(prm, smem);
}
template <bool IP>
__global__ __launch_bounds__(kMergeThreads) void knn_merge_rerank_sel(MergeParams prm) {
    extern __shared__ __attribute__((aligned(16))) char smem[];
    knn_merge_rerank_body<IP, true>(prm, smem);
}
template <bool IP>
__global__ __launch_bounds__(kMergeThreads) void knn_merge_rerank_selc(MergeParams prm, const float* sel_thr) {
    extern __shared__ __attribute__((aligned(16))) char smem[];
    knn_merge_rerank_body<IP, true>(prm, smem, sel_thr);
}

constexpr int kFbThreads = 512;
constexpr int kFbWaves = kFbThreads / 64;
constexpr int kFbCap = 1024;
constexpr int kFbRound = 32;

constexpr int kFbQueryGroups = 8, kFbMergeGroups = 32;
template <bool IP, bool SEL = false>
__device__ __forceinline__ void knn_exact_fallback_query(const MergeParams& prm, const int q, const int slab, char* smem, const SelArgs* sa = nullptr) {
    const int flag = prm.flags[q];
    if (flag == 0 || (flag < 0 && slab != 0)) return;
    const bool direct = flag < 0;
    const int64_t row_lo = direct ? 0 : (prm.N * slab) / prm.fb_S;
    const int64_t row_hi = direct ? prm.N : (prm.N * (slab + 1)) / prm.fb_S;
    const int tid = threadIdx.x, lane = tid & 63, wave = tid >> 6;
    double* ld = reinterpret_cast<double*>(smem);
    int32_t* li = reinterpret_cast<int32_t*>(ld + kFbCap);
    float* qrow = reinterpret_cast<float*>(li + kFbCap);
    int* misc = reinterpret_cast<int*>(qrow + ac::align_up((size_t)prm.Dp, 4));
    double* tau_d = reinterpret_cast<double*>(misc + 4);
    int32_t* tau_i = reinterpret_cast<int32_t*>(tau_d + 1);

    for (int c = tid; c < prm.Dp; c += kFbThreads)
        qrow[c] = c < prm.D ? prm.Q[(size_t)q * prm.ldQ + c] : 0.f;
    if (tid == 0) { misc[0] = 0; *tau_d = INFINITY; *tau_i = 0x7fffffff; }
    __syncthreads();
    const int nc4 = prm.Dp >> 2;
    const int k = prm.k;

    auto prune = [&]() {
        const int n = misc[0] < kFbCap ? misc[0] : kFbCap;
        double myd[2]; int32_t myi[2]; int rank[2];
#pragma unroll
        for (int e = 0; e < 2; ++e) {
            const int s = tid + kFbThreads * e;
            myd[e] = s < n ? ld[s] : INFINITY;
            myi[e] = s < n ? li[s] : 0x7fffffff;
            rank[e] = 0;
        }
        for (int s = 0; s < n; ++s) {
            const double d = ld[s]; const int32_t i = li[s];
#pragma unroll
            for (int e = 0; e < 2; ++e) rank[e] += (d < myd[e] || (d == myd[e] && i < myi[e])) ? 1 : 0;
        }
        __syncthreads();
#pragma unroll
        for (int e = 0; e < 2; ++e) {
            const int s = tid + kFbThreads * e;
            if (s < n && rank[e] < k) {
                ld[rank[e]] = myd[e]; li[rank[e]] = myi[e];
                if (rank[e] == k - 1) { *tau_d = myd[e]; *tau_i = myi[e]; }
            }
        }
        if (tid == 0) misc[0] = n < k ? n : k;
        __syncthreads();
    };

    for (int64_t base = row_lo; base < row_hi; base += (int64_t)kFbWaves * kFbRound) {
        const double td = *tau_d; const int32_t ti = *tau_i;
        for (int m = 0; m < kFbRound; ++m) {
            const int64_t row = base + (int64_t)m * kFbWaves + wave;
            if (row >= row_hi) break;
            if constexpr (SEL) { if (!row_selected(*sa, row)) continue; }
            double a = exact_wave<IP>(prm.P + (size_t)row * prm.ldP, nc4, lane,
                                      [&](int c4) { return *reinterpret_cast<const f32x4*>(qrow + 4 * c4); });
            if (IP) a = -a;
            if (lane == 0 && (a < td || (a == td && (int32_t)row < ti))) {
                const int s = atomicAdd(&misc[0], 1);
                if (s < kFbCap) { ld[s] = a; li[s] = (int32_t)row; }
            }
        }
        __syncthreads();
        const int c_now = misc[0];
        __syncthreads();
        if (c_now > kFbCap - kFbWaves * kFbRound) prune();
    }
    prune();
    const int n = misc[0];
    if (direct) {
        for (int t = tid; t < k; t += kFbThreads) emit_hit<IP>(prm, (size_t)q * k + t, t < n, ld[t], (int64_t)li[t]);
    } else {
        const size_t base = ((size_t)(flag - 1) * prm.fb_S + slab) * k;
        for (int t = tid; t < k; t += kFbThreads) {
            prm.fb_d[base + t] = t < n ? ld[t] : INFINITY;
            prm.fb_i[base + t] = t < n ? li[t] : 0x7fffffff;
        }
    }
}
template <bool IP>
__global__ __launch_bounds__(kFbThreads) void knn_exact_fallback(MergeParams prm, int nq) {
    extern __shared__ __attribute__((aligned(16))) char smem[];
    for (int q = blockIdx.y; q < nq; q += gridDim.y) {
        knn_exact_fallback_query<IP>(prm, q, blockIdx.x, smem);
        __syncthreads();
    }
}
template <bool IP>
__global__ __launch_bounds__(kFbThreads) void knn_exact_fallback_sel(MergeParams prm, int nq, SelArgs sa) {
    extern __shared__ __attribute__((aligned(16))) char smem[];
    for (int q = blockIdx.y; q < nq; q += gridDim.y) {
        knn_exact_fallback_query<IP, true>(prm, q, blockIdx.x, smem, &sa);
        __syncthreads();
    }
}

template <bool IP>
__device__ __forceinline__ void knn_exact_fb_merge_query(const MergeParams& prm, const int npow2, const int q, char* smem) {
    const int tid = threadIdx.x;
    const int flag = prm.flags[q];
    if (flag <= 0) return;
    double* ds = reinterpret_cast<double*>(smem);
    int32_t* is = reinterpret_cast<int32_t*>(ds + npow2);
    const int n = prm.fb_S * prm.k;
    const size_t base = (size_t)(flag - 1) * n;
    for (int t = tid; t < npow2; t += 256) {
        ds[t] = t < n ? prm.fb_d[base + t] : INFINITY;
        is[t] = t < n ? prm.fb_i[base + t] : 0x7fffffff;
    }
    __syncthreads();
    for (int size = 2; size <= npow2; size <<= 1)
        for (int stride = size >> 1; stride > 0; stride >>= 1) {
            for (int t = tid; t < (npow2 >> 1); t += 256) {
                const int lo = 2 * t - (t & (stride - 1));
                const int hi = lo + stride;
                const bool asc = (lo & size) == 0;
                const double dl = ds[lo], dh = ds[hi];
                const int32_t il = is[lo], ih = is[hi];
                const bool gt = dl > dh || (dl == dh && il > ih);
                if (gt == asc) { ds[lo] = dh; ds[hi] = dl; is[lo] = ih; is[hi] = il; }
            }
            __syncthreads();
        }
    for (int t = tid; t < prm.k; t += 256) emit_hit<IP>(prm, (size_t)q * prm.k + t, is[t] != 0x7fffffff, ds[t], (int64_t)is[t]);
}
template <bool IP>
__global__ __launch_bounds__(256) void knn_exact_fb_merge(MergeParams prm, int npow2, int nq) {
    extern __shared__ __attribute__((aligned(16))) char smem[];
    for (int q = blockIdx.x; q < nq; q += gridDim.x) {
        knn_exact_fb_merge_query<IP>(prm, npow2, q, smem);
        __syncthreads();
    }
}

template <typename DT, bool DESC = false>
__global__ __launch_bounds__(256) void topk_merge_kernel(const DT* Din, const int64_t* Iin,
                                                         int shards, int nq, int k, float* outD,
                                                         int64_t* outI) {
    extern __shared__ __attribute__((aligned(16))) char smem[];
    const int q = blockIdx.x, tid = threadIdx.x;
    const int n = shards * k;
    int64_t* ids = reinterpret_cast<int64_t*>(smem);
    DT* ds = reinterpret_cast<DT*>(ids + n);
    for (int t = tid; t < n; t += 256) {
        const int s = t / k, e = t - s * k;
        ids[t] = Iin[((size_t)s * nq + q) * k + e];
        ds[t] = Din[((size_t)s * nq + q) * k + e];
    }
    for (int t = tid; t < k; t += 256) { outD[(size_t)q * k + t] = DESC ? -FLT_MAX : FLT_MAX; outI[(size_t)q * k + t] = -1; }
    __syncthreads();
    for (int t = tid; t < n; t += 256) {
        const int64_t it = ids[t];
        if (it < 0) continue;
        const DT dt = ds[t];
        int rank = 0;
        for (int s = 0; s < n; ++s) {
            const int64_t is = ids[s];
            if (is < 0) continue;
            const DT d = ds[s];
            rank += ((DESC ? d > dt : d < dt) || (d == dt && (is < it || (is == it && s < t)))) ? 1 : 0;
        }
        if (rank < k) { outD[(size_t)q * k + rank] = (float)dt; outI[(size_t)q * k + rank] = it; }
    }
}

__global__ __launch_bounds__(64) void proto_scores_kernel(const float* D, const int64_t* I, int nq,
                                                          int k, float* out) {
    const int q = blockIdx.x, lane = threadIdx.x;
    float mx = -INFINITY;
    for (int e = lane; e < k; e += 64)
        if (I[(size_t)q * k + e] >= 0) mx = fmaxf(mx, expf(-D[(size_t)q * k + e]));
#pragma unroll
    for (int o = 1; o < 64; o <<= 1) mx = fmaxf(mx, __shfl_xor(mx, o));
    float sum = 0.f;
    for (int e = lane; e < k; e += 64)
        if (I[(size_t)q * k + e] >= 0) sum += expf(expf(-D[(size_t)q * k + e]) - mx);
#pragma unroll
    for (int o = 1; o < 64; o <<= 1) sum += __shfl_xor(sum, o);
    for (int e = lane; e < k; e += 64) {
        const bool v = I[(size_t)q * k + e] >= 0;
        out[(size_t)q * k + e] = v ? expf(expf(-D[(size_t)q * k + e]) - mx) / sum : 0.f;
    }
}

__global__ __launch_bounds__(256) void rows_to_class_kernel(const int64_t* I, int64_t n, const int32_t* row_class,
                                                            int64_t nrows, const int64_t* class_lut, int nlut,
                                                            int64_t* out) {
    const int64_t t = (int64_t)blockIdx.x * 256 + threadIdx.x;
    if (t >= n) return;
    const int64_t id = I[t];
    int64_t c = -1;
    if (id >= 0 && id < nrows) {
        c = row_class ? (int64_t)row_class[id] : id;
        if (class_lut) c = (c >= 0 && c < nlut) ? class_lut[c] : -1;
    }
    out[t] = c;
}

constexpr int kSmallThreads = 256;

template <bool IP, int MODE = 0>
__device__ __forceinline__ void knn_small_exact_body(const MergeParams& prm, int npow2, char* smem, const SelArgs* sa = nullptr) {
    double* ds = reinterpret_cast<double*>(smem);
    int32_t* is = reinterpret_cast<int32_t*>(ds + npow2);
    const int q = blockIdx.x, tid = threadIdx.x;
    const float* qv = prm.Q + (size_t)q * prm.ldQ;
    for (int r = tid; r < npow2; r += kSmallThreads) {
        double a = INFINITY;
        int64_t row = r;
        bool have = r < prm.N;
        if constexpr (MODE == 1) have = have && row_selected(*sa, r);
        if constexpr (MODE == 2) {
            have = r < sa->n_ids;
            if (have) { row = sa->ids[r]; have = row >= 0 && row < prm.N; }
        }
        if (MODE == 0 ? r < prm.N : have) {
            const float* p = prm.P + (size_t)(MODE == 2 ? row : (int64_t)r) * prm.ldP;
            a = exact_lane<IP>(p, qv, prm.D);
            if (IP) a = -a;
        }
        ds[r] = a;
        if constexpr (MODE == 0) is[r] = r < prm.N ? r : 0x7fffffff;
        else is[r] = have ? (int32_t)row : 0x7fffffff;
    }
    __syncthreads();
    for (int size = 2; size <= npow2; size <<= 1)
        for (int stride = size >> 1; stride > 0; stride >>= 1) {
            for (int t = tid; t < (npow2 >> 1); t += kSmallThreads) {
                const int lo = 2 * t - (t & (stride - 1));
                const int hi = lo + stride;
                const bool asc = (lo & size) == 0;
                const double dl = ds[lo], dh = ds[hi];
                const int32_t il = is[lo], ih = is[hi];
                const bool gt = dl > dh || (dl == dh && il > ih);
                if (gt == asc) { ds[lo] = dh; ds[hi] = dl; is[lo] = ih; is[hi] = il; }
            }
            __syncthreads();
        }
    for (int t = tid; t < prm.k; t += kSmallThreads) {
        bool real = t < prm.N;
        if constexpr (MODE != 0) real = t < npow2 && is[t < npow2 ? t : 0] != 0x7fffffff;
        emit_hit<IP>(prm, (size_t)q * prm.k + t, real, real ? ds[t] : 0.0, real ? (int64_t)is[t] : -1);
    }
}
template <bool IP>
__global__ __launch_bounds__(kSmallThreads) void knn_small_exact(MergeParams prm, int npow2) {
    extern __shared__ __attribute__((aligned(16))) char smem[];
    knn_small_exact_body<IP>(prm, npow2, smem);
}
template <bool IP>
__global__ __launch_bounds__(kSmallThreads) void knn_small_exact_sel(MergeParams prm, int npow2, SelArgs sa) {
    extern __shared__ __attribute__((aligned(16))) char smem[];
    knn_small_exact_body<IP, 1>(prm, npow2, smem, &sa);
}
template <bool IP>
__global__ __launch_bounds__(kSmallThreads) void knn_small_exact_ids(MergeParams prm, int npow2, SelArgs sa) {
    extern __shared__ __attribute__((aligned(16))) char smem[];
    knn_small_exact_body<IP, 2>(prm, npow2, smem, &sa);
}

}

namespace ac {

void knn_exact_plan(ExactPlan* ep, WsTake& take, int k, int kp, int Dp, size_t list_bytes, int fb_F) {
    ep->fb_S = 4096 / next_pow2(k);
    if (ep->fb_S > 64) ep->fb_S = 64;
    if (ep->fb_S < 1) ep->fb_S = 1;
    ep->fb_F = fb_F;
    const size_t fb_entries = (size_t)fb_F * ep->fb_S * k;
    ep->off_fb_d = take(fb_entries * 8);
    ep->off_fb_i = take(fb_entries * 4);
    ep->off_fb_ctr = take(256);
    ep->merge_lds = list_bytes + align_up((size_t)Dp * 4, 16) + (size_t)kp * 16 + 256 * 4 + 64;
    ep->fb_lds = (size_t)kFbCap * 12 + align_up((size_t)Dp, 4) * 4 + 64;
}

MergeParams knn_merge_params(const float* P, int64_t N, int64_t ldP, const float* Q, int64_t ldQ, int D, int Dp, int k, int kp,
                             int64_t row_offset, float* outD, double* outD64, int64_t* outI, int32_t* stats, char* ws,
                             const ExactPlan& ep) {
    MergeParams mp;
    mp.P = P; mp.N = N; mp.ldP = ldP; mp.Q = Q; mp.ldQ = ldQ; mp.D = D; mp.Dp = Dp; mp.k = k; mp.kp = kp;
    mp.row_offset = row_offset;
    mp.outD = outD; mp.outD64 = outD64; mp.outI = outI;
    mp.flags = (int32_t*)(ws + ep.off_flags);
    mp.stats = stats;
    mp.fb_S = ep.fb_S; mp.fb_F = ep.fb_F;
    mp.fb_d = (double*)(ws + ep.off_fb_d); mp.fb_i = (int32_t*)(ws + ep.off_fb_i); mp.fb_slotctr = (int32_t*)(ws + ep.off_fb_ctr);
    return mp;
}

int knn_merge_launch(bool ip, const MergeParams& mp, int nq, size_t attr_lds, size_t lds, hipStream_t stream, const SelArgs* sel,
                     const float* sel_thr) {
    if (sel && sel_thr) {
        void (*cfn)(MergeParams, const float*) = ip ? knn_merge_rerank_selc<true> : knn_merge_rerank_selc<false>;
        if (attr_lds) AC_HIP_CHECK(hipFuncSetAttribute((const void*)cfn, hipFuncAttributeMaxDynamicSharedMemorySize, (int)attr_lds));
        hipLaunchKernelGGL(cfn, dim3(nq), dim3(kMergeThreads), lds, stream, mp, sel_thr);
        AC_LAUNCH_CHECK();
        return AC_OK;
    }
    void (*fn)(MergeParams) = ip ? knn_merge_rerank<true> : knn_merge_rerank<false>;
    if (sel) fn = ip ? knn_merge_rerank_sel<true> : knn_merge_rerank_sel<false>;
    if (attr_lds) AC_HIP_CHECK(hipFuncSetAttribute((const void*)fn, hipFuncAttributeMaxDynamicSharedMemorySize, (int)attr_lds));
    hipLaunchKernelGGL(fn, dim3(nq), dim3(kMergeThreads), lds, stream, mp);
    AC_LAUNCH_CHECK();
    return AC_OK;
}

int knn_exact_tail(bool ip, const MergeParams& mp, const ExactPlan& ep, int nq, size_t merge_lds, hipStream_t stream, const SelArgs* sel,
                   const float* sel_thr) {
    const int rc = knn_merge_launch(ip, mp, nq, ep.merge_lds, merge_lds, stream, sel, sel_thr);
    if (rc != AC_OK || mp.N == 0) return rc;
    const dim3 fb_grid(ep.fb_S, nq < kFbQueryGroups ? nq : kFbQueryGroups);
    if (sel) {
        void (*fbs_fn)(MergeParams, int, SelArgs) = ip ? knn_exact_fallback_sel<true> : knn_exact_fallback_sel<false>;
        (void)hipFuncSetAttribute((const void*)fbs_fn, hipFuncAttributeMaxDynamicSharedMemorySize, (int)ep.fb_lds);
        hipLaunchKernelGGL(fbs_fn, fb_grid, dim3(kFbThreads), ep.fb_lds, stream, mp, nq, *sel);
    } else {
    void (*fb_fn)(MergeParams, int) = ip ? knn_exact_fallback<true> : knn_exact_fallback<false>;
    (void)hipFuncSetAttribute((const void*)fb_fn, hipFuncAttributeMaxDynamicSharedMemorySize, (int)ep.fb_lds);
    hipLaunchKernelGGL(fb_fn, fb_grid, dim3(kFbThreads), ep.fb_lds, stream, mp, nq);
    }
    AC_LAUNCH_CHECK();
    const int np2 = next_pow2(ep.fb_S * mp.k > 2 ? ep.fb_S * mp.k : 2);
    void (*fbm_fn)(MergeParams, int, int) = ip ? knn_exact_fb_merge<true> : knn_exact_fb_merge<false>;
    (void)hipFuncSetAttribute((const void*)fbm_fn, hipFuncAttributeMaxDynamicSharedMemorySize, np2 * 12);
    hipLaunchKernelGGL(fbm_fn, dim3(nq < kFbMergeGroups ? nq : kFbMergeGroups), dim3(256), (size_t)np2 * 12, stream, mp, np2, nq);
    AC_LAUNCH_CHECK();
    return AC_OK;
}

int knn_small_exact_launch(bool ip, const MergeParams& mp, int nq, int npow2, hipStream_t stream, const SelArgs* sel) {
    const size_t lds = (size_t)npow2 * 12;
    if (sel) {
        void (*sfn)(MergeParams, int, SelArgs);
        if (sel->by_ids) sfn = ip ? knn_small_exact_ids<true> : knn_small_exact_ids<false>;
        else sfn = ip ? knn_small_exact_sel<true> : knn_small_exact_sel<false>;
        (void)hipFuncSetAttribute((const void*)sfn, hipFuncAttributeMaxDynamicSharedMemorySize, (int)lds);
        hipLaunchKernelGGL(sfn, dim3(nq), dim3(kSmallThreads), lds, stream, mp, npow2, *sel);
        AC_LAUNCH_CHECK();
        return AC_OK;
    }
    void (*fn)(MergeParams, int) = ip ? knn_small_exact<true> : knn_small_exact<false>;
    (void)hipFuncSetAttribute((const void*)fn, hipFuncAttributeMaxDynamicSharedMemorySize, (int)lds);
    hipLaunchKernelGGL(fn, dim3(nq), dim3(kSmallThreads), lds, stream, mp, npow2);
    AC_LAUNCH_CHECK();
    return AC_OK;
}

}

template <typename DT, bool DESC>
static int topk_merge(const char* name, size_t lds_limit, const DT* d_D_in, const int64_t* d_I_in, int shards, int nq, int k,
                      float* d_outD, int64_t* d_outI, ac_stream_t stream_) {
    AC_REQUIRE(shards >= 1 && nq >= 0 && k >= 1, AC_EINVAL, "%s: bad shape", name);
    AC_REQUIRE(d_D_in && d_I_in && d_outD && d_outI, AC_EINVAL, "%s: null pointer", name);
    if (nq == 0) return AC_OK;
    const size_t lds = (size_t)shards * k * (8 + sizeof(DT));
    AC_REQUIRE(lds <= lds_limit, AC_EUNSUPPORTED, "%s: shards*k=%d too large", name, shards * k);
    (void)hipFuncSetAttribute((const void*)topk_merge_kernel<DT, DESC>, hipFuncAttributeMaxDynamicSharedMemorySize, (int)lds);
    hipLaunchKernelGGL((topk_merge_kernel<DT, DESC>), dim3(nq), dim3(256), lds, (hipStream_t)stream_, d_D_in, d_I_in, shards, nq, k,
                       d_outD, d_outI);
    AC_LAUNCH_CHECK();
    return AC_OK;
}

extern "C" int ac_topk_merge(const float* d_D_in, const int64_t* d_I_in, int shards, int nq, int k,
                             float* d_outD, int64_t* d_outI, ac_stream_t stream) {
    return topk_merge<float, false>("topk_merge", 96 * 1024, d_D_in, d_I_in, shards, nq, k, d_outD, d_outI, stream);
}

extern "C" int ac_topk_merge_f64(const double* d_D_in, const int64_t* d_I_in, int shards, int nq, int k,
                                 float* d_outD, int64_t* d_outI, ac_stream_t stream) {
    return topk_merge<double, false>("topk_merge_f64", 128 * 1024, d_D_in, d_I_in, shards, nq, k, d_outD, d_outI, stream);
}

extern "C" int ac_topk_merge_ip_f64(const double* d_D_in, const int64_t* d_I_in, int shards, int nq, int k,
                                    float* d_outD, int64_t* d_outI, ac_stream_t stream) {
    return topk_merge<double, true>("topk_merge_ip_f64", 128 * 1024, d_D_in, d_I_in, shards, nq, k, d_outD, d_outI, stream);
}

extern "C" int ac_rows_to_class(const int64_t* d_I, int64_t n, const int32_t* d_row_class, int64_t nrows,
                                const int64_t* d_class_lut, int nlut, int64_t* d_out, ac_stream_t stream_) {
    AC_REQUIRE(d_I && d_out && n >= 0 && nrows >= 0, AC_EINVAL, "rows_to_class: bad arguments");
    if (n == 0) return AC_OK;
    hipLaunchKernelGGL(rows_to_class_kernel, dim3((unsigned)((n + 255) / 256)), dim3(256), 0, (hipStream_t)stream_,
                       d_I, n, d_row_class, nrows, d_class_lut, nlut, d_out);
    AC_LAUNCH_CHECK();
    return AC_OK;
}

extern "C" int ac_proto_scores(const float* d_D, const int64_t* d_I, int nq, int k, float* d_out,
                               ac_stream_t stream_) {
    hipStream_t stream = (hipStream_t)stream_;
    AC_REQUIRE(nq >= 0 && k >= 1 && d_D && d_I && d_out, AC_EINVAL, "proto_scores: bad arguments");
    if (nq == 0) return AC_OK;
    hipLaunchKernelGGL(proto_scores_kernel, dim3(nq), dim3(64), 0, stream, d_D, d_I, nq, k, d_out);
    AC_LAUNCH_CHECK();
    return AC_OK;
}
```

Baseline: 54910.

## Fuse BERT tail row gathers into few-tile GEMM and merge kNN fallback stages

In the last BERT layer, the CLS-row gather kernel is replaced by row-index arrays passed to a new few-tile GEMM variant. That kernel reads A rows and residual rows indirectly, so the separate gather launch disappears. The split-K LayerNorm/normalize kernel gets a templated specialization for H<=768 that uses 3 vectors per lane and 16 partials per load group, cutting register use and wasted lanes. The kNN exact fallback merge now runs inside the last-arriving slab block, tracked by an atomic arrival counter, and the fallback kernel exits early when no query needs it. Together these remove extra launches, at the cost of atomic synchronisation that relies on correct memory scopes and counter reset.

```diff
diff --git a/adaptive-classifier_amd/csrc/bert.hip b/adaptive-classifier_amd/csrc/bert.hip
--- a/adaptive-classifier_amd/csrc/bert.hip
+++ b/adaptive-classifier_amd/csrc/bert.hip
@@ -110,6 +110,7 @@
     else hipLaunchKernelGGL(ln_kernel_t<false>, dim3(blocks), dim3(256), 0, stream, in, T, H, g, b, eps, out, planes, in_stride);
 }
 
+template <int NVT, int ZG>
 __global__ __launch_bounds__(256) void splitk_ln_normalize_kernel(const float* __restrict__ part, int ksplit, int M, int H,
                                                                   const float* __restrict__ bias, const float* __restrict__ residual,
                                                                   int64_t ldr, const float* __restrict__ g, const float* __restrict__ be,
@@ -119,30 +120,30 @@
     if (i >= M) return;
     const int nv = H >> 2;
     const size_t slice = (size_t)M * H;
-    f32x4 x[kMaxVec];
+    f32x4 x[NVT];
     const f32x4 zero4 = {0.f, 0.f, 0.f, 0.f};
 #pragma unroll
-    for (int e = 0; e < kMaxVec; ++e) x[e] = zero4;
-    for (int z0 = 0; z0 < ksplit; z0 += 4) {
-        f32x4 t[4][kMaxVec];
-#pragma unroll
-        for (int u = 0; u < 4; ++u)
-#pragma unroll
-            for (int e = 0; e < kMaxVec; ++e) {
+    for (int e = 0; e < NVT; ++e) x[e] = zero4;
+    for (int z0 = 0; z0 < ksplit; z0 += ZG) {
+        f32x4 t[ZG][NVT];
+#pragma unroll
+        for (int u = 0; u < ZG; ++u)
+#pragma unroll
+            for (int e = 0; e < NVT; ++e) {
                 const int c4 = lane + 64 * e;
                 t[u][e] = (z0 + u < ksplit && c4 < nv) ? *reinterpret_cast<const f32x4*>(part + (size_t)(z0 + u) * slice + (size_t)i * H + 4 * c4) : zero4;
             }
 #pragma unroll
-        for (int u = 0; u < 4; ++u)
+        for (int u = 0; u < ZG; ++u)
             if (z0 + u < ksplit) {
 #pragma unroll
-                for (int e = 0; e < kMaxVec; ++e)
+                for (int e = 0; e < NVT; ++e)
                     if (z0 + u == 0) x[e] = t[u][e];
                     else { x[e].x += t[u][e].x; x[e].y += t[u][e].y; x[e].z += t[u][e].z; x[e].w += t[u][e].w; }
             }
     }
 #pragma unroll
-    for (int e = 0; e < kMaxVec; ++e) {
+    for (int e = 0; e < NVT; ++e) {
         const int c4 = lane + 64 * e;
         if (c4 < nv) {
             const f32x4 s = x[e];
@@ -153,12 +154,12 @@
     }
     float s = 0.f;
 #pragma unroll
-    for (int e = 0; e < kMaxVec; ++e)
+    for (int e = 0; e < NVT; ++e)
         if (lane + 64 * e < nv) s += (x[e].x + x[e].y) + (x[e].z + x[e].w);
     const float mean = wave_sum(s) / (float)H;
     float q = 0.f;
 #pragma unroll
-    for (int e = 0; e < kMaxVec; ++e)
+    for (int e = 0; e < NVT; ++e)
         if (lane + 64 * e < nv) {
             const float d0 = x[e].x - mean, d1 = x[e].y - mean, d2 = x[e].z - mean, d3 = x[e].w - mean;
             q += (d0 * d0 + d1 * d1) + (d2 * d2 + d3 * d3);
@@ -167,7 +168,7 @@
     const float rstd = 1.0f / sqrtf(var + eps);
     float ss = 0.f;
 #pragma unroll
-    for (int e = 0; e < kMaxVec; ++e) {
+    for (int e = 0; e < NVT; ++e) {
         const int c4 = lane + 64 * e;
         if (c4 < nv) {
             const f32x4 gg = *reinterpret_cast<const f32x4*>(g + 4 * c4);
@@ -183,7 +184,7 @@
     }
     const float nrm = fmaxf(sqrtf(wave_sum(ss)), 1e-12f);
 #pragma unroll
-    for (int e = 0; e < kMaxVec; ++e) {
+    for (int e = 0; e < NVT; ++e) {
         const int c4 = lane + 64 * e;
         if (c4 < nv) {
             f32x4 y = x[e];
@@ -710,10 +711,13 @@
 
 namespace {
 
-static bool tail_fused() {
+static int tail_level() {
     const char* e = getenv("AC_BERT_TAIL_FUSED");
-    return !(e && atoi(e) == 0);
-}
+    if (!e) return 2;
+    if (strcmp(e, "end") == 0) return 1;
+    return atoi(e) == 0 ? 0 : 2;
+}
+static bool tail_fused() { return tail_level() >= 1; }
 inline bool pools_mean(int pool_opt) { return pool_opt == AC_POOL_MEAN; }
 inline int token_layers(const ac_bert_config& c) { return pools_mean(c.pool_opt) ? c.layers : c.layers - 1; }
 struct EncodePlan { bool wplanes, pl, f16; };
@@ -810,7 +814,17 @@
         const float* resid = x;
         int64_t ldres = last ? (int64_t)S * H : H;
         const bool q_cls_only = last && T >= 4 * b;
-        if (last && cu) {
+        const bool tail = last && tail_level() == 2;
+        const bool w_al = (((uintptr_t)w->qkv_w[l]) & 15) == 0 && (((uintptr_t)w->ao_w[l]) & 15) == 0;
+        const bool rows_in_place = tail && cu && q_cls_only && (((uintptr_t)x) & 15) == 0 && (((uintptr_t)ctx) & 15) == 0 && w_al &&
+                                   ac::linear_rows_applies(b, H, H, true, 0, false, qkv_w3 != nullptr) &&
+                                   ac::linear_rows_applies(b, H, H, true, 0, true, ao_w3 != nullptr);
+        ac::LinearRows q_rows, ao_rows;
+        if (last && cu && rows_in_place) {
+            q_rows.a_rows = cu;
+            ao_rows.res_rows = cu;
+            ldres = H;
+        } else if (last && cu) {
             hipLaunchKernelGGL(gather_rows_kernel, dim3((b + 3) / 4), dim3(256), 0, stream, x, cu, b, H, ffn);
             AC_LAUNCH_CHECK();
             resid = ffn;
@@ -834,7 +848,7 @@
                                       stream, 0.f, 0, qkv_w3 ? qkv_w3 + (int64_t)H * 8 : nullptr, pl ? xp : nullptr, nullptr, 3 * H);
             if (rc) return rc;
             rc = ac::linear_f32_splitk(resid, ldres, w->qkv_w[l], H, w->qkv_b[l], nullptr, 0, y, H, b, H, H, 0, qkv_w3, ctx,
-                                       (size_t)T * H * sizeof(float), stream, 3 * H);
+                                       (size_t)T * H * sizeof(float), stream, 3 * H, nullptr, rows_in_place ? &q_rows : nullptr);
         } else {
             rc = f16 ? ac::linear_f16x2(xp, w->qkv_wh[l], w->qkv_b[l], nullptr, 0, qkv, 3 * H, nullptr, T, 3 * H, H, 0, stream)
                      : ac::linear_f32(x, H, w->qkv_w[l], H, w->qkv_b[l], nullptr, 0, qkv, 3 * H, T, 3 * H, H, 0, nullptr, 1.f,
@@ -887,7 +901,7 @@
             if (rc) return rc;
         } else {
             rc = last ? ac::linear_f32_splitk(ctx, H, w->ao_w[l], H, w->ao_b[l], resid, ldres, y, H, Ml, H, H, 0, ao_w3, qkv,
-                                              (size_t)T * 3 * H * sizeof(float), stream)
+                                              (size_t)T * 3 * H * sizeof(float), stream, 0, nullptr, rows_in_place ? &ao_rows : nullptr)
                       : (f16 ? ac::linear_f16x2(ctxp, w->ao_wh[l], w->ao_b[l], resid, ldres, y, H, nullptr, Ml, H, H, 0, stream)
                              : ac::linear_f32(ctx, H, w->ao_w[l], H, w->ao_b[l], resid, ldres, y, H, Ml, H, H, 0, nullptr, 1.f, stream,
                                               0.f, 0, ao_w3, lp ? ctxp : nullptr));
@@ -914,8 +928,12 @@
                                        (size_t)T * 3 * H * sizeof(float), stream, 0, &ks);
             if (rc) return rc;
             if (ks > 0) {
-                hipLaunchKernelGGL(splitk_ln_normalize_kernel, dim3(b), dim3(64), 0, stream, qkv, ks, b, H, w->ff2_b[l], x1, (int64_t)H,
-                                   w->ln2_g[l], w->ln2_b[l], c.ln_eps, d_out, ldo);
+                if (H <= 768 && tail_level() == 2)
+                    hipLaunchKernelGGL((splitk_ln_normalize_kernel<3, 16>), dim3(b), dim3(64), 0, stream, qkv, ks, b, H, w->ff2_b[l], x1, (int64_t)H,
+                                       w->ln2_g[l], w->ln2_b[l], c.ln_eps, d_out, ldo);
+                else
+                    hipLaunchKernelGGL((splitk_ln_normalize_kernel<kMaxVec, 4>), dim3(b), dim3(64), 0, stream, qkv, ks, b, H, w->ff2_b[l], x1, (int64_t)H,
+                                       w->ln2_g[l], w->ln2_b[l], c.ln_eps, d_out, ldo);
                 AC_LAUNCH_CHECK();
                 return AC_OK;
             }
diff --git a/adaptive-classifier_amd/csrc/common.h b/adaptive-classifier_amd/csrc/common.h
--- a/adaptive-classifier_amd/csrc/common.h
+++ b/adaptive-classifier_amd/csrc/common.h
@@ -66,9 +66,15 @@
                const uint8_t* mask, float mask_scale, hipStream_t stream, float drop_p = 0.f,
                uint64_t drop_seed = 0, const uint16_t* W_planes = nullptr, const uint16_t* A_planes = nullptr,
                uint16_t* C_planes = nullptr, int64_t w_plane_rows = 0);
+struct LinearRows {
+    const int32_t* a_rows = nullptr;
+    const int32_t* res_rows = nullptr;
+};
 int linear_f32_splitk(const float* A, int64_t lda, const float* W, int64_t ldw, const float* bias, const float* residual,
                       int64_t ldr, float* C, int64_t ldc, int M, int N, int K, int act, const uint16_t* W_planes, float* scratch,
-                      size_t scratch_bytes, hipStream_t stream, int64_t w_plane_rows = 0, int* partials_only = nullptr);
+                      size_t scratch_bytes, hipStream_t stream, int64_t w_plane_rows = 0, int* partials_only = nullptr,
+                      const LinearRows* rows = nullptr);
+bool linear_rows_applies(int M, int N, int K, bool aligned, int act, bool residual, bool w_planes);
 bool pipe_ln_applies(int M, int N, int K);
 size_t pipe_ln_part_bytes(int M, int N);
 int pipe_ln_panels(int M);
@@ -270,6 +276,7 @@
     double* fb_d = nullptr;
     int32_t* fb_i = nullptr;
     int32_t* fb_slotctr = nullptr;
+    int32_t* fb_arrive = nullptr;
     int thr_only = 0;
 };
 struct SelArgs {
@@ -285,7 +292,7 @@
     size_t operator()(size_t n) { const size_t o = off; off += align_up(n, 256); return o; }
 };
 struct ExactPlan {
-    int fb_S = 1, fb_F = 1;
+    int fb_S = 1, fb_F = 1, fb_np2 = 2;
     size_t off_flags = 0, off_fb_d = 0, off_fb_i = 0, off_fb_ctr = 0, merge_lds = 0, fb_lds = 0;
 };
 void knn_exact_plan(ExactPlan* ep, WsTake& take, int k, int kp, int Dp, size_t list_bytes, int fb_F);
diff --git a/adaptive-classifier_amd/csrc/gemm.hip b/adaptive-classifier_amd/csrc/gemm.hip
--- a/adaptive-classifier_amd/csrc/gemm.hip
+++ b/adaptive-classifier_amd/csrc/gemm.hip
@@ -554,16 +554,17 @@
 }
 
 constexpr int kFtWaves = kBlock8 / 64;
-__global__ __launch_bounds__(kFtWaves * 64) void gemm_fewtiles_nt(const float* __restrict__ A, int64_t lda,
-                                                                  const float* __restrict__ W, int64_t ldw,
-                                                                  float* __restrict__ C, int64_t ldc, int M, int N, int K,
-                                                                  Epilogue epi, int tiles_n) {
-    __shared__ float red[kFtWaves][16][64];
+template <bool ROWS>
+__device__ __forceinline__ void fewtiles_tile(float (&red)[kFtWaves][16][64], const float* __restrict__ A, int64_t lda,
+                                              const float* __restrict__ W, int64_t ldw, float* __restrict__ C, int64_t ldc, int M, int N,
+                                              int K, const Epilogue& epi, int tiles_n, const int32_t* __restrict__ a_rows,
+                                              const int32_t* __restrict__ res_rows) {
     const int tid = threadIdx.x, lane = tid & 63, wave = tid >> 6;
     const int m0 = (blockIdx.x / tiles_n) * 32, n0 = (blockIdx.x % tiles_n) * 32;
     const int i = lane & 31, h = lane >> 5;
     int arow = m0 + i; if (arow > M - 1) arow = M - 1;
     int wrow = n0 + i; if (wrow > N - 1) wrow = N - 1;
+    if constexpr (ROWS) { if (a_rows) arow = a_rows[arow]; }
     const float* ap = A + (int64_t)arow * lda + 8 * h;
     const float* wp = W + (int64_t)wrow * ldw + 8 * h;
     f32x16 acc;
@@ -605,8 +606,35 @@
                          ((red[4][r][l] + red[5][r][l]) + (red[6][r][l] + red[7][r][l])));
         const int64_t row = m0 + acc_row32(r, l);
         const int col = n0 + (l & 31);
-        if (row < M && col < N) C[row * ldc + col] = apply_epilogue(epi, v, row, col, C, ldc, N);
-    }
+        if constexpr (ROWS) {
+            if (row < M && col < N) {
+                if (res_rows) {
+                    Epilogue e = epi;
+                    e.residual = nullptr;
+                    C[row * ldc + col] = apply_epilogue(e, v, row, col, C, ldc, N) + epi.residual[(int64_t)res_rows[row] * epi.ldr + col];
+                } else {
+                    C[row * ldc + col] = apply_epilogue(epi, v, row, col, C, ldc, N);
+                }
+            }
+        } else {
+            if (row < M && col < N) C[row * ldc + col] = apply_epilogue(epi, v, row, col, C, ldc, N);
+        }
+    }
+}
+__global__ __launch_bounds__(kFtWaves * 64) void gemm_fewtiles_nt(const float* __restrict__ A, int64_t lda,
+                                                                  const float* __restrict__ W, int64_t ldw,
+                                                                  float* __restrict__ C, int64_t ldc, int M, int N, int K,
+                                                                  Epilogue epi, int tiles_n) {
+    __shared__ float red[kFtWaves][16][64];
+    fewtiles_tile<false>(red, A, lda, W, ldw, C, ldc, M, N, K, epi, tiles_n, nullptr, nullptr);
+}
+__global__ __launch_bounds__(kFtWaves * 64) void gemm_fewtiles_rows_nt(const float* __restrict__ A, int64_t lda,
+                                                                       const float* __restrict__ W, int64_t ldw,
+                                                                       float* __restrict__ C, int64_t ldc, int M, int N, int K,
+                                                                       Epilogue epi, int tiles_n, const int32_t* __restrict__ a_rows,
+                                                                       const int32_t* __restrict__ res_rows) {
+    __shared__ float red[kFtWaves][16][64];
+    fewtiles_tile<true>(red, A, lda, W, ldw, C, ldc, M, N, K, epi, tiles_n, a_rows, res_rows);
 }
 
 constexpr int kSmWaves = kBlock8 / 64;
@@ -797,15 +825,38 @@
     e.bias = bias; e.residual = residual; e.ldr = ldr; e.act = act;
     return launch_gemm_pipe(p.cfg, Ap, M, Wp, w_plane_rows > 0 ? w_plane_rows : N, C, ldc, Cp, M, N, K, p.cls, e, stream, 1);
 }
+static GemmPlan fewtiles_plan(int M, int N, int K, bool aligned, int act, bool bias, bool residual, bool w_planes) {
+    GemmQuery q;
+    q.M = M; q.N = N; q.K = K; q.a_kmaj = q.b_kmaj = true; q.aligned = aligned; q.w_planes = w_planes;
+    q.act = act; q.bias = bias; q.residual = residual;
+    return gemm_plan(q, gemm_env());
+}
+bool linear_rows_applies(int M, int N, int K, bool aligned, int act, bool residual, bool w_planes) {
+    const acg::GemmEnv env = gemm_env();
+    return (int64_t)M * N * K <= kSplitKFewMaxMac && fewtiles_takes(M, N, K, aligned, env) &&
+           fewtiles_plan(M, N, K, aligned, act, true, residual, w_planes).family == GEMM_FEWTILES;
+}
 int linear_f32_splitk(const float* A, int64_t lda, const float* W, int64_t ldw, const float* bias, const float* residual,
                       int64_t ldr, float* C, int64_t ldc, int M, int N, int K, int act, const uint16_t* Wp, float* scratch,
-                      size_t scratch_bytes, hipStream_t stream, int64_t w_plane_rows, int* partials_only) {
+                      size_t scratch_bytes, hipStream_t stream, int64_t w_plane_rows, int* partials_only, const LinearRows* rows) {
     if (partials_only) *partials_only = 0;
     const acg::GemmEnv env = gemm_env();
     const int64_t tiles = tiles_of(M, N, 64, BN);
     const bool a_aligned = (lda % 4) == 0 && ((((uintptr_t)A) & 15) == 0);
     const bool direct = W && (int64_t)M * N * K <= kSplitKFewMaxMac &&
                         fewtiles_takes(M, N, K, a_aligned && (ldw % 4) == 0 && ((((uintptr_t)W) & 15) == 0), env);
+    if (rows && (rows->a_rows || rows->res_rows)) {
+        const bool aligned = a_aligned && (ldw % 4) == 0 && ((((uintptr_t)W) & 15) == 0);
+        const GemmPlan p = fewtiles_plan(M, N, K, aligned, act, bias != nullptr, residual != nullptr, Wp != nullptr);
+        AC_REQUIRE(direct && p.family == GEMM_FEWTILES && (!rows->res_rows || residual), AC_EUNSUPPORTED,
+                   "linear_f32_splitk: row-indexed operands need the few-tile kernel (M=%d N=%d K=%d)", M, N, K);
+        Epilogue e;
+        e.bias = bias; e.residual = residual; e.ldr = ldr; e.act = act;
+        hipLaunchKernelGGL(gemm_fewtiles_rows_nt, dim3(p.grid_x, p.grid_y), dim3(p.block), 0, stream, A, lda, W, ldw, C, ldc, M, N, K, e,
+                           (N + 31) / 32, rows->a_rows, rows->res_rows);
+        AC_LAUNCH_CHECK();
+        return AC_OK;
+    }
     const int ksplit = direct ? 1 : splitk_slices(M, N, K, a_aligned, Wp && scratch ? scratch_bytes : 0, env);
     if (ksplit == 1)
         return linear_f32(A, lda, W, ldw, bias, residual, ldr, C, ldc, M, N, K, act, nullptr, 1.f, stream, 0.f, 0, Wp, nullptr, nullptr, w_plane_rows);
diff --git a/adaptive-classifier_amd/csrc/knn_exact.hip b/adaptive-classifier_amd/csrc/knn_exact.hip
--- a/adaptive-classifier_amd/csrc/knn_exact.hip
+++ b/adaptive-classifier_amd/csrc/knn_exact.hip
@@ -306,13 +306,23 @@
 }
 
 constexpr int kFbThreads = 512;
+__device__ __forceinline__ void fb_st_sc1(double* p, double v) {
+    __hip_atomic_store(reinterpret_cast<unsigned long long*>(p), (unsigned long long)__double_as_longlong(v), __ATOMIC_RELAXED, __HIP_MEMORY_SCOPE_AGENT);
+}
+__device__ __forceinline__ void fb_st_sc1(int32_t* p, int32_t v) { __hip_atomic_store(p, v, __ATOMIC_RELAXED, __HIP_MEMORY_SCOPE_AGENT); }
+__device__ __forceinline__ double fb_ld_sc1(const double* p) {
+    return __longlong_as_double((long long)__hip_atomic_load(reinterpret_cast<const unsigned long long*>(p), __ATOMIC_RELAXED, __HIP_MEMORY_SCOPE_AGENT));
+}
+__device__ __forceinline__ int32_t fb_ld_sc1(const int32_t* p) { return __hip_atomic_load(p, __ATOMIC_RELAXED, __HIP_MEMORY_SCOPE_AGENT); }
 constexpr int kFbWaves = kFbThreads / 64;
 constexpr int kFbCap = 1024;
 constexpr int kFbRound = 32;
 
-constexpr int kFbQueryGroups = 8, kFbMergeGroups = 32;
+constexpr int kFbQueryGroups = 8;
+template <bool IP>
+__device__ __forceinline__ void knn_exact_fb_merge_slot(const MergeParams& prm, int npow2, int q, int slot, char* smem);
 template <bool IP, bool SEL = false>
-__device__ __forceinline__ void knn_exact_fallback_query(const MergeParams& prm, const int q, const int slab, char* smem, const SelArgs* sa = nullptr) {
+__device__ __forceinline__ void knn_exact_fallback_query(const MergeParams& prm, const int q, const int slab, const int npow2, char* smem, const SelArgs* sa = nullptr) {
     const int flag = prm.flags[q];
     if (flag == 0 || (flag < 0 && slab != 0)) return;
     const bool direct = flag < 0;
@@ -387,45 +397,53 @@
     } else {
         const size_t base = ((size_t)(flag - 1) * prm.fb_S + slab) * k;
         for (int t = tid; t < k; t += kFbThreads) {
-            prm.fb_d[base + t] = t < n ? ld[t] : INFINITY;
-            prm.fb_i[base + t] = t < n ? li[t] : 0x7fffffff;
-        }
-    }
-}
-template <bool IP>
-__global__ __launch_bounds__(kFbThreads) void knn_exact_fallback(MergeParams prm, int nq) {
-    extern __shared__ __attribute__((aligned(16))) char smem[];
+            fb_st_sc1(prm.fb_d + base + t, t < n ? ld[t] : INFINITY);
+            fb_st_sc1(prm.fb_i + base + t, t < n ? li[t] : 0x7fffffff);
+        }
+        asm volatile("s_waitcnt vmcnt(0)" ::: "memory");
+        __syncthreads();
+        const int sh = 8 * ((flag - 1) & 3);
+        if (tid == 0) misc[1] = __hip_atomic_fetch_add(prm.fb_arrive + ((flag - 1) >> 2), 1 << sh, __ATOMIC_RELAXED, __HIP_MEMORY_SCOPE_AGENT);
+        __syncthreads();
+        const bool last_slab = ((misc[1] >> sh) & 0xff) == prm.fb_S - 1;
+        __syncthreads();
+        if (last_slab) knn_exact_fb_merge_slot<IP>(prm, npow2, q, flag - 1, smem);
+    }
+}
+template <bool IP>
+__global__ __launch_bounds__(kFbThreads) void knn_exact_fallback(MergeParams prm, int nq, int npow2) {
+    extern __shared__ __attribute__((aligned(16))) char smem[];
+    if (*prm.fb_slotctr == 0) return;
     for (int q = blockIdx.y; q < nq; q += gridDim.y) {
-        knn_exact_fallback_query<IP>(prm, q, blockIdx.x, smem);
-        __syncthreads();
-    }
-}
-template <bool IP>
-__global__ __launch_bounds__(kFbThreads) void knn_exact_fallback_sel(MergeParams prm, int nq, SelArgs sa) {
-    extern __shared__ __attribute__((aligned(16))) char smem[];
+        knn_exact_fallback_query<IP>(prm, q, blockIdx.x, npow2, smem);
+        __syncthreads();
+    }
+}
+template <bool IP>
+__global__ __launch_bounds__(kFbThreads) void knn_exact_fallback_sel(MergeParams prm, int nq, int npow2, SelArgs sa) {
+    extern __shared__ __attribute__((aligned(16))) char smem[];
+    if (*prm.fb_slotctr == 0) return;
     for (int q = blockIdx.y; q < nq; q += gridDim.y) {
-        knn_exact_fallback_query<IP, true>(prm, q, blockIdx.x, smem, &sa);
-        __syncthreads();
-    }
-}
-
-template <bool IP>
-__device__ __forceinline__ void knn_exact_fb_merge_query(const MergeParams& prm, const int npow2, const int q, char* smem) {
+        knn_exact_fallback_query<IP, true>(prm, q, blockIdx.x, npow2, smem, &sa);
+        __syncthreads();
+    }
+}
+
+template <bool IP>
+__device__ __forceinline__ void knn_exact_fb_merge_slot(const MergeParams& prm, const int npow2, const int q, const int slot, char* smem) {
     const int tid = threadIdx.x;
-    const int flag = prm.flags[q];
-    if (flag <= 0) return;
     double* ds = reinterpret_cast<double*>(smem);
     int32_t* is = reinterpret_cast<int32_t*>(ds + npow2);
     const int n = prm.fb_S * prm.k;
-    const size_t base = (size_t)(flag - 1) * n;
-    for (int t = tid; t < npow2; t += 256) {
-        ds[t] = t < n ? prm.fb_d[base + t] : INFINITY;
-        is[t] = t < n ? prm.fb_i[base + t] : 0x7fffffff;
+    const size_t base = (size_t)slot * n;
+    for (int t = tid; t < npow2; t += kFbThreads) {
+        ds[t] = t < n ? fb_ld_sc1(prm.fb_d + base + t) : INFINITY;
+        is[t] = t < n ? fb_ld_sc1(prm.fb_i + base + t) : 0x7fffffff;
     }
     __syncthreads();
     for (int size = 2; size <= npow2; size <<= 1)
         for (int stride = size >> 1; stride > 0; stride >>= 1) {
-            for (int t = tid; t < (npow2 >> 1); t += 256) {
+            for (int t = tid; t < (npow2 >> 1); t += kFbThreads) {
                 const int lo = 2 * t - (t & (stride - 1));
                 const int hi = lo + stride;
                 const bool asc = (lo & size) == 0;
@@ -436,15 +454,7 @@
             }
             __syncthreads();
         }
-    for (int t = tid; t < prm.k; t += 256) emit_hit<IP>(prm, (size_t)q * prm.k + t, is[t] != 0x7fffffff, ds[t], (int64_t)is[t]);
-}
-template <bool IP>
-__global__ __launch_bounds__(256) void knn_exact_fb_merge(MergeParams prm, int npow2, int nq) {
-    extern __shared__ __attribute__((aligned(16))) char smem[];
-    for (int q = blockIdx.x; q < nq; q += gridDim.x) {
-        knn_exact_fb_merge_query<IP>(prm, npow2, q, smem);
-        __syncthreads();
-    }
+    for (int t = tid; t < prm.k; t += kFbThreads) emit_hit<IP>(prm, (size_t)q * prm.k + t, is[t] != 0x7fffffff, ds[t], (int64_t)is[t]);
 }
 
 template <typename DT, bool DESC = false>
@@ -581,13 +591,15 @@
     ep->fb_S = 4096 / next_pow2(k);
     if (ep->fb_S > 64) ep->fb_S = 64;
     if (ep->fb_S < 1) ep->fb_S = 1;
-    ep->fb_F = fb_F;
+    ep->fb_F = fb_F < 64 ? fb_F : 64;
     const size_t fb_entries = (size_t)fb_F * ep->fb_S * k;
     ep->off_fb_d = take(fb_entries * 8);
     ep->off_fb_i = take(fb_entries * 4);
     ep->off_fb_ctr = take(256);
     ep->merge_lds = list_bytes + align_up((size_t)Dp * 4, 16) + (size_t)kp * 16 + 256 * 4 + 64;
     ep->fb_lds = (size_t)kFbCap * 12 + align_up((size_t)Dp, 4) * 4 + 64;
+    ep->fb_np2 = next_pow2(ep->fb_S * k > 2 ? ep->fb_S * k : 2);
+    if (ep->fb_lds < (size_t)ep->fb_np2 * 12) ep->fb_lds = (size_t)ep->fb_np2 * 12;
 }
 
 MergeParams knn_merge_params(const float* P, int64_t N, int64_t ldP, const float* Q, int64_t ldQ, int D, int Dp, int k, int kp,
@@ -601,6 +613,7 @@
     mp.stats = stats;
     mp.fb_S = ep.fb_S; mp.fb_F = ep.fb_F;
     mp.fb_d = (double*)(ws + ep.off_fb_d); mp.fb_i = (int32_t*)(ws + ep.off_fb_i); mp.fb_slotctr = (int32_t*)(ws + ep.off_fb_ctr);
+    mp.fb_arrive = mp.fb_slotctr + 16;
     return mp;
 }
 
@@ -627,19 +640,14 @@
     if (rc != AC_OK || mp.N == 0) return rc;
     const dim3 fb_grid(ep.fb_S, nq < kFbQueryGroups ? nq : kFbQueryGroups);
     if (sel) {
-        void (*fbs_fn)(MergeParams, int, SelArgs) = ip ? knn_exact_fallback_sel<true> : knn_exact_fallback_sel<false>;
+        void (*fbs_fn)(MergeParams, int, int, SelArgs) = ip ? knn_exact_fallback_sel<true> : knn_exact_fallback_sel<false>;
         (void)hipFuncSetAttribute((const void*)fbs_fn, hipFuncAttributeMaxDynamicSharedMemorySize, (int)ep.fb_lds);
-        hipLaunchKernelGGL(fbs_fn, fb_grid, dim3(kFbThreads), ep.fb_lds, stream, mp, nq, *sel);
+        hipLaunchKernelGGL(fbs_fn, fb_grid, dim3(kFbThreads), ep.fb_lds, stream, mp, nq, ep.fb_np2, *sel);
     } else {
-    void (*fb_fn)(MergeParams, int) = ip ? knn_exact_fallback<true> : knn_exact_fallback<false>;
-    (void)hipFuncSetAttribute((const void*)fb_fn, hipFuncAttributeMaxDynamicSharedMemorySize, (int)ep.fb_lds);
-    hipLaunchKernelGGL(fb_fn, fb_grid, dim3(kFbThreads), ep.fb_lds, stream, mp, nq);
-    }
-    AC_LAUNCH_CHECK();
-    const int np2 = next_pow2(ep.fb_S * mp.k > 2 ? ep.fb_S * mp.k : 2);
-    void (*fbm_fn)(MergeParams, int, int) = ip ? knn_exact_fb_merge<true> : knn_exact_fb_merge<false>;
-    (void)hipFuncSetAttribute((const void*)fbm_fn, hipFuncAttributeMaxDynamicSharedMemorySize, np2 * 12);
-    hipLaunchKernelGGL(fbm_fn, dim3(nq < kFbMergeGroups ? nq : kFbMergeGroups), dim3(256), (size_t)np2 * 12, stream, mp, np2, nq);
+        void (*fb_fn)(MergeParams, int, int) = ip ? knn_exact_fallback<true> : knn_exact_fallback<false>;
+        (void)hipFuncSetAttribute((const void*)fb_fn, hipFuncAttributeMaxDynamicSharedMemorySize, (int)ep.fb_lds);
+        hipLaunchKernelGGL(fb_fn, fb_grid, dim3(kFbThreads), ep.fb_lds, stream, mp, nq, ep.fb_np2);
+    }
     AC_LAUNCH_CHECK();
     return AC_OK;
 }
```

Result: no change. 55090, median of 6 (+0.3%).
